# rvp-group/srrg2_slam_interfaces

Hardware: AMD Instinct MI355X
Metric: icp_iterations_per_sec (higher is better)
Workload: dtype f32; 1 GPU; C2: SE(3) point-to-plane AlignerSlice, 100000-pt synthetic cloud pair per GPU, 10 ICP iterations per compute(), gated NN 0.25 m + normal gate, Cauchy 0.05; points=100000, alignments_total=1, all_success=True, last_status=0, last_num_inliers=99432, parallelism=single GPU

## Files before the change

### __graft_entry__.py

```python
import os
import subprocess
import sys

ROOT = os.path.dirname(os.path.abspath(__file__))
if ROOT not in sys.path:
    sys.path.insert(0, ROOT)


def build():
    env = dict(os.environ)
    env.setdefault("HIPCC", "/opt/rocm/bin/hipcc")
    subprocess.check_call(["make", "-j", str(min(8, os.cpu_count() or 1)), "-C", os.path.join(ROOT, "srrg2_slam_interfaces_amd", "csrc"),
                           "ARCH=gfx950", "all", "stall"], env=env)
    subprocess.check_call(["make", "-C", os.path.join(ROOT, "oracle")], env=env)
    subprocess.check_call(["make", "-C", os.path.join(ROOT, "tests", "cpp")], env=env)
    import srrg2_slam_interfaces_amd
    from srrg2_slam_interfaces_amd import _capi

    lib = _capi.lib()
    assert lib.srrg2_amd_abi_version() == 4


def smoke():
    import numpy as np

    import srrg2_slam_interfaces_amd as pkg
    from oracle import pyoracle
    from srrg2_slam_interfaces_amd import _abi as abi
    from srrg2_slam_interfaces_amd import synthetic as syn

    d = syn.cloud_pair_3d(n=8000, seed=77)
    runs = []
    for al in (pyoracle.OracleAligner(abi.SE3_QUAT_RIGHT), pkg.MultiAligner(abi.SE3_QUAT_RIGHT, device=0)):
        c = abi.default_slice_config(abi.SE3_QUAT_RIGHT)
        c.kind = abi.SLICE_P2PLANE
        c.finder_max_distance = 0.25
        c.robustifier = abi.ROBUST_CAUCHY
        c.robustifier_chi_threshold = 0.05
        si = al.add_slice(c)
        al.set_fixed(si, d["fixed"], d["fixed_normals"])
        al.set_moving(si, d["moving"], d["moving_normals"])
        al.set_moving_in_fixed(syn.identity(3))
        al.compute()
        runs.append(al)
    ref, gpu = runs
    assert ref.status() == gpu.status() == abi.SUCCESS, (ref.status(), gpu.status())
    cr, cg = ref.correspondences(0), gpu.correspondences(0)
    assert np.array_equal(cr["fixed_idx"], cg["fixed_idx"]) and np.array_equal(cr["moving_idx"], cg["moving_idx"])
    assert np.max(np.abs(ref.moving_in_fixed() - gpu.moving_in_fixed())) <= 1e-5
    print("smoke ok: %d correspondences, X bit-identical=%s" %
          (len(cg), ref.moving_in_fixed().tobytes() == gpu.moving_in_fixed().tobytes()))


if __name__ == "__main__":
    build()
    if len(sys.argv) > 1 and sys.argv[1] == "smoke":
        smoke()
```

### include/srrg2_slam_amd.h

```cpp
#ifndef SRRG2_SLAM_AMD_H
#define SRRG2_SLAM_AMD_H

#include <stddef.h>
#include <stdint.h>

#ifdef __cplusplus
extern "C" {
#endif

#define SRRG2_AMD_ABI_VERSION 4
#define SRRG2_MAX_SLICES 8


enum srrg2_variable_kind {
  SRRG2_SE2_RIGHT       = 0,
  SRRG2_SE3_EULER_RIGHT = 1,
  SRRG2_SE3_QUAT_RIGHT  = 2
};

enum srrg2_status {
  SRRG2_SUCCESS                    = 0,
  SRRG2_NOT_ENOUGH_CORRESPONDENCES = 1,
  SRRG2_NOT_ENOUGH_INLIERS         = 2,
  SRRG2_FAIL                       = 3
// ... 363 lines not shown
                      srrg2_merge_result* out);
int srrg2_scene_merge_from_aligner(srrg2_scene_h scene, srrg2_scene_h measurement, const float* measurement_in_scene,
                                   srrg2_aligner_h aligner, int slice_idx, srrg2_scene_h clipped,
                                   const srrg2_merger_params* p, srrg2_merge_result* out);


enum srrg2_adaptor_status { SRRG2_ADAPTOR_READY = 0, SRRG2_ADAPTOR_INITIALIZING = 1, SRRG2_ADAPTOR_ERROR = 2 };
enum srrg2_image_type { SRRG2_IMAGE_NONE = 0, SRRG2_IMAGE_U8 = 1, SRRG2_IMAGE_U16 = 2, SRRG2_IMAGE_F32 = 3 };

typedef struct srrg2_depth_adaptor_params {
  float camera_matrix[9];
  int32_t rows, cols;
  float depth_scale;
  float depth_min, depth_max;
  int32_t normal_col_gap, normal_row_gap;
  float normal_max_distance_squared;
  int32_t drop_points_without_normal;
  int32_t compact;
} srrg2_depth_adaptor_params;

typedef struct srrg2_scan_adaptor_params {
  double angle_min, angle_increment;
  float range_min, range_max;
  int32_t normal_half_window;
  float normal_max_distance_squared;
  int32_t drop_points_without_normal;
  int32_t compact;
} srrg2_scan_adaptor_params;

typedef struct srrg2_adapt_result {
  int32_t status;
  int32_t num_raw;
  int32_t num_in_range;
  int32_t num_valid;
  int32_t scene_size;
} srrg2_adapt_result;

void srrg2_adapt_default_depth_params(srrg2_depth_adaptor_params* p);
void srrg2_adapt_default_scan_params(srrg2_scan_adaptor_params* p);
int srrg2_adapt_depth_image(srrg2_scene_h dst, const void* depth, int depth_type, int depth_row_stride_bytes,
                            const void* intensity, int intensity_type, int intensity_row_stride_bytes, int mem,
                            const srrg2_depth_adaptor_params* p, srrg2_adapt_result* out );
int srrg2_adapt_laser_scan(srrg2_scene_h dst, const float* ranges, int num_beams, int mem,
                           const srrg2_scan_adaptor_params* p, srrg2_adapt_result* out );

#define SRRG2_TUNE_PROJ_SEPARATE_LAUNCHES (1 << 17)
#define SRRG2_TUNE_INIT_LAUNCH (1 << 23)
#define SRRG2_TUNE_KNOWN_BITS (SRRG2_TUNE_PROJ_SEPARATE_LAUNCHES | SRRG2_TUNE_INIT_LAUNCH)
typedef struct srrg2_aligner_tuning {
  int32_t strategy_mask;
  int32_t queue_probe_iteration;
  int32_t small_max_points;
  int32_t fast_from_iteration;
  int32_t fast_points_per_thread;
  int32_t fast_min_points;
  int32_t fast_gather;
  int32_t fast_batch_queue;
  int32_t queue_min_points;
  int32_t msort_segments;
  int32_t msort_key_bits;
  int32_t lds_tile;
  float   cell_target;
  float   rmax_cap;
  int32_t search_lists;
  int32_t search_team;
  int32_t batch_pipeline;
  int32_t fused_control;
  int32_t reserved_[6];
} srrg2_aligner_tuning;
void srrg2_aligner_default_tuning(srrg2_aligner_tuning* t);
int srrg2_aligner_get_tuning(srrg2_aligner_h h, srrg2_aligner_tuning* t_out);
int srrg2_aligner_set_tuning(srrg2_aligner_h h, const srrg2_aligner_tuning* t);


int srrg2_aligner_profile_enable(srrg2_aligner_h h, int enable);
int srrg2_aligner_profile_get(srrg2_aligner_h h, double* step_kernel_ms, int64_t* step_kernel_launches,
                              int reset);
#define SRRG2_PATH_FUSED_CONTROL 1
#define SRRG2_PATH_ALL_PASSES_FUSED 2
#define SRRG2_PATH_FINAL_WAVE 4
#define SRRG2_PATH_PROLOGUE_IN_PASS 8
#define SRRG2_PATH_ONE_WORKGROUP 16
#define SRRG2_PATH_PRIORS_FUSED 32
int srrg2_aligner_last_compute_path(srrg2_aligner_h h, int32_t* flags_out);

#ifndef SRRG2_DESCRIPTOR_BYTES
#define SRRG2_DESCRIPTOR_BYTES 32
#endif
typedef struct srrg2_descriptor_db* srrg2_descriptor_db_h;
int srrg2_descriptor_db_create(int device, srrg2_descriptor_db_h* out);
int srrg2_descriptor_db_destroy(srrg2_descriptor_db_h h);
int srrg2_descriptor_db_add(srrg2_descriptor_db_h h, const uint8_t* descriptors, const uint8_t* valid, int n,
                            int* index_out);
int srrg2_descriptor_db_size(srrg2_descriptor_db_h h, int* maps, int64_t* descriptors);
int srrg2_descriptor_db_match(srrg2_descriptor_db_h h, const uint8_t* descriptors, const uint8_t* valid, int n,
                              int64_t query_index, float max_distance, uint32_t min_age, int64_t min_matches,
                              int* K_out);
int srrg2_descriptor_db_get_candidates(srrg2_descriptor_db_h h, int32_t* reference, int64_t* num_matches,
                                       int64_t* corr_offsets, int* n_inout);
int srrg2_descriptor_db_get_correspondences(srrg2_descriptor_db_h h, srrg2_correspondence* buf, int64_t* n_inout);
int srrg2_descriptor_db_get_map_counts(srrg2_descriptor_db_h h, int64_t* counts, int* n_inout);
int srrg2_descriptor_db_last_match_ms(srrg2_descriptor_db_h h, double* ms);
int srrg2_descriptor_db_add_scene(srrg2_descriptor_db_h h, srrg2_scene_h scene, int* index_out);
int srrg2_descriptor_db_match_scene(srrg2_descriptor_db_h h, srrg2_scene_h scene, int64_t query_index, float max_distance,
                                    uint32_t min_age, int64_t min_matches, int* K_out);

#ifdef __cplusplus
}
#endif
#endif
```

### srrg2_slam_interfaces_amd/_abi.py

```python
import ctypes as C

ABI_VERSION = 4
MAX_SLICES = 8

SE2_RIGHT, SE3_EULER_RIGHT, SE3_QUAT_RIGHT = 0, 1, 2
SUCCESS, NOT_ENOUGH_CORRESPONDENCES, NOT_ENOUGH_INLIERS, FAIL = 0, 1, 2, 3
SLICE_P2P, SLICE_P2PLANE, SLICE_REPROJECTION, SLICE_PRIOR = 0, 1, 2, 3
FINDER_NONE, FINDER_NN_GATED, FINDER_PROJECTIVE, FINDER_CORRESPONDENCES = 0, 1, 2, 3
ROBUST_NONE, ROBUST_CLAMP, ROBUST_SATURATED, ROBUST_CAUCHY = 0, 1, 2, 3
FACTOR_INLIER, FACTOR_KERNELIZED, FACTOR_SUPPRESSED = 0, 1, 2
MEM_HOST, MEM_DEVICE, MEM_DEVICE_KEPT = 0, 1, 2


class Correspondence(C.Structure):
    _fields_ = [("fixed_idx", C.c_int32), ("moving_idx", C.c_int32), ("response", C.c_float)]


class IterationStats(C.Structure):
    _fields_ = [
        ("iteration", C.c_int32),
        ("num_inliers", C.c_int32),
        ("num_outliers", C.c_int32),
        ("num_suppressed", C.c_int32),
        ("num_correspondences", C.c_int32),
# ... 121 lines not shown
        ("angle_min", C.c_double),
        ("angle_increment", C.c_double),
        ("range_min", C.c_float),
        ("range_max", C.c_float),
        ("normal_half_window", C.c_int32),
        ("normal_max_distance_squared", C.c_float),
        ("drop_points_without_normal", C.c_int32),
        ("compact", C.c_int32),
    ]


class AdaptResult(C.Structure):
    _fields_ = [("status", C.c_int32), ("num_raw", C.c_int32), ("num_in_range", C.c_int32), ("num_valid", C.c_int32),
                ("scene_size", C.c_int32)]

    def as_dict(self):
        return {n: getattr(self, n) for n, _ in self._fields_}


class NormalsParams(C.Structure):
    _fields_ = [("radius", C.c_float), ("min_neighbours", C.c_int32), ("max_curvature", C.c_float), ("viewpoint", C.c_float * 3),
                ("drop_points_without_normal", C.c_int32), ("reserved", C.c_int32)]


class NormalsResult(C.Structure):
    _fields_ = [("num_points", C.c_int32), ("num_finite", C.c_int32), ("num_with_normal", C.c_int32), ("num_too_few", C.c_int32),
                ("num_degenerate", C.c_int32), ("num_too_curved", C.c_int32), ("scene_size", C.c_int32)]

    def as_dict(self):
        return {n: getattr(self, n) for n, _ in self._fields_}


VOXEL_CENTROID, VOXEL_FIRST = 0, 1


class VoxelParams(C.Structure):
    _fields_ = [("leaf_size", C.c_float), ("origin", C.c_float * 3), ("mode", C.c_int32), ("min_points_per_voxel", C.c_int32),
                ("reserved", C.c_int32 * 2)]


class VoxelResult(C.Structure):
    _fields_ = [("num_points", C.c_int32), ("num_finite", C.c_int32), ("num_occupied", C.c_int32), ("num_voxels", C.c_int32),
                ("num_with_normal", C.c_int32), ("max_points_per_voxel", C.c_int32)]

    def as_dict(self):
        return {n: getattr(self, n) for n, _ in self._fields_}


def transform_size(variable_kind):
    return 9 if variable_kind == SE2_RIGHT else 12


def point_dim(variable_kind):
    return 2 if variable_kind == SE2_RIGHT else 3


def default_aligner_params():
    return AlignerParams(10, 10, 0, 0)


def default_termination_params():
    return TerminationParams(5, 20, 20, 20, 0.2)


def default_slice_config(variable_kind):
    c = SliceConfig()
    c.kind = SLICE_P2P
    c.finder = FINDER_NN_GATED
    c.robustifier = ROBUST_NONE
    c.robustifier_chi_threshold = 1.0
    c.min_num_correspondences = 0
    c.finder_max_distance = 1.0
    c.finder_normal_cos = -2.0
    c.finder_cell_size = 0.0
    ident = [1, 0, 0, 0, 1, 0, 0, 0, 1] if variable_kind == SE2_RIGHT else [1, 0, 0, 0, 0, 1, 0, 0, 0, 0, 1, 0]
    for i, v in enumerate(ident):
        c.sensor_in_robot[i] = v
    for i in range(6):
        c.prior_information_diag[i] = 100.0 if variable_kind == SE2_RIGHT else 1.0
    c.prior_sets_initial_guess = 1
    return c

PATH_FUSED_CONTROL, PATH_ALL_PASSES_FUSED, PATH_FINAL_WAVE, PATH_PROLOGUE_IN_PASS, PATH_ONE_WORKGROUP, PATH_PRIORS_FUSED = 1, 2, 4, 8, 16, 32
```

### srrg2_slam_interfaces_amd/csrc/aligner_host.hip

```cpp
#include <algorithm>
#include <cmath>
#include <cstdio>
#include <cstdlib>
#include <chrono>
#include <cstring>
#include <string>
#include <vector>

#include "det_math.h"
#include "kernels.h"

#include "host_util.h"

namespace srrg2amd {
thread_local std::string g_err;
int fail(int code, const std::string& msg) {
  g_err = msg;
  return code;
}
}

namespace {

using srrg2amd::DevBuf;
// ... 32 lines not shown
  bool moving_has_normals = false;
  DevBuf<int> corr_fixed;
  DevBuf<srrg2_correspondence> gcorr;
  DevBuf<int> gcorr_off;
  DevBuf<uint8_t> gcorr_stat;
  std::vector<srrg2_correspondence> h_gcorr;
  std::vector<int> h_gcorr_off;
  int* qprobe_host = nullptr; size_t qprobe_cap = 0;
  ProblemDev* ms_probs_host = nullptr; size_t ms_probs_host_cap = 0;
  bool ms_pending = false;
  bool fast_queue_only = false;
  DevBuf<float4> prev_f;
  DevBuf<float> prev_m;
  DevBuf<unsigned long long> dbg;
  DevBuf<float4> prev_n;
  DevBuf<int> prev_pos;
  DevBuf<float> corr_resp;
  DevBuf<uint8_t> corr_stat;
  DevBuf<long long> partials;
  const void* slots_zeroed_at = nullptr;
  int slots_zeroed = 0;
  unsigned* bbox_host = nullptr; size_t bbox_host_cap = 0;
  unsigned bbox_seq = 0;
  bool scalars_self_init = false;
  DevBuf<unsigned> bbox_rows;
  DevBuf<unsigned long long> zbuf;
  DevBuf<int> queue;
  DevBuf<int> qcount;
  float prior_Z[12]{};
  bool has_prior = false;
  void release() {
    if (qprobe_host) (void) hipHostFree(qprobe_host);
    qprobe_host = nullptr;
    qprobe_cap  = 0;
    if (bbox_host) (void) hipHostFree(bbox_host);
    bbox_host     = nullptr;
    bbox_host_cap = 0;
    if (ms_probs_host) (void) hipHostFree(ms_probs_host);
    ms_probs_host     = nullptr;
    ms_probs_host_cap = 0;
    fixed_raw.release(); fixed_nrm_raw.release(); fixed_sorted.release(); fixed_nrm_sorted.release();
    cell_start.release(); cursor.release(); scan_sums.release(); scalars.release(); pos_of.release();
    list_start.release(); list_sums.release(); list_ent.release(); list_box.release(); list_offs.release(); list_hdr.release();
    moving.release(); moving_nrm.release(); pinf.release();
    moving_raw.release(); moving_nrm_raw.release(); ms_counts.release(); ms_cursor.release(); ms_sums.release();
    ms_bb.release(); ms_probs.release();
    corr_fixed.release(); gcorr.release(); gcorr_off.release(); gcorr_stat.release(); prev_n.release(); prev_pos.release(); prev_f.release(); prev_m.release(); corr_resp.release(); corr_stat.release(); partials.release(); zbuf.release(); queue.release(); qcount.release(); bbox_rows.release();
  }
};

}

struct srrg2_aligner_s {
  int kind = 0, dim = 3, dof = 6, tsize = 12, device = 0;
  hipStream_t stream = nullptr;
  static constexpr int MAX_PARTS = 8;
  hipStream_t pstream[MAX_PARTS]{};
  int cu_count          = 256;
  int fused_grid_max    = 130000;
  hipEvent_t ev_staged  = nullptr;
  hipEvent_t ev_records = nullptr;
  bool records_unsynced = false;
  int parts_dirty       = 0;
  int batch_parts       = 0;
  int part_begin[MAX_PARTS + 1]{};
  srrg2_aligner_params params{10, 10, 0, 0};
  srrg2_reduce_fn reduce_fn = nullptr;
  void* reduce_user         = nullptr;
  long long shard_total     = 0;
  bool has_term = false;
  srrg2_termination_params term{5, 20, 20, 20, 0.2f};
  std::vector<Slice*> slices;
  float X[12]{};
  int status = SRRG2_FAIL;
  int K = 1;
  DevBuf<ProblemDev> probs;
  DevBuf<ProblemState> states;
  DevBuf<ProblemOut> outs;
  DevBuf<srrg2_iteration_stats> stats;
  DevBuf<float> guesses;
  DevBuf<unsigned long long> pub;
  DevBuf<unsigned> pub_epoch;
  DevBuf<CtlParams> ctl_dev;
  DevBuf<char> staging;
  DevBuf<float4> pair_raw, pair_nrm_raw, pair_sorted, pair_nrm_sorted;
  DevBuf<int> pair_cell_start, pair_cursor, pair_scan_sums, pair_pos_of;
  DevBuf<unsigned> pair_rows;
  DevBuf<ProblemDev> pair_fprobs;
  DevBuf<GridDev> pair_grids;
  DevBuf<char> pair_staging;
  unsigned* pair_rows_host = nullptr; size_t pair_rows_host_cap = 0;
  ProblemDev* pair_fprobs_host = nullptr; size_t pair_fprobs_host_cap = 0;
  GridDev* pair_grids_host = nullptr; size_t pair_grids_host_cap = 0;
  bool pair_normals  = false;
  bool pairs_computed = false;
  ProblemOut* outs_host = nullptr; size_t outs_host_cap = 0;
  int seq = 0;
  srrg2_iteration_stats* stats_host = nullptr; size_t stats_host_cap = 0;
  float* guesses_host = nullptr; size_t guesses_host_cap = 0;
  ProblemDev* probs_host = nullptr; size_t probs_host_cap = 0;
  int max_stats = 0;
  std::vector<srrg2_iteration_stats> last_stats;
  int last_ncorr[SRRG2_MAX_SLICES]{};
  float last_H[36]{};
  bool computed = false;
  int last_path = 0;
  int records_state = 0;
  std::vector<SliceDev> last_sdev;
  std::vector<int> last_proj_owner;
  std::vector<int> last_nm_max;
  srrg2_aligner_tuning tuning{};
  std::string timeline_path;
  bool hosttime = false;
  bool profile = false;
  double prof_ms = 0.0;
  int64_t prof_launches = 0;
  std::vector<std::pair<hipEvent_t, hipEvent_t>> prof_events;
  size_t prof_used = 0;
};

namespace {

using srrg2_aligner = srrg2_aligner_s;

void identity(int kind, float* T) {
  if (kind == SRRG2_SE2_RIGHT) {
    const float I[9] = {1, 0, 0, 0, 1, 0, 0, 0, 1};
    std::memcpy(T, I, sizeof(I));
  } else {
    const float I[12] = {1, 0, 0, 0, 0, 1, 0, 0, 0, 0, 1, 0};
    std::memcpy(T, I, sizeof(I));
  }
}

float proj_extent(int n, float c) {
  return std::fmax(std::fmax((float) n, std::fabs(c + 0.5f)), std::fabs(((float) n - 0.5f) - c));
}

int set_device(srrg2_aligner* a) {
  HIP_TRY(hipSetDevice(a->device));
  return 0;
}

int quiesce_stream2(srrg2_aligner* a) {
  const int n    = a->parts_dirty;
  a->parts_dirty = 0;
  for (int p = 1; p < n; ++p) HIP_TRY(hipStreamSynchronize(a->pstream[p]));
  return 0;
}

template <typename T>
int ensure_pinned(T*& p, size_t& cap, size_t n) {
  if (n <= cap) return 0;
  if (p) (void) hipHostFree(p);
  p = nullptr;
  cap = 0;
  HIP_TRY(hipHostMalloc((void**) &p, (n + 16) * sizeof(T), hipHostMallocDefault));
  cap = n + 16;
  return 0;
}

int stage_input(srrg2_aligner* a, const float* src, int stride_bytes, int n, int dim, int mem, const float** dev_ptr,
                int* stride_floats, size_t staging_offset, DevBuf<char>* staging = nullptr) {
  DevBuf<char>& stg = staging ? *staging : a->staging;
  if (n <= 0) {
    *dev_ptr       = (const float*) stg.p;
// ... 503 lines not shown
  const int split = (K > 1 && a->batch_parts >= 2 && a->part_begin[a->batch_parts] == K) ? a->batch_parts : 0;
  a->batch_parts  = 0;
  if (!split && (rc = quiesce_stream2(a))) return rc;
  const int nslices = (int) a->slices.size();
  int max_nm = 0;
  std::vector<ProblemDev> probs((size_t) K);
  for (int si = 0; si < nslices; ++si) {
    Slice* s = a->slices[si];
    if (s->alias_of < 0) continue;
    if (s->alias_of >= nslices || a->slices[s->alias_of]->alias_of >= 0 || a->slices[s->alias_of]->cfg.kind == SRRG2_SLICE_PRIOR)
      return fail(SRRG2_E_STATE, "compute: a slice shares the clouds of a slice that is gone");
    Slice* o = a->slices[s->alias_of];
    if (s->cfg.finder != SRRG2_FINDER_PROJECTIVE || o->cfg.finder != SRRG2_FINDER_PROJECTIVE)
      return fail(SRRG2_E_UNSUPPORTED, "compute: shared clouds are for slices with the projective finder");
    s->fixed_raw.borrow(o->fixed_raw);   s->fixed_nrm_raw.borrow(o->fixed_nrm_raw);
    s->moving.borrow(o->moving);         s->moving_nrm.borrow(o->moving_nrm);
    s->moving_raw.borrow(o->moving_raw); s->moving_nrm_raw.borrow(o->moving_nrm_raw);
    s->pinf.borrow(o->pinf);             s->scalars.borrow(o->scalars);
    s->nf = o->nf; s->nm_total = o->nm_total; s->has_fixed = o->has_fixed; s->has_moving = o->has_moving;
    s->fixed_has_normals = o->fixed_has_normals; s->moving_has_normals = o->moving_has_normals;
    s->moving_is_batch = o->moving_is_batch;
    const size_t n = (size_t) std::max(s->nm_total, 1);
    if ((rc = s->corr_fixed.reserve(n)) || (rc = s->corr_resp.reserve(n)) || (rc = s->corr_stat.reserve(n))) return rc;
  }
  for (int si = 0; si < nslices; ++si) {
    Slice* s = a->slices[si];
    if (s->cfg.kind == SRRG2_SLICE_PRIOR) {
      if (!s->has_prior) return fail(SRRG2_E_STATE, "compute: prior slice without measurement");
      continue;
    }
    if (!s->has_fixed && !pairs) return fail(SRRG2_E_STATE, "compute: cue slice| no fixed");
    if (!s->has_moving) return fail(SRRG2_E_STATE, "compute: cue slice| no moving");
    if (K == 1 && s->moving_is_batch)
      return fail(SRRG2_E_STATE, "compute: the moving cloud bound to the cue slice is the concatenation of the last "
                                 "compute_batch (K > 1); bind one with set_moving first");
    if (s->cfg.kind == SRRG2_SLICE_P2PLANE && !(pairs ? a->pair_normals : s->fixed_has_normals))
      return fail(SRRG2_E_STATE, "compute: point-to-plane slice needs fixed normals");
    if (s->cfg.finder == SRRG2_FINDER_PROJECTIVE && s->nf != s->cfg.image_rows * s->cfg.image_cols)
      return fail(SRRG2_E_STATE, "compute: projective finder needs an organised fixed cloud of rows x cols points");
  }
  const int slots = 2 * std::max(a->params.max_iterations, 1);
  a->max_stats    = slots;
  if ((rc = a->probs.reserve((size_t) K * std::max(nslices, 1)))) return rc;
  if ((rc = a->states.reserve((size_t) K))) return rc;
  if ((rc = a->outs.reserve((size_t) K))) return rc;
  if ((rc = a->stats.reserve((size_t) K * slots))) return rc;
  if ((rc = a->guesses.reserve((size_t) K * a->tsize))) return rc;
  if ((rc = ensure_pinned(a->outs_host, a->outs_host_cap, (size_t) K))) return rc;
  if ((rc = ensure_pinned(a->stats_host, a->stats_host_cap, (size_t) K * slots))) return rc;
  if ((rc = ensure_pinned(a->guesses_host, a->guesses_host_cap, (size_t) K * a->tsize))) return rc;
  std::memcpy(a->guesses_host, guesses, (size_t) K * a->tsize * sizeof(float));
  if ((rc = ensure_pinned(a->probs_host, a->probs_host_cap, (size_t) K * std::max(nslices, 1)))) return rc;
  std::vector<ProblemDev> all((size_t) K * std::max(nslices, 1));
  for (int si = 0; si < nslices; ++si) {
    Slice* s = a->slices[si];
    const int32_t* off = slice_offsets ? slice_offsets[s->alias_of >= 0 ? s->alias_of : si] : offsets;
    for (int k = 0; k < K; ++k) {
      ProblemDev pd{0, 0};
      if (s->cfg.kind != SRRG2_SLICE_PRIOR) {
        if (K == 1) {
          pd.moff = 0;
          pd.nm   = s->nm_total;
        } else {
          pd.moff = off[k] - off[0];
          pd.nm   = off[k + 1] - off[k];
        }
        max_nm = std::max(max_nm, pd.nm);
      }
      all[(size_t) si * K + k] = pd;
    }
  }
  std::memcpy(a->probs_host, all.data(), all.size() * sizeof(ProblemDev));

  CtlParams C{};
  C.variable_kind = a->kind;
  C.nslices       = nslices;
  C.K             = K;
  C.params        = a->params;
  C.has_term      = a->has_term ? 1 : 0;
  C.term          = a->term;
  C.max_stats     = slots;
  C.seq           = ++a->seq;
  if (C.seq <= 0) C.seq = a->seq = 1;
  for (int k = 0; k < K; ++k) a->outs_host[k].seq = 0;
  const srrg2_aligner_tuning& tn = a->tuning;
  C.probe_it      = tn.queue_probe_iteration;
  if (a->params.max_iterations <= C.probe_it + 3 || K > 4) C.probe_it = -1;
  bool small = false;
  {
    int ncue = 0, fc = -1;
    for (int si = 0; si < nslices; ++si)
      if (a->slices[si]->cfg.kind != SRRG2_SLICE_PRIOR) {
        if (fc < 0) fc = si;
        ++ncue;
      }
    const int small_max = tn.small_max_points;
    small = ncue == 1 && a->slices[fc]->cfg.finder == SRRG2_FINDER_NN_GATED && max_nm <= small_max &&
            a->timeline_path.empty() && !a->reduce_fn;
    const bool priors_launch = nslices > ncue && (tn.fused_control == 2 || nslices - ncue > 2);
    if (small && !pairs && (priors_launch || tn.fused_control == 0 || a->params.max_iterations < 2)) small = max_nm <= 640;
    if (small && !pairs && !(priors_launch || tn.fused_control == 0 || a->params.max_iterations < 2)) {
      const Slice* sfc = a->slices[fc];
      const int sl     = tn.search_lists;
      const bool lists = sl >= 2 || (sl == 1 && K > 4) || (sl < 0 && (K > 4 || sfc->grid_computes >= 1 || sfc->lists_tried));
      small            = !lists && max_nm <= 384;
    }
  }
  const int fast_from = tn.fast_from_iteration;
  bool fuse = false;
  auto fast_ppt_of = [&](int k_launch) {
    return tn.fast_points_per_thread > 0 ? tn.fast_points_per_thread : (k_launch >= (fuse ? 16 : 64) ? 2 : 1);
  };
  const int fast_min = tn.fast_min_points;
  const bool fast_gather = tn.fast_gather >= 0 ? tn.fast_gather != 0 : K > 4;
  const bool fast_batch_queue = tn.fast_batch_queue != 0;
  const int lds_tile = pairs ? 0 : (tn.lds_tile >= 0 ? tn.lds_tile : (K > 4 ? 1 : 0));
  const int search_lists = tn.search_lists;
  const int search_team_knob = tn.search_team;
  std::vector<char> cnl((size_t) std::max(nslices, 1), 0);
  std::vector<SliceDev> sdev((size_t) nslices);
  int first_cue = -1;
  for (int si = 0; si < nslices; ++si) {
    Slice* s     = a->slices[si];
    SliceCtl& sc = C.slices[si];
    sc.kind                     = s->cfg.kind;
    sc.min_num_correspondences  = s->cfg.min_num_correspondences;
    sc.robust_kind              = s->cfg.robustifier;
    sc.robust_thr               = s->cfg.robustifier_chi_threshold;
    sc.gate                     = s->cfg.finder_max_distance;
    sc.has_prior                = s->has_prior ? 1 : 0;
    sc.prior_sets_initial_guess = s->cfg.prior_sets_initial_guess;
    std::memcpy(sc.prior_Z, s->prior_Z, sizeof(sc.prior_Z));
    std::memcpy(sc.prior_info, s->cfg.prior_information_diag, sizeof(sc.prior_info));
    sc.partials  = nullptr;
    sc.finder    = s->cfg.finder;
    sc.K0        = s->cfg.camera_matrix[0];
    sc.K4        = s->cfg.camera_matrix[4];
    sc.umax      = proj_extent(s->cfg.image_cols, s->cfg.camera_matrix[2]);
    sc.vmax      = proj_extent(s->cfg.image_rows, s->cfg.camera_matrix[5]);
    sc.depth_min = s->cfg.depth_min;
    sc.pinf_bits = nullptr;
    sc.ninf_bits = nullptr;
    if (s->cfg.kind == SRRG2_SLICE_PRIOR) continue;
    if (first_cue < 0) first_cue = si;
    int nm_max_s = 0;
    for (int k = 0; k < K; ++k) nm_max_s = std::max(nm_max_s, all[(size_t) si * K + k].nm);
    const int queue_min = tn.queue_min_points;
    const bool want_lists = search_lists >= 2 || (search_lists == 1 && K > 4) ||
                            (search_lists < 0 && (K > 4 || s->grid_computes >= 1 || s->lists_tried));
    if (!pairs) s->grid_computes++;
    if (s->cfg.finder == SRRG2_FINDER_NN_GATED && !small && want_lists && !pairs) {
      if ((rc = ensure_lists(a, s, 96LL << 20))) return rc;
      cnl[(size_t) si] = s->grid.list_R > 0 ? 1 : 0;
    }
    const bool use_queue = s->cfg.finder == SRRG2_FINDER_NN_GATED && nm_max_s >= queue_min && K <= 4 && !small && !cnl[(size_t) si] && !pairs;
    const bool fast_queue = s->cfg.finder == SRRG2_FINDER_NN_GATED && K > 4 && !small && fast_batch_queue && !pairs;
    s->fast_queue_only = fast_queue && !use_queue;
    const int nblocks    = PARTIAL_SLOTS;
    {
      const size_t cap_before = s->partials.cap;
      if ((rc = s->partials.reserve((size_t) 3 * K * nblocks * ACC_N))) return rc;
      if (s->partials.cap != cap_before) s->slots_zeroed = 0;
    }
    if (use_queue || fast_queue) {
      if ((rc = s->queue.reserve((size_t) std::max(s->nm_total, 1) * 10))) return rc;
      if ((rc = s->qcount.reserve((size_t) 2 * K))) return rc;
    }
// ... 273 lines not shown
                                       a->probs.p + (size_t) first_cue * K, a->states.p, a->stats.p, a->outs_host, a->stats_host,
                                       a->stream);
    else
      srrg2amd::launch_icp_small(a->dim, s->cfg.kind == SRRG2_SLICE_P2PLANE, sdev[first_cue], C,
                                 a->probs.p + (size_t) first_cue * K, a->states.p, a->stats.p, a->outs_host, a->stats_host,
                                 a->stream);
  }
  const int probe_it = C.probe_it;
  std::vector<char> queue_on((size_t) std::max(nslices, 1), 1);
  bool probed = false;
  bool final_launched = false;
  auto read_probe = [&]() {
    probed = true;
    for (int si = 0; si < nslices; ++si) {
      if (!sdev[si].queue) continue;
      volatile int* mirror = a->slices[si]->qprobe_host;
      bool small           = true;
      for (int k = 0; k < K; ++k) {
        int spins = 0;
        while (mirror[2 * k] == 0x7f7f7f7f || mirror[2 * k + 1] == 0x7f7f7f7f) {
          if ((++spins & 1023) == 0 && hipStreamQuery(a->stream) != hipErrorNotReady) break;
        }
        const int near = mirror[2 * k], far = mirror[2 * k + 1];
        if (near == 0x7f7f7f7f || far > 32 || near > std::max(1024, all[(size_t) si * K + k].nm / 64)) small = false;
      }
      queue_on[(size_t) si] = small ? 0 : 1;
    }
  };
  auto fused_pass = [&](int slot0, int it) {
    if (!fuse) return false;
    if (fused_all) return true;
    const bool queue_needed = sdev[first_cue].queue && queue_on[(size_t) first_cue];
    return fast_at(slot0, it) && !queue_needed && (slot0 > 0 || probed || probe_it < 0 || !sdev[first_cue].queue);
  };
  auto control = [&](int it, bool last_phase, int h) {
    if (a->reduce_fn) {
      Slice* s = a->slices[first_cue];
      if (a->reduce_fn(a->reduce_user, SRRG2_REDUCE_SUM_I64, s->partials.p, (size_t) K * PARTIAL_SLOTS * ACC_N, (void*) a->stream))
        hook_failed = true;
    }
    const bool last_it = it == a->params.max_iterations - 1;
    if (fuse) {
      Ch[h].parity      = pround % 3;
      Ch[h].zero_parity = (pround + 2) % 3;
      Ch[h].epoch       = epoch + 1;
      const int slot0_now = last_phase && a->params.enable_inlier_only_runs ? a->params.max_iterations : 0;
      if (!fused_all && !probed && slot0_now == 0 && probe_it >= 0 && it == probe_it + 1) read_probe();
      if (!last_it && fused_pass(slot0_now, it + 1) && (fused_all || it != probe_it)) return;
    }
    if (last_phase && last_it) {
      if (fuse && fuse_proj) {
        SliceDev pack[4];
        const ProblemDev* pp[4];
        for (size_t z = 0; z < proj_group.size(); ++z) {
          const int si = proj_group[z];
          Slice* sz    = a->slices[si];
          pack[z]      = sdev[si];
          pp[z]        = a->probs.p + (size_t) si * K;
          pack[z].fc.ctl           = a->ctl_dev.p;
          pack[z].fc.epoch         = epoch + 1;
          pack[z].fc.prev_partials = slot_buffer(sz, pround);
          pack[z].fc.zero_partials = slot_buffer(sz, pround + 2);
        }
        srrg2amd::launch_icp_final_wave_pack(pack, pp, (int) proj_group.size(), a->states.p, a->stats.p, a->outs_host, a->stats_host,
                                             !a->params.enable_inlier_only_runs, hstream[h]);
      } else if (fuse) {
        SliceDev sd          = sdev[first_cue];
        sd.prob0             = h0[h];
        sd.fc.ctl            = a->ctl_dev.p + h;
        sd.fc.epoch          = epoch + 1;
        sd.fc.prev_partials  = slot_buffer(a->slices[first_cue], pround);
        sd.fc.zero_partials  = slot_buffer(a->slices[first_cue], pround + 2);
        srrg2amd::launch_icp_final_wave(Ch[h], sd, a->states.p, a->stats.p, a->outs_host, a->stats_host,
                                        !a->params.enable_inlier_only_runs, hstream[h]);
      } else {
        srrg2amd::launch_icp_control_final(Ch[h], a->states.p, a->stats.p, a->outs_host, a->stats_host,
                                           !a->params.enable_inlier_only_runs , hstream[h]);
      }
      final_launched = true;
    } else {
      srrg2amd::launch_icp_control(Ch[h], a->states.p, a->stats.p, hstream[h]);
    }
  };
  auto run_phase = [&](int slot0, bool last_phase) -> int {
    for (int it = 0; it < a->params.max_iterations; ++it) {
      if (!probed && slot0 == 0 && probe_it >= 0 && it == probe_it + 2) read_probe();
      if (!proj_group.empty()) {
        SliceDev pack[4];
        const ProblemDev* pp[4];
        int nm_max = 0;
        for (size_t z = 0; z < proj_group.size(); ++z) {
          const int si = proj_group[z];
          pack[z]      = sdev[si];
          pp[z]        = a->probs.p + (size_t) si * K;
          for (int k = 0; k < K; ++k) nm_max = std::max(nm_max, all[(size_t) si * K + k].nm);
        }
        hipEvent_t e0 = nullptr, e1 = nullptr;
        if (a->profile) {
          if (a->prof_used == a->prof_events.size()) {
            hipEvent_t x, y;
            HIP_TRY(hipEventCreate(&x));
            HIP_TRY(hipEventCreate(&y));
            a->prof_events.emplace_back(x, y);
          }
          e0 = a->prof_events[a->prof_used].first;
          e1 = a->prof_events[a->prof_used].second;
          a->prof_used++;
          HIP_TRY(hipEventRecord(e0, a->stream));
        }
        if (fuse)
          for (size_t z = 0; z < proj_group.size(); ++z) {
            Slice* sz              = a->slices[proj_group[z]];
            pack[z].fc.ctl         = a->ctl_dev.p;
            pack[z].fc.epoch       = epoch;
            pack[z].partials       = slot_buffer(sz, pround);
            pack[z].fc.prev_partials = slot_buffer(sz, pround + 2);
            pack[z].fc.zero_partials = slot_buffer(sz, pround + 1);
            pack[z].fc.prior       = (slot0 > 0 || it > 0) ? 1 : 0;
            if (it == 0) pack[z].fc.prior_mask = 0;
          }
        if (proj_fused) {
          const bool first_pass_init = fold_init && fuse_proj && slot0 == 0 && it == 0;
          srrg2amd::launch_proj_step_fused(pack, pp, (int) proj_group.size(), a->states.p, K, nm_max, a->stream,
                                           first_pass_init ? &Ch[0] : nullptr, first_pass_init ? &fold_inl : nullptr,
                                           first_pass_init ? a->probs.p : nullptr);
          sdev[proj_group[0]].zbuf_parity ^= 1;
        } else {
          srrg2amd::launch_proj_step_pack(pack, pp, (int) proj_group.size(), a->states.p, K, nm_max, a->stream);
          for (int si : proj_group) sdev[si].zbuf_parity ^= 1;
        }
        if (a->profile) HIP_TRY(hipEventRecord(e1, a->stream));
        control(it, last_phase, 0);
        ++epoch;
        ++pround;
        continue;
      }
      for (int si = 0; si < nslices; ++si) {
        Slice* s = a->slices[si];
        if (s->cfg.kind == SRRG2_SLICE_PRIOR) continue;
        const bool plane = s->cfg.kind == SRRG2_SLICE_P2PLANE;
        int nm_max       = 0;
        for (int k = 0; k < K; ++k) nm_max = std::max(nm_max, all[(size_t) si * K + k].nm);
        hipEvent_t e0 = nullptr, e1 = nullptr;
        if (a->profile) {
          if (a->prof_used == a->prof_events.size()) {
            hipEvent_t x, y;
            HIP_TRY(hipEventCreate(&x));
            HIP_TRY(hipEventCreate(&y));
            a->prof_events.emplace_back(x, y);
          }
          e0 = a->prof_events[a->prof_used].first;
          e1 = a->prof_events[a->prof_used].second;
          a->prof_used++;
          HIP_TRY(hipEventRecord(e0, a->stream));
        }
        if (s->cfg.finder == SRRG2_FINDER_CORRESPONDENCES) {
          int max_nc = 0;
          for (int k = 0; k < K; ++k) max_nc = std::max(max_nc, s->h_gcorr_off[(size_t) k + 1] - s->h_gcorr_off[(size_t) k]);
          srrg2amd::launch_corr_step(a->dim, plane, sdev[si], a->probs.p + (size_t) si * K, a->states.p, K, max_nc, a->stream);
        } else if (s->cfg.finder == SRRG2_FINDER_PROJECTIVE) {
          srrg2amd::launch_proj_step(s->cfg.kind == SRRG2_SLICE_REPROJECTION, sdev[si], a->probs.p + (size_t) si * K,
                                     a->states.p, K, nm_max, a->stream);
          sdev[si].zbuf_parity ^= 1;
        } else {
          SliceDev sd = sdev[si];
          const bool fast = (slot0 > 0 || (it >= fast_from && it >= 1)) && nm_max >= fast_min;
          if (!queue_on[si] || (s->fast_queue_only && !fast)) {
            sd.queue  = nullptr;
            sd.qcount = nullptr;
// ... 55 lines not shown
      if ((rc = run_phase(a->params.max_iterations, true))) return rc;
    }
  }
  if (!final_launched)
    for (int h = 0; h < nhalves; ++h)
      srrg2amd::launch_icp_finalize(Ch[h], a->states.p, a->stats.p, a->outs_host, a->stats_host,
                                    !a->params.enable_inlier_only_runs , hstream[h]);
  if (split) a->parts_dirty = std::max(a->parts_dirty, split);
  HIP_TRY(hipGetLastError());
  const bool hosttime = a->hosttime;
  auto t_enq = std::chrono::steady_clock::now();
  bool seen = true;
  for (int k = 0; k < K && seen; ++k) {
    volatile int* flag = &a->outs_host[k].seq;
    int spins          = 0;
    hipStream_t qs = a->stream;
    for (int h = 1; h < nhalves; ++h)
      if (k >= h0[h]) qs = hstream[h];
    while (*flag != C.seq)
      if ((++spins & 4095) == 0 && hipStreamQuery(qs) != hipErrorNotReady) {
        seen = *flag == C.seq;
        break;
      }
  }
  if (!seen || a->profile || !a->timeline_path.empty()) {
    HIP_TRY(hipStreamSynchronize(a->stream));
    for (int h = 1; h < nhalves; ++h) HIP_TRY(hipStreamSynchronize(hstream[h]));
  }
  if (hook_failed) return fail(SRRG2_E_INVALID, "the reduction hook of the point-sharded alignment failed");
  if (hosttime) {
    auto t_end = std::chrono::steady_clock::now();
    std::fprintf(stderr, "compute: prep %.1f us, first launch %.1f us, enqueue %.1f us, wait %.1f us\n",
                 std::chrono::duration<double, std::micro>(t_prep - t_begin).count(),
                 std::chrono::duration<double, std::micro>(t_init - t_prep).count(),
                 std::chrono::duration<double, std::micro>(t_enq - t_begin).count(),
                 std::chrono::duration<double, std::micro>(t_end - t_enq).count());
  }
  if (const char* tl_path = a->timeline_path.empty() ? nullptr : a->timeline_path.c_str()) {
    for (int si = 0; si < nslices; ++si) {
      Slice* s = a->slices[si];
      if (!sdev[si].dbg) continue;
      int nm_max = 0;
      for (int k = 0; k < K; ++k) nm_max = std::max(nm_max, all[(size_t) si * K + k].nm);
      const unsigned long long nw = (unsigned long long) K * ((nm_max + 255) / 256) * 4;
      std::vector<unsigned long long> host(32 * nw * 16);
      HIP_TRY(hipMemcpy(host.data(), s->dbg.p, host.size() * sizeof(unsigned long long), hipMemcpyDeviceToHost));
      if (FILE* f = std::fopen(tl_path, "wb")) {
        std::fwrite(&nw, sizeof(nw), 1, f);
        std::fwrite(host.data(), sizeof(unsigned long long), host.size(), f);
        std::fclose(f);
      }
    }
  }
  if (a->profile) {
    for (size_t i = 0; i < a->prof_used; ++i) {
      float ms = 0.f;
      HIP_TRY(hipEventElapsedTime(&ms, a->prof_events[i].first, a->prof_events[i].second));
      a->prof_ms += ms;
      a->prof_launches++;
    }
    a->prof_used = 0;
  }
  for (Slice* sl : a->slices) sl->ms_pending = false;
  a->K = K;
  const ProblemOut& o = a->outs_host[K - 1];
  std::memcpy(a->X, o.X, sizeof(float) * a->tsize);
  a->status = o.status;
  int ns    = std::min(o.nstats, slots);
  a->last_stats.assign(a->stats_host + (size_t) (K - 1) * slots, a->stats_host + (size_t) (K - 1) * slots + ns);
  for (int si = 0; si < SRRG2_MAX_SLICES; ++si) a->last_ncorr[si] = o.ncorr[si];
  std::memcpy(a->last_H, o.H, sizeof(a->last_H));
  a->computed = true;
  a->last_sdev = sdev;
  a->last_proj_owner.assign((size_t) nslices, -1);
  if (proj_fused)
    for (int si : proj_group) a->last_proj_owner[(size_t) si] = proj_group[0];
  a->last_nm_max.assign((size_t) nslices, 0);
  for (int si = 0; si < nslices; ++si)
    for (int k = 0; k < K; ++k) a->last_nm_max[(size_t) si] = std::max(a->last_nm_max[(size_t) si], all[(size_t) si * K + k].nm);
  a->records_state  = pairs ? 2 : 1;
  a->pairs_computed = pairs;
  a->last_path = (fuse ? SRRG2_PATH_FUSED_CONTROL : 0) | (fuse && fused_all ? SRRG2_PATH_ALL_PASSES_FUSED : 0) |
                 (fuse && final_launched && !small ? SRRG2_PATH_FINAL_WAVE : 0) | (fold_init ? SRRG2_PATH_PROLOGUE_IN_PASS : 0) |
                 (small ? SRRG2_PATH_ONE_WORKGROUP : 0) | (fuse && prior_mask ? SRRG2_PATH_PRIORS_FUSED : 0);
  if (fuse && final_launched && first_cue >= 0 && !small) {
    for (int si = 0; si < nslices; ++si) {
      if (si != first_cue && !(fuse_proj && std::find(proj_group.begin(), proj_group.end(), si) != proj_group.end())) continue;
      Slice* s           = a->slices[si];
      s->slots_zeroed    = 3 * K;
      s->slots_zeroed_at = (const void*) s->partials.p;
    }
  }
  return 0;
}

int plan_batch_parts(srrg2_aligner* a, int K, const int32_t* offsets, int* pbegin) {
  int nparts = 0;
  {
    const srrg2_aligner_tuning& tn = a->tuning;
    int max_nm = 0;
    for (int k = 0; k < K; ++k) max_nm = std::max(max_nm, offsets[k + 1] - offsets[k]);
    bool one_cue = true;
    for (size_t si = 1; si < a->slices.size(); ++si)
      if (a->slices[si]->cfg.kind != SRRG2_SLICE_PRIOR) one_cue = false;
    int want = tn.batch_pipeline == 0 ? 1 : (tn.batch_pipeline == 1 ? 2 : (tn.batch_pipeline > 1 ? tn.batch_pipeline : (K >= 8 ? 2 : 1)));
    want     = std::min(std::min(want, (int) srrg2_aligner::MAX_PARTS), K);
    if (want >= 2 && one_cue && a->slices[0]->cfg.finder == SRRG2_FINDER_NN_GATED && max_nm > tn.small_max_points &&
        !tn.fast_batch_queue && !a->reduce_fn && !a->profile && a->timeline_path.empty()) {
      nparts = want;
      for (int p = 1; p < nparts; ++p)
        if (!a->pstream[p] && hipStreamCreateWithFlags(&a->pstream[p], hipStreamNonBlocking) != hipSuccess) {
          (void) hipGetLastError();
          a->pstream[p] = nullptr;
          nparts        = p >= 2 ? p : 0;
          break;
        }
      for (int p = 0; p <= nparts; ++p) pbegin[p] = (int) ((long long) K * p / nparts);
    }
  }
  return nparts;
}

void fill_batch_results(const srrg2_aligner* a, int K, srrg2_batch_result* results) {
  const int slots = a->max_stats;
  for (int k = 0; k < K; ++k) {
    const ProblemOut& o = a->outs_host[k];
    std::memset(&results[k], 0, sizeof(results[k]));
    std::memcpy(results[k].moving_in_fixed, o.X, sizeof(float) * a->tsize);
    results[k].status         = o.status;
    results[k].num_iterations = o.nstats;
    if (o.nstats > 0) results[k].last = a->stats_host[(size_t) k * slots + std::min(o.nstats, slots) - 1];
    int tot = 0;
    for (size_t si = 0; si < a->slices.size(); ++si) {
      const int c = a->slices[si]->cfg.kind == SRRG2_SLICE_PRIOR ? 1 : o.ncorr[si];
      if (c >= 0) tot += c;
    }
    results[k].num_correspondences = tot;
    std::memcpy(results[k].information, o.H, sizeof(o.H));
  }
}

int materialize_records(srrg2_aligner* a, bool host_wait = true) {
  if (a->records_state != 1) {
    if (host_wait && a->records_unsynced) {
      HIP_TRY(hipStreamSynchronize(a->stream));
      a->records_unsynced = false;
    }
    return 0;
  }
  int rc;
  if ((rc = set_device(a))) return rc;
  if ((rc = quiesce_stream2(a))) return rc;
  std::vector<char> rebuilt(a->slices.size(), 0);
  for (size_t si = 0; si < a->slices.size() && si < a->last_sdev.size(); ++si) {
    Slice* s = a->slices[si];
    if (s->cfg.kind == SRRG2_SLICE_PRIOR) continue;
    if (s->cfg.finder == SRRG2_FINDER_PROJECTIVE) {
      const int owner = si < a->last_proj_owner.size() && a->last_proj_owner[si] >= 0 ? a->last_proj_owner[si] : (int) si;
      srrg2amd::launch_proj_records(a->last_sdev[(size_t) owner], a->last_sdev[si], a->probs.p + (size_t) owner * a->K,
                                    a->probs.p + si * (size_t) a->K, a->states.p, a->K, a->last_nm_max[si],
                                    !rebuilt[(size_t) owner], a->stream);
      rebuilt[(size_t) owner] = 1;
      continue;
    }
    if (s->cfg.finder != SRRG2_FINDER_NN_GATED) continue;
    srrg2amd::launch_icp_outputs(a->dim, s->cfg.kind == SRRG2_SLICE_P2PLANE, a->last_sdev[si], a->probs.p + si * (size_t) a->K,
                                 a->states.p, a->K, a->last_nm_max[si], a->stream);
// ... 66 lines not shown
}

int srrg2_aligner_set_tuning(srrg2_aligner_h a, const srrg2_aligner_tuning* t) {
  if (!a || !t) return fail(SRRG2_E_INVALID, "set_tuning: null argument");
  if (t->fast_points_per_thread < 0 || t->fast_from_iteration < 1 || !(t->cell_target > 0.f) || t->msort_key_bits > 18 ||
      t->msort_key_bits < -1 || t->msort_segments < 0 || t->search_team < 0)
    return fail(SRRG2_E_INVALID, "set_tuning: value out of range");
  if (t->strategy_mask & ~SRRG2_TUNE_KNOWN_BITS) return fail(SRRG2_E_INVALID, "set_tuning: unknown strategy_mask bit");
  a->tuning = *t;
  return 0;
}

void srrg2_termination_default_params(srrg2_termination_params* p) {
  if (!p) return;
  p->window_size = 5;
  p->num_correspondences_range = 20;
  p->num_inliers_range = 20;
  p->num_outliers_range = 20;
  p->chi_epsilon = 0.2f;
}

void srrg2_slice_default_config(srrg2_slice_config* c, int variable_kind) {
  if (!c) return;
  std::memset(c, 0, sizeof(*c));
  c->kind = SRRG2_SLICE_P2P;
  c->finder = SRRG2_FINDER_NN_GATED;
  c->robustifier = SRRG2_ROBUST_NONE;
  c->robustifier_chi_threshold = 1.f;
  c->min_num_correspondences = 0;
  c->finder_max_distance = 1.f;
  c->finder_normal_cos = -2.f;
  c->finder_cell_size = 0.f;
  identity(variable_kind, c->sensor_in_robot);
  for (int i = 0; i < 6; ++i) c->prior_information_diag[i] = variable_kind == SRRG2_SE2_RIGHT ? 100.f : 1.f;
  c->prior_sets_initial_guess = 1;
}

int srrg2_aligner_create(int variable_kind, int device, srrg2_aligner_h* out) {
  if (!out || variable_kind < 0 || variable_kind > 2) return fail(SRRG2_E_INVALID, "create: bad arguments");
  int n = 0;
  hipError_t e = hipGetDeviceCount(&n);
  if (e != hipSuccess || n <= 0)
    return fail(SRRG2_E_NO_DEVICE, "create: no HIP device visible (this library has no CPU fallback)");
  if (device < 0 || device >= n) return fail(SRRG2_E_INVALID, "create: bad device ordinal");
  srrg2_aligner* a = new srrg2_aligner();
  a->kind   = variable_kind;
  a->dim    = variable_kind == SRRG2_SE2_RIGHT ? 2 : 3;
  a->dof    = variable_kind == SRRG2_SE2_RIGHT ? 3 : 6;
  a->tsize  = variable_kind == SRRG2_SE2_RIGHT ? 9 : 12;
  a->device = device;
  identity(variable_kind, a->X);
  tuning_from_environment(&a->tuning);
  if (const char* tl = std::getenv("SRRG2_AMD_TIMELINE")) a->timeline_path = tl;
  a->hosttime = std::getenv("SRRG2_AMD_HOSTTIME") != nullptr;
  if (const char* fg = std::getenv("SRRG2_AMD_FUSED_GRID_MAX")) a->fused_grid_max = std::atoi(fg);
  bool ok = hipSetDevice(device) == hipSuccess && hipStreamCreateWithFlags(&a->stream, hipStreamNonBlocking) == hipSuccess;
  a->pstream[0] = a->stream;
  ok = ok && hipEventCreateWithFlags(&a->ev_staged, hipEventDisableTiming) == hipSuccess;
  ok = ok && hipEventCreateWithFlags(&a->ev_records, hipEventDisableTiming) == hipSuccess;
  if (ok && (hipDeviceGetAttribute(&a->cu_count, hipDeviceAttributeMultiprocessorCount, device) != hipSuccess || a->cu_count <= 0)) {
    (void) hipGetLastError();
    a->cu_count = 256;
  }
  if (!ok) {
    for (int p = 0; p < srrg2_aligner::MAX_PARTS; ++p)
      if (a->pstream[p]) (void) hipStreamDestroy(a->pstream[p]);
    delete a;
    return fail(SRRG2_E_HIP, "create: cannot create stream");
  }
  *out = a;
  return 0;
}

int srrg2_aligner_destroy(srrg2_aligner_h a) {
  if (!a) return 0;
  (void) hipSetDevice(a->device);
  for (int p = 0; p < srrg2_aligner::MAX_PARTS; ++p)
    if (a->pstream[p]) (void) hipStreamSynchronize(a->pstream[p]);
  for (Slice* s : a->slices) {
    s->release();
    delete s;
  }
  a->probs.release(); a->states.release(); a->outs.release(); a->stats.release(); a->guesses.release();
  a->pub.release(); a->pub_epoch.release(); a->ctl_dev.release();
  a->staging.release();
  a->pair_raw.release(); a->pair_nrm_raw.release(); a->pair_sorted.release(); a->pair_nrm_sorted.release();
  a->pair_cell_start.release(); a->pair_cursor.release(); a->pair_scan_sums.release(); a->pair_pos_of.release();
  a->pair_rows.release(); a->pair_fprobs.release(); a->pair_grids.release(); a->pair_staging.release();
  if (a->pair_rows_host) (void) hipHostFree(a->pair_rows_host);
  if (a->pair_fprobs_host) (void) hipHostFree(a->pair_fprobs_host);
  if (a->pair_grids_host) (void) hipHostFree(a->pair_grids_host);
  if (a->outs_host) (void) hipHostFree(a->outs_host);
  if (a->stats_host) (void) hipHostFree(a->stats_host);
  if (a->guesses_host) (void) hipHostFree(a->guesses_host);
  if (a->probs_host) (void) hipHostFree(a->probs_host);
  for (auto& ev : a->prof_events) {
    (void) hipEventDestroy(ev.first);
    (void) hipEventDestroy(ev.second);
  }
  if (a->ev_staged) (void) hipEventDestroy(a->ev_staged);
  if (a->ev_records) (void) hipEventDestroy(a->ev_records);
  for (int p = srrg2_aligner::MAX_PARTS - 1; p >= 0; --p)
    if (a->pstream[p]) (void) hipStreamDestroy(a->pstream[p]);
  delete a;
  return 0;
}

int srrg2_aligner_set_params(srrg2_aligner_h a, const srrg2_aligner_params* p) {
  if (!a || !p || p->max_iterations < 0) return fail(SRRG2_E_INVALID, "set_params: bad arguments");
  a->params = *p;
  return 0;
}

int srrg2_aligner_set_termination(srrg2_aligner_h a, const srrg2_termination_params* p) {
  if (!a) return fail(SRRG2_E_INVALID, "set_termination: null handle");
  if (!p) {
    a->has_term = false;
    return 0;
  }
  if (p->window_size < 1 || p->window_size > TERM_WINDOW_MAX) return fail(SRRG2_E_INVALID, "set_termination: window_size");
  a->has_term = true;
  a->term     = *p;
  return 0;
}

int srrg2_aligner_add_slice(srrg2_aligner_h a, const srrg2_slice_config* c, int* idx) {
  if (!a || !c) return fail(SRRG2_E_INVALID, "add_slice: bad arguments");
  if ((int) a->slices.size() >= SRRG2_MAX_SLICES) return fail(SRRG2_E_INVALID, "add_slice: too many slices");
  if (c->kind != SRRG2_SLICE_PRIOR && c->finder != SRRG2_FINDER_NN_GATED && c->finder != SRRG2_FINDER_PROJECTIVE &&
      c->finder != SRRG2_FINDER_CORRESPONDENCES)
    return fail(SRRG2_E_INVALID, "add_slice| no finder");
  if (c->finder == SRRG2_FINDER_CORRESPONDENCES && c->kind != SRRG2_SLICE_P2P && c->kind != SRRG2_SLICE_P2PLANE)
    return fail(SRRG2_E_INVALID, "add_slice: given correspondences drive point-to-point / point-to-plane factors");
  if (c->finder == SRRG2_FINDER_PROJECTIVE || c->kind == SRRG2_SLICE_REPROJECTION) {
    if (a->dim != 3) return fail(SRRG2_E_UNSUPPORTED, "add_slice: projective finder / reprojection factor are SE(3) only");
    if (c->finder != SRRG2_FINDER_PROJECTIVE)
      return fail(SRRG2_E_INVALID, "add_slice: a reprojection slice needs the projective finder");
    if (c->image_rows <= 0 || c->image_cols <= 0 || !(c->depth_min > 0.f) || !(c->depth_max >= c->depth_min) ||
        !(c->camera_matrix[0] > 0.f) || !(c->camera_matrix[4] > 0.f))
      return fail(SRRG2_E_INVALID, "add_slice: projective slice with bad camera / image / depth range");
  }
  if (c->kind == SRRG2_SLICE_PRIOR && a->kind == SRRG2_SE3_EULER_RIGHT)
    return fail(SRRG2_E_UNSUPPORTED, "add_slice: SE3 prior factors exist for the quaternion variable only "
                                     "(SE3PriorErrorFactorAD, aligner_slice_odometry_prior.h:33)");
  Slice* s = new Slice();
  s->cfg   = *c;
  if (idx) *idx = (int) a->slices.size();
  a->slices.push_back(s);
  return 0;
}

int srrg2_aligner_clear_slices(srrg2_aligner_h a) {
  if (!a) return fail(SRRG2_E_INVALID, "clear_slices: null handle");
  (void) hipSetDevice(a->device);
  (void) hipStreamSynchronize(a->stream);
  for (Slice* s : a->slices) {
    s->release();
    delete s;
  }
  a->slices.clear();
  return 0;
}

int srrg2_aligner_set_robustifier(srrg2_aligner_h a, int si, int kind, float thr) {
  int rc = check_slice(a, si, "set_robustifier");
  if (rc) return rc;
  a->slices[si]->cfg.robustifier               = kind;
// ... 747 lines not shown
```

### srrg2_slam_interfaces_amd/csrc/device_types.h

```cpp
#pragma once
#include <hip/hip_runtime.h>
#include <stdint.h>

#include "../../include/srrg2_slam_amd.h"

#define ACC_N 32
#define PARTIAL_SLOTS 32
#define ACC_B 21
#define ACC_CHI_IN 27
#define ACC_CHI_OUT 28
#define ACC_N_IN 29
#define ACC_N_OUT 30
#define ACC_N_CORR 31
#define TERM_WINDOW_MAX 64
#define NO_MATCH 0x7fffffff

__host__ __device__ __forceinline__ constexpr int hidx(int a, int b) {
  return a * 6 - (a * (a - 1)) / 2 + (b - a);
}

struct GridDev {
  float ox, oy, oz;
  float h, inv_h;
  int nx, ny, nz;
  int rmax;
  int rfar_gate;
  float gate2;
  float gate2_ext;
  int n;
  const int* cell_start;
  const float4* pts;
  const float4* nrm;
  const int* pos_of;
  int list_R;
  const struct GridLists* lists;
};
struct GridLists {
  int R;
  int lnx, lny, lnz;
  const int* start;
  const uint4* ent;
  float cls_b2[14];
};
#define CNL_MAX_R 3
#ifndef CNL_ENTRY_MAX
#define CNL_ENTRY_MAX 16
#endif
#define CNL_MAX_CLASS 12

#define PUB_SLICE_GRANULES 64
#define PUB_G_KEXP 24
#define PUB_G_FLAGS 25
#define PUB_G_NSTATS 26
#define PUB_G_WCOUNT 27
#define PUB_G_NPASSES 28
#define PUB_G_X 32
#define PUB_FLAG_STOP 1u
#define PUB_FLAG_PHASE1 2u
#define PUB_FLAG_PRIOR 4u
#define PUB_EPOCH_REPLICAS 8
#define PUB_EPOCH_STRIDE 32
struct CtlParams;
struct FusedCtl {
  unsigned long long* pub;
  unsigned* pub_epoch;
  const CtlParams* ctl;
  srrg2_iteration_stats* stats;
  long long* prev_partials;
  long long* zero_partials;
  int epoch;
  int min_num_correspondences;
  int max_stats;
  int has_term;
  int first_round;
  int prior;
  int prior_mask;
  int nslices;
};

struct SliceDev {
  GridDev grid;
  const float4* mpts;
  const float4* mnrm;
  int* corr_fixed;
  float* corr_resp;
  uint8_t* corr_stat;
  float4* prev_f;
  float4* prev_n;
  int* prev_pos;
  float* prev_m;
  long long* partials;
  void* queue;
  int* qcount;
  int slice_idx;
  int robust_kind;
  float robust_thr;
  float normal_cos;
  int use_normal_gate;
  int gather_prev;
  int variable_kind;
  int finder;
  int factor;
  float K[9];
  int rows, cols;
  float depth_min, depth_max;
  float gate;
  const float4* fixed_org;
  const float4* fixed_org_nrm;
  unsigned long long* zbuf;
  int zbuf_parity;
  const srrg2_correspondence* gcorr;
  const int* gcorr_off;
  uint8_t* gcorr_stat;
  const float4* moving_raw;
  unsigned long long* dbg;
  int prob0;
  float Sinv[12];
  FusedCtl fc;
};

struct ProblemDev {
  int moff;
  int nm;
};

struct ProblemState {
  float X[12];
  float Xprev[12];
  int status;
  int done;
  int finished;
  int nstats;
  int phase;
  int kexp[SRRG2_MAX_SLICES];
  int ncorr[SRRG2_MAX_SLICES];
  int ninl[SRRG2_MAX_SLICES];
  int qmode[SRRG2_MAX_SLICES];
  float Tf[SRRG2_MAX_SLICES][12], Tfprev[SRRG2_MAX_SLICES][12];
  float Tlast[SRRG2_MAX_SLICES][12];
  int npasses;
  int w_count;
  double w_corr[TERM_WINDOW_MAX], w_inl[TERM_WINDOW_MAX], w_out[TERM_WINDOW_MAX], w_chi[TERM_WINDOW_MAX];
  double last_H[36], last_b[6], last_dx[6];
};

struct ProblemOut {
  float X[12];
  int status;
  int nstats;
  int ncorr[SRRG2_MAX_SLICES];
  float H[36];
  int seq;
};

struct SliceCtl {
  int kind;
  int min_num_correspondences;
  int robust_kind;
  float robust_thr;
  float gate;
  int has_prior;
  int prior_sets_initial_guess;
  float prior_Z[12];
  float prior_info[6];
  int finder;
  float K0, K4;
  float umax, vmax;
  float depth_min;
  int* qcount;
  int* qprobe_host;
  const ProblemDev* probs;
  int nm_global;
  const long long* partials;
  const unsigned* pinf_bits;
  const unsigned* ninf_bits;
  const unsigned* finf_bits;
  const int* gcorr_off;
  float Sinv[12];
};

#define PAIR_ROW_WORDS 8
#define PAIR_ROW_NINF 7

struct InitInline {
  int use;
  float guess[12];
  ProblemDev pd[SRRG2_MAX_SLICES];
};

#define INIT_BATCH_MAX 16
struct InitBatch {
  float guess[INIT_BATCH_MAX][12];
  ProblemDev pd[INIT_BATCH_MAX];
  int cue_slice;
};

struct CtlParams {
  int variable_kind;
  int nslices;
  int K;
  srrg2_aligner_params params;
  int has_term;
  srrg2_termination_params term;
  int max_stats;
  int probe_it;
  int seq;
  int prob0, nprob;
  unsigned long long* pub;
  unsigned* pub_epoch;
  CtlParams* ctl_dev;
  int epoch;
  int parity;
  int zero_parity;
  SliceCtl slices[SRRG2_MAX_SLICES];
};
```

### srrg2_slam_interfaces_amd/csrc/kernels.h

```cpp
#pragma once
#include "device_types.h"

namespace srrg2amd {

void launch_ingest(const float* src, int stride_floats, int n, int dim, float4* dst, unsigned* maxabs_bits,
                   int finite_per_point, hipStream_t s);
void launch_ingest_batch(const float* src, int stride_floats, const ProblemDev* probs, int K, int max_nm, int dim,
                         float4* dst, unsigned* maxabs_bits, int finite_per_point, hipStream_t s);
void launch_bbox(const float4* pts, int n, unsigned* mn, unsigned* mx, int* nvalid, hipStream_t s);
void launch_ingest_bbox(const float* src, int stride_floats, int n, int dim, float4* dst, unsigned* maxabs_bits, unsigned* mn,
                        unsigned* mx, int* nvalid, hipStream_t s, unsigned* ticket, unsigned* host_out, unsigned seq,
                        unsigned* block_out , unsigned* clear_after);
#define INGEST_BBOX_MAX_BLOCKS 512
void launch_grid_count(const GridDev& g, const float4* pts, int n, int* counts, hipStream_t s);
void launch_count_nonzero(const int* counts, int n, int* out, hipStream_t s);
int scan_num_blocks(int n);
void launch_exclusive_scan(int* data, int n, int* block_sums, int* grand_total, hipStream_t s, int* copy = nullptr);
void launch_grid_scatter(const GridDev& g, const float4* pts, const float4* nrm, int n, int* cursor, float4* out_pts,
                         float4* out_nrm, int* pos_of, hipStream_t s);
void launch_cnl_build(const GridDev& g, const GridLists& L, const int4* offs, int noffs, int* list_start, uint2* box_at,
                      uint4* ent, hipStream_t s);
void launch_icp_step_cnl(int dim, bool plane, const SliceDev& S, const GridLists& GL, const ProblemDev* probs,
                         ProblemState* states, int K, int max_nm, int team, hipStream_t s, const CtlParams* init_C = nullptr,
                         const InitInline* init_inl = nullptr, const InitBatch* init_bat = nullptr);
bool launch_msort_local(const float* src, int sf, const float* nsrc, int nsf, const ProblemDev* probs, int K, int dim, int kbits,
                        int aniso, int segments, int max_nm, float4* out_pts, float4* out_nrm, unsigned* maxabs_bits,
                        hipStream_t s);
void launch_msort(const float4* pts, const float4* nrm, const ProblemDev* probs, int K, int max_nm, int kbits, int aniso,
                  unsigned* bb, int* counts, int* cursor, int* scan_sums, int* scan_total, float4* out_pts,
                  float4* out_nrm, hipStream_t s);
void launch_icp_step(int dim, bool plane, const SliceDev& S, const ProblemDev* probs, ProblemState* states, int K,
                     int max_nm, hipStream_t s, const CtlParams* init_C = nullptr, const InitInline* init_inl = nullptr);
void launch_icp_step_tile(int dim, bool plane, const SliceDev& S, const ProblemDev* probs, ProblemState* states, int K,
                          int max_nm, int cap, hipStream_t s);
void launch_icp_step_fast(int dim, bool plane, const SliceDev& S, const ProblemDev* probs, ProblemState* states, int K,
                          int max_nm, int ppt, bool gather, hipStream_t s);
void launch_icp_outputs(int dim, bool plane, const SliceDev& S, const ProblemDev* probs, const ProblemState* states, int K,
                        int max_nm, hipStream_t s);
int icp_step_blocks(int max_nm);
int icp_queue_blocks(int max_nm, int K);
void launch_proj_step_pack(const SliceDev* slices, const ProblemDev* const* probs, int nslices, ProblemState* states, int K,
                           int max_nm, hipStream_t s);
void launch_proj_records(const SliceDev& S0, const SliceDev& S, const ProblemDev* probs0, const ProblemDev* probs,
                         ProblemState* states, int K, int max_nm, bool rebuild, hipStream_t s);
void launch_proj_step_fused(const SliceDev* slices, const ProblemDev* const* probs, int nslices, ProblemState* states, int K,
                            int max_nm, hipStream_t s,
                            const CtlParams* init_C = nullptr, const InitInline* init_inl = nullptr, ProblemDev* probs_base = nullptr);
void launch_corr_step(int dim, bool plane, const SliceDev& S, const ProblemDev* probs, ProblemState* states, int K,
                      int max_ncorr, hipStream_t s);
void launch_proj_step(bool repro, const SliceDev& S, const ProblemDev* probs, ProblemState* states, int K, int max_nm,
                      hipStream_t s);
void launch_icp_init(const CtlParams& C, const ProblemDev* probs_host, ProblemDev* probs, ProblemState* states,
                     const float* guesses_host, int tsize, hipStream_t s, bool pairs = false);
bool make_init_inline(const CtlParams& C, const ProblemDev* probs_host, const float* guesses_host, int tsize, InitInline* inl);
void launch_icp_control(const CtlParams& C, ProblemState* states, srrg2_iteration_stats* stats, hipStream_t s);
void launch_icp_final_wave_pack(const SliceDev* slices, const ProblemDev* const* probs, int nslices, ProblemState* states,
                                srrg2_iteration_stats* stats, ProblemOut* outs_host, srrg2_iteration_stats* stats_host,
                                bool with_post, hipStream_t s);
void launch_icp_small(int dim, bool plane, const SliceDev& S, const CtlParams& C, const ProblemDev* probs, ProblemState* states,
                      srrg2_iteration_stats* stats, ProblemOut* outs_host, srrg2_iteration_stats* stats_host, hipStream_t s);
void launch_icp_step_pairs(int dim, bool plane, const SliceDev& S, const GridDev* grids, const ProblemDev* probs,
                           ProblemState* states, int K, int max_nm, hipStream_t s);
void launch_icp_step_fast_pairs(int dim, bool plane, const SliceDev& S, const GridDev* grids, const ProblemDev* probs,
                                ProblemState* states, int K, int max_nm, int ppt, bool gather, hipStream_t s);
void launch_icp_small_pairs(int dim, bool plane, const SliceDev& S, const GridDev* grids, const CtlParams& C, const ProblemDev* probs,
                            ProblemState* states, srrg2_iteration_stats* stats, ProblemOut* outs_host,
                            srrg2_iteration_stats* stats_host, hipStream_t s);
void launch_pairs_ingest(const float* src, int sf, const float* nsrc, int nsf, const ProblemDev* fprobs, int K, int max_nf, int dim,
                         float4* dst, float4* dst_nrm, unsigned* rows, hipStream_t s);
void launch_pairs_grid_build(const GridDev* grids, const ProblemDev* fprobs, int K, int max_nf, int max_cells, int total_cells,
                             const float4* pts, const float4* nrm, int* cell_start, int* cursor, int* scan_sums, int* scan_total,
                             float4* out_pts, float4* out_nrm, int* pos_of, hipStream_t s);
void launch_icp_final_wave(const CtlParams& C, const SliceDev& S, ProblemState* states, srrg2_iteration_stats* stats,
                           ProblemOut* outs_host, srrg2_iteration_stats* stats_host, bool with_post, hipStream_t s);
void launch_icp_control_final(const CtlParams& C, ProblemState* states, srrg2_iteration_stats* stats, ProblemOut* outs_host,
                               srrg2_iteration_stats* stats_host, bool with_post, hipStream_t s);
void launch_icp_post(const CtlParams& C, ProblemState* states, const srrg2_iteration_stats* stats, hipStream_t s);
void launch_icp_finalize(const CtlParams& C, ProblemState* states, const srrg2_iteration_stats* stats,
                         ProblemOut* outs_host, srrg2_iteration_stats* stats_host, bool with_post, hipStream_t s);

}
```

### srrg2_slam_interfaces_amd/csrc/kernels.hip

```cpp
#include <cstdlib>
#include <algorithm>

#include "kernels.h"

#include <type_traits>

#include "det_math.h"

#include "device_util.h"

namespace {

#define FX_MAGIC 6755399441055744.0
#define FX_MAGIC_BITS 0x4338000000000000ll
__device__ __forceinline__ long long fx_bits(double biased) { return __double_as_longlong(biased) - FX_MAGIC_BITS; }

__device__ __forceinline__ unsigned long long key_min(unsigned long long a, unsigned long long b) {
  double r;
  asm("v_min_f64 %0, %1, %2" : "=v"(r) : "v"(__longlong_as_double((long long) a)), "v"(__longlong_as_double((long long) b)));
  return (unsigned long long) __double_as_longlong(r);
}

template <int DIM>
__device__ __forceinline__ float cand_d2(const float4 f, float qx, float qy, float qz) {
// ... 1826 lines not shown
        ((st->nstats > 0 || st->phase == 1) ? PUB_FLAG_PRIOR : 0u);
  else if (lane == PUB_G_NSTATS) v = (unsigned) st->nstats;
  else if (lane == PUB_G_WCOUNT) v = (unsigned) st->w_count;
  else if (lane == PUB_G_NPASSES) v = (unsigned) st->npasses;
  else if (lane >= PUB_G_X && lane < PUB_G_X + 12) v = __float_as_uint(st->X[lane - PUB_G_X]);
  return v;
}
__device__ __forceinline__ void pub_write_epoch(unsigned* pub_epoch, int prob, int lane, unsigned epoch) {
  if (lane < PUB_EPOCH_REPLICAS)
    __hip_atomic_store(pub_epoch + ((size_t) prob * PUB_EPOCH_REPLICAS + lane) * PUB_EPOCH_STRIDE, epoch, __ATOMIC_RELAXED,
                       __HIP_MEMORY_SCOPE_AGENT);
}
__device__ __forceinline__ void pub_publish_state(const CtlParams& C, const ProblemState* st, int prob, int lane, unsigned epoch) {
  for (int s = 0; s < C.nslices; ++s) {
    if (C.slices[s].kind == SRRG2_SLICE_PRIOR) continue;
    pub_store(C.pub + ((size_t) prob * SRRG2_MAX_SLICES + s) * PUB_SLICE_GRANULES + lane,
              ((unsigned long long) epoch << 32) | pub_granule_of(C, st, s, lane));
  }
}

template <int D>
__device__ __forceinline__ int wave_prior(const float (&prior_Z)[12], const float (&prior_info)[6], float robust_thr, int rk,
                                          const float (&X)[12], int lane, double& pH, double& pb, double& chi_out) {
  const int hr = lane / D, hc = lane - hr * D;
  double e[D];
  float Zinv[12], E[12];
  double qw = 0.0;
  if constexpr (D == 6) {
    dm::se3_inverse(prior_Z, Zinv);
    dm::se3_compose(Zinv, X, E);
    dm::se3_t2v_quat(E, e);
    const double n2 = (e[3] * e[3] + e[4] * e[4]) + e[5] * e[5];
    qw              = n2 < 1.0 ? sqrt(1.0 - n2) : 0.0;
  } else {
    dm::se2_inverse(prior_Z, Zinv);
    dm::se2_compose(Zinv, X, E);
    dm::se2_t2v(E, e);
  }
  auto Jat = [&](int k, int col) -> double {
    if constexpr (D == 6) {
      if (k < 3) return col == 0 ? (double) E[k * 4 + 0] : (col == 1 ? (double) E[k * 4 + 1] : (col == 2 ? (double) E[k * 4 + 2] : 0.0));
      const double m0 = k == 3 ? qw : (k == 4 ? e[5] : -e[4]);
      const double m1 = k == 3 ? -e[5] : (k == 4 ? qw : e[3]);
      const double m2 = k == 3 ? e[4] : (k == 4 ? -e[3] : qw);
      return col == 3 ? m0 : (col == 4 ? m1 : (col == 5 ? m2 : 0.0));
    } else {
      if (k < 2) return col == 0 ? (double) E[k * 3 + 0] : (col == 1 ? (double) E[k * 3 + 1] : 0.0);
      return col == 2 ? 1.0 : 0.0;
    }
  };
  double chi = 0.0;
#pragma unroll
  for (int i = 0; i < D; ++i) chi = chi + (e[i] * (double) prior_info[i]) * e[i];
  bool kernelized;
  const float w = robust_weight(rk, robust_thr, (float) chi, kernelized);
  chi_out       = chi;
  const int status = !isfinite(chi) ? (int) SRRG2_FACTOR_SUPPRESSED
                                    : (kernelized ? (int) SRRG2_FACTOR_KERNELIZED : (int) SRRG2_FACTOR_INLIER);
  pH = 0.0;
  pb = 0.0;
  if (status == SRRG2_FACTOR_SUPPRESSED) return status;
  double th = 0.0, tb = 0.0;
#pragma unroll
  for (int k = 0; k < D; ++k) {
    th = th + (Jat(k, hr) * (double) prior_info[k]) * Jat(k, hc);
    tb = tb + (Jat(k, lane) * (double) prior_info[k]) * e[k];
  }
  pH = (double) w * th;
  pb = (double) w * tb;
  return status;
}

struct FinalRegs {
  bool applied;
  float Xl;
  double Hl;
  int nstats;
  int num_in;
  int sw;
  bool stats_written;
  int nc[4], ni[4];
};

template <int D, int MAXS, bool PUBLISH = true, bool PRIORS = false, bool FINAL = false>
__device__ __forceinline__ void wave_control(const SliceDev* __restrict__ Sv, int ns, ProblemState* __restrict__ states, int prob,
                                             const unsigned long long (&g)[MAXS], unsigned (*out)[MAXS] = nullptr,
                                             FinalRegs* fin = nullptr) {
  if constexpr (FINAL) fin->applied = false;
  const FusedCtl& F  = Sv[0].fc;
  const int lane     = threadIdx.x & 63;
  ProblemState* st   = &states[prob];
  const unsigned epoch = (unsigned) F.epoch;
  constexpr int TS   = D == 3 ? 9 : 12;
  int pw[SRRG2_MAX_SLICES];
#pragma unroll
  for (int q = 0; q < SRRG2_MAX_SLICES; ++q) {
    pw[q] = 0;
    if constexpr (PRIORS)
      if (((unsigned) F.prior_mask >> q) & 1u) pw[q] = reinterpret_cast<const int*>(&F.ctl->slices[q])[lane & 31];
  }
  long long v[MAXS];
#pragma unroll
  for (int z = 0; z < MAXS; ++z) {
    v[z] = 0;
    if (z < ns) {
      const long long* p = Sv[z].fc.prev_partials + (size_t) prob * PARTIAL_SLOTS * ACC_N;
#pragma unroll
      for (int q = 0; q < PARTIAL_SLOTS * ACC_N / 64; ++q) v[z] += p[q * 64 + lane];
    }
  }
  const int w          = (int) (unsigned) g[0];
  float Xl             = __int_as_float(__shfl(w, (PUB_G_X + lane) & 63));
  const unsigned fl0   = (unsigned) __builtin_amdgcn_readlane(w, PUB_G_FLAGS);
  const int nstats0    = __builtin_amdgcn_readlane(w, PUB_G_NSTATS);
  const int wc         = __builtin_amdgcn_readlane(w, PUB_G_WCOUNT);
  const int npasses0   = __builtin_amdgcn_readlane(w, PUB_G_NPASSES);
  float told[MAXS];
  int kexp[MAXS];
#pragma unroll
  for (int z = 0; z < MAXS; ++z) {
    told[z] = __int_as_float((int) (unsigned) g[z]);
    kexp[z] = __builtin_amdgcn_readlane((int) (unsigned) g[z], PUB_G_KEXP);
  }
  if (fl0 & PUB_FLAG_STOP) {
#pragma unroll
    for (int z = 0; z < MAXS; ++z)
      if (z < ns) {
        if constexpr (PUBLISH)
          pub_store(F.pub + ((size_t) prob * SRRG2_MAX_SLICES + Sv[z].slice_idx) * PUB_SLICE_GRANULES + lane,
                    ((unsigned long long) epoch << 32) | (unsigned) g[z]);
        else
          (*out)[z] = (unsigned) g[z];
      }
    if constexpr (PUBLISH) pub_write_epoch(F.pub_epoch, prob, lane, epoch);
    return;
  }
  double wo = 0.0, wi = 0.0, wx = 0.0;
  int W = 1;
  if (F.has_term) {
    W = F.ctl->term.window_size;
    if (lane < W) {
      wo = st->w_out[lane];
      wi = st->w_inl[lane];
      wx = st->w_chi[lane];
    }
  }
  int ps0 = -1, ps1 = -1, pt0 = 0, pt1 = 0;
  double pH0 = 0.0, pb0 = 0.0, pc0 = 0.0, pH1 = 0.0, pb1 = 0.0, pc1 = 0.0;
  if constexpr (PRIORS) {
    const unsigned pm0 = (unsigned) F.prior_mask, pm1 = pm0 & (pm0 - 1u);
    ps0 = pm0 ? __builtin_ctz(pm0) : -1;
    ps1 = pm1 ? __builtin_ctz(pm1) : -1;
    float Xa[12];
#pragma unroll
    for (int i = 0; i < 12; ++i) Xa[i] = i < TS ? rl_f(Xl, i) : 0.f;
#pragma unroll 1
    for (int j = 0; j < 2; ++j) {
      const int sl = j == 0 ? ps0 : ps1;
      if (sl < 0) break;
      int pword = pw[0];
#pragma unroll
      for (int q = 1; q < SRRG2_MAX_SLICES; ++q) pword = sl == q ? pw[q] : pword;
      constexpr int W_RK = (int) (offsetof(SliceCtl, robust_kind) / 4), W_THR = (int) (offsetof(SliceCtl, robust_thr) / 4),
                    W_Z = (int) (offsetof(SliceCtl, prior_Z) / 4), W_INFO = (int) (offsetof(SliceCtl, prior_info) / 4);
      static_assert(W_INFO + 6 <= 32, "the prefetched head of SliceCtl covers the prior's fields");
      const int robust_kind  = __builtin_amdgcn_readlane(pword, W_RK);
      const float robust_thr = __int_as_float(__builtin_amdgcn_readlane(pword, W_THR));
      float pZ[12], pinfo[6];
#pragma unroll
      for (int i = 0; i < 12; ++i) pZ[i] = __int_as_float(__builtin_amdgcn_readlane(pword, W_Z + i));
#pragma unroll
      for (int i = 0; i < 6; ++i) pinfo[i] = __int_as_float(__builtin_amdgcn_readlane(pword, W_INFO + i));
      const int rk = ((fl0 & PUB_FLAG_PHASE1) && robust_kind != SRRG2_ROBUST_NONE) ? (int) SRRG2_ROBUST_CLAMP : robust_kind;
      double pH, pb, pchi;
      const int pstat = wave_prior<D>(pZ, pinfo, robust_thr, rk, Xa, lane, pH, pb, pchi);
      if (j == 0) {
        pH0 = pH; pb0 = pb; pc0 = pchi; pt0 = pstat;
      } else {
        pH1 = pH; pb1 = pb; pc1 = pchi; pt1 = pstat;
      }
    }
  }
  const int hr = lane / D, hc = lane - hr * D;
  const int hsrc = hidx(hr < hc ? hr : hc, hr < hc ? hc : hr) & 31;
  double Hl = 0.0, bl = 0.0;
  int num_in = 0, num_out = 0, num_sup = 0, num_corr = 0;
  double chi_in = 0.0, chi_out = 0.0;
  bool good = false;
  const unsigned pmask = PRIORS ? (unsigned) F.prior_mask : 0u;
  const int first_cue  = Sv[0].slice_idx;
  const int s_end      = pmask ? F.nslices : first_cue + 1;
#pragma unroll 1
  for (int sl = pmask ? 0 : first_cue; sl < s_end; ++sl) {
  if ((pmask >> sl) & 1u) {
    const bool pfirst = sl == ps0;
    const double pH = pfirst ? pH0 : pH1, pb = pfirst ? pb0 : pb1, pchi = pfirst ? pc0 : pc1;
    const int pstat = pfirst ? pt0 : pt1;
    good = true;
    Hl   = Hl + pH;
    bl   = bl + pb;
    if (pstat == SRRG2_FACTOR_INLIER) {
      num_in += 1;
      chi_in = chi_in + pchi;
    } else if (pstat == SRRG2_FACTOR_KERNELIZED) {
      num_out += 1;
      chi_out = chi_out + pchi;
    } else {
      num_sup += 1;
    }
    num_corr += 1;
    if constexpr (PUBLISH)
      if (lane == 0) st->ninl[sl] = pstat == SRRG2_FACTOR_INLIER ? 1 : 0;
    continue;
  }
  if (sl != first_cue) continue;
#pragma unroll
  for (int z = 0; z < MAXS; ++z) {
    if (z >= ns) break;
    v[z] += __shfl_xor(v[z], 32);
    if constexpr (PUBLISH) {
      long long* p = Sv[z].fc.zero_partials + (size_t) prob * PARTIAL_SLOTS * ACC_N;
#pragma unroll
      for (int q = 0; q < PARTIAL_SLOTS * ACC_N / 64; ++q) p[q * 64 + lane] = 0;
    }
    const double scaled = (double) v[z] * dm::pow2(-kexp[z]);
    const int nc = (int) rl_ll(v[z], ACC_N_CORR), n_in = (int) rl_ll(v[z], ACC_N_IN), n_out = (int) rl_ll(v[z], ACC_N_OUT);
    good |= nc > Sv[z].fc.min_num_correspondences;
    if constexpr (FINAL)
      if (z < 4) {
        fin->nc[z] = nc;
        fin->ni[z] = n_in;
      }
    Hl = Hl + __shfl(scaled, hsrc);
    bl = bl + __shfl(scaled, (ACC_B + lane) & 31);
    num_in += n_in;
    num_out += n_out;
    num_sup += nc - n_in - n_out;
    num_corr += nc >= 0 ? nc : 0;
    chi_in  = chi_in + rl_d(scaled, ACC_CHI_IN);
    chi_out = chi_out + rl_d(scaled, ACC_CHI_OUT);
    if constexpr (PUBLISH) {
      const int s = Sv[z].slice_idx;
      if (lane == 0) {
        st->ncorr[s] = nc;
        st->ninl[s]  = n_in;
      }
      if (lane < 12) st->Tlast[s][lane] = told[z];
    }
  }
  }
  if constexpr (PUBLISH)
    if (lane == 0) st->npasses = npasses0 + 1;
  if (!good) {
    if constexpr (PUBLISH)
      if (lane == 0) {
        st->status = SRRG2_NOT_ENOUGH_CORRESPONDENCES;
        st->done   = 1;
      }
#pragma unroll
    for (int z = 0; z < MAXS; ++z) {
      if (z >= ns) break;
      unsigned nv = (unsigned) g[z];
      if (lane == PUB_G_FLAGS) nv = fl0 | PUB_FLAG_STOP;
      if (lane == PUB_G_NPASSES) nv = (unsigned) (npasses0 + 1);
      if constexpr (PUBLISH)
        pub_store(F.pub + ((size_t) prob * SRRG2_MAX_SLICES + Sv[z].slice_idx) * PUB_SLICE_GRANULES + lane,
                  ((unsigned long long) epoch << 32) | nv);
      else
        (*out)[z] = nv;
    }
    if constexpr (PUBLISH) pub_write_epoch(F.pub_epoch, prob, lane, epoch);
    return;
  }
  PASS_TS_W(F.epoch, 5, Hl);
  double Lv = 0.0, Dv = 0.0, Iv = 0.0;
  double Tv = Hl;
  bool bad  = false;
#pragma unroll
  for (int j = 0; j < D; ++j) {
    const double sj = rl_d(Tv, j * D + j);
    if (!(sj > 0.0)) {
      bad = true;
      break;
    }
    const double inv = 1.0 / sj;
    if (lane == j * D + j) {
      Dv = sj;
      Iv = inv;
    }
    if (hc == j && hr > j && lane < D * D) Lv = Tv * inv;
    if (j + 1 < D) {
      const double lij = __shfl(Lv, (hr * D + j) & 63);
      const double ljj = __shfl(Lv, (hc * D + j) & 63);
      Tv               = Tv - (lij * ljj) * sj;
    }
  }
  double yv = 0.0, dxv = 0.0;
  if (!bad) {
    double tv = -bl;
#pragma unroll
    for (int k = 0; k < D; ++k) {
      const double yk = rl_d(tv, k);
      if (lane == k) yv = tv;
      if (k + 1 < D) tv = tv - __shfl(Lv, (lane * D + k) & 63) * yk;
    }
#pragma unroll
// ... 37 lines not shown
        const double qw  = sqrt(small ? 1.0 - n2 : 1.0);
        const double xx = v3 * v3, yy = v4 * v4, zz = v5 * v5;
        const double xy = v3 * v4, xz = v3 * v5, yz = v4 * v5;
        const double wx_ = qw * v3, wy_ = qw * v4, wz_ = qw * v5;
        R0 = small ? 1.0 - 2.0 * (yy + zz) : 1.0; R1 = small ? 2.0 * (xy - wz_) : 0.0;      R2 = small ? 2.0 * (xz + wy_) : 0.0;
        R3 = small ? 2.0 * (xy + wz_) : 0.0;      R4 = small ? 1.0 - 2.0 * (xx + zz) : 1.0; R5 = small ? 2.0 * (yz - wx_) : 0.0;
        R6 = small ? 2.0 * (xz - wy_) : 0.0;      R7 = small ? 2.0 * (yz + wx_) : 0.0;      R8 = small ? 1.0 - 2.0 * (xx + yy) : 1.0;
      } else {
        double sa, ca, sb, cb, sc, cc;
        dm::sincos(v3, sa, ca);
        dm::sincos(v4, sb, cb);
        dm::sincos(v5, sc, cc);
        R0 = cb * cc;                   R1 = -(cb * sc);                R2 = sb;
        R3 = ca * sc + (sa * sb) * cc;  R4 = ca * cc - (sa * sb) * sc;  R5 = -(sa * cb);
        R6 = sa * sc - (ca * sb) * cc;  R7 = sa * cc + (ca * sb) * sc;  R8 = ca * cb;
      }
      const int i = lane >> 2, j = lane & 3;
      const double a0 = (double) __shfl(Xl, (i * 4 + 0) & 63), a1 = (double) __shfl(Xl, (i * 4 + 1) & 63),
                   a2 = (double) __shfl(Xl, (i * 4 + 2) & 63), a3 = (double) __shfl(Xl, (i * 4 + 3) & 63);
      double r0 = v0, r1 = v1, r2 = v2;
      if (j == 0) { r0 = R0; r1 = R3; r2 = R6; }
      if (j == 1) { r0 = R1; r1 = R4; r2 = R7; }
      if (j == 2) { r0 = R2; r1 = R5; r2 = R8; }
      double o = (a0 * r0 + a1 * r1) + a2 * r2;
      if (j == 3) o = o + a3;
      if (lane < 12) Xl = (float) o;
    }
    if constexpr (PUBLISH)
      if (lane < TS) st->X[lane] = Xl;
  }
  PASS_TS_W(F.epoch, 7, (double) Xl);
  const float chi_in_f = (float) chi_in, chi_out_f = (float) chi_out;
  static_assert(sizeof(srrg2_iteration_stats) == 32, "eight words");
  const int sw = lane == 0 ? nstats0 : lane == 1 ? num_in : lane == 2 ? num_out : lane == 3 ? num_sup : lane == 4 ? num_corr
               : lane == 5 ? (bad ? 1 : 0) : lane == 6 ? __float_as_int(chi_in_f) : __float_as_int(chi_out_f);
  if (PUBLISH && nstats0 < F.max_stats && lane < 8) reinterpret_cast<int*>(F.stats + (size_t) prob * F.max_stats + nstats0)[lane] = sw;
  if constexpr (FINAL) {
    fin->applied = true;
    fin->Xl = Xl;
    fin->Hl = Hl;
    fin->nstats = nstats0 + 1;
    fin->num_in = num_in;
    fin->sw = sw;
    fin->stats_written = nstats0 < F.max_stats;
  }
  if constexpr (PUBLISH)
    if (lane == 0) st->nstats = nstats0 + 1;
  bool stop = false;
  int wc1   = wc;
  if (F.has_term && num_in != 0) {
    const srrg2_termination_params& tp = F.ctl->term;
    const float chi = chi_in_f / (float) num_in;
    const int slot  = wc % W;
    const int n     = wc + 1 < W ? wc + 1 : W;
    wc1             = wc + 1;
    if (n >= W) {
      const bool in = lane < n;
      if (lane == slot) {
        wo = (double) num_out;
        wi = (double) num_in;
        wx = (double) chi;
      }
      const double first_o = rl_d(wo, 0), first_i = rl_d(wi, 0), first_x = rl_d(wx, 0);
      const double omax = wave_max_d(in ? wo : first_o), omin = wave_min_d(in ? wo : first_o);
      const double imax = wave_max_d(in ? wi : first_i), imin = wave_min_d(in ? wi : first_i);
      const double xmax = wave_max_d(in ? wx : first_x), xmin = wave_min_d(in ? wx : first_x);
      stop = true;
      if (omax - omin > (double) tp.num_correspondences_range) stop = false;
      if (imax - imin > (double) tp.num_inliers_range) stop = false;
      const float chi_range = (float) (xmax - xmin);
      if (chi_range > (float) tp.num_outliers_range) stop = false;
      if (chi_range / (float) xmax > tp.chi_epsilon) stop = false;
    }
    if (PUBLISH && lane == 0) {
      st->w_corr[slot] = num_corr;
      st->w_inl[slot]  = num_in;
      st->w_out[slot]  = num_out;
      st->w_chi[slot]  = (double) chi;
      st->w_count      = wc + 1;
    }
  }
  if (PUBLISH && stop && lane == 0) st->done = 1;
  const unsigned x_up = __float_as_uint(__shfl(Xl, (lane - PUB_G_X) & 63));
#pragma unroll
  for (int z = 0; z < MAXS; ++z) {
    if (z >= ns) break;
    const int s = Sv[z].slice_idx;
    float tnew  = told[z];
    if (!bad) {
      const float* A = Sv[z].Sinv;
      const int i = (lane >> 2) % 3, j = lane & 3;
      const float A0 = i == 0 ? A[0] : (i == 1 ? A[D == 6 ? 4 : 3] : A[D == 6 ? 8 : 6]);
      const float A1 = i == 0 ? A[1] : (i == 1 ? A[D == 6 ? 5 : 4] : A[D == 6 ? 9 : 7]);
      const float A2 = i == 0 ? A[2] : (i == 1 ? A[D == 6 ? 6 : 5] : A[D == 6 ? 10 : 8]);
      if constexpr (D == 6) {
        const float A3  = i == 0 ? A[3] : (i == 1 ? A[7] : A[11]);
        const double b0 = (double) __shfl(Xl, (0 * 4 + j) & 63), b1 = (double) __shfl(Xl, (1 * 4 + j) & 63),
                     b2 = (double) __shfl(Xl, (2 * 4 + j) & 63);
        double o = ((double) A0 * b0 + (double) A1 * b1) + (double) A2 * b2;
        if (j == 3) o = o + (double) A3;
        tnew = (float) o;
      } else {
        const int jj = j == 3 ? 2 : j;
        const double b0 = (double) __shfl(Xl, (0 * 3 + jj) & 63), b1 = (double) __shfl(Xl, (1 * 3 + jj) & 63);
        double o = (double) A0 * b0 + (double) A1 * b1;
        if (j == 3) o = o + (double) A2;
        float f = (float) o;
        if (j == 2) f = 0.f;
        if (i == 2) f = j == 2 ? 1.f : 0.f;
        tnew = f;
      }
      if (PUBLISH && lane < 12) st->Tf[s][lane] = tnew;
    }
    if (PUBLISH && lane < 12) st->Tfprev[s][lane] = told[z];
    const unsigned told_up = __float_as_uint(__shfl(told[z], (lane - 12) & 63));
    unsigned nv = 0u;
    if (lane < 12) nv = __float_as_uint(tnew);
    if (lane >= 12 && lane < 24) nv = told_up;
    if (lane == PUB_G_KEXP) nv = (unsigned) kexp[z];
    if (lane == PUB_G_FLAGS) nv = (stop ? PUB_FLAG_STOP : 0u) | (fl0 & PUB_FLAG_PHASE1) | PUB_FLAG_PRIOR;
    if (lane == PUB_G_NSTATS) nv = (unsigned) (nstats0 + 1);
    if (lane == PUB_G_WCOUNT) nv = (unsigned) wc1;
    if (lane == PUB_G_NPASSES) nv = (unsigned) (npasses0 + 1);
    if (lane >= PUB_G_X && lane < PUB_G_X + 12) nv = x_up;
    if constexpr (PUBLISH)
      pub_store(F.pub + ((size_t) prob * SRRG2_MAX_SLICES + s) * PUB_SLICE_GRANULES + lane, ((unsigned long long) epoch << 32) | nv);
    else
      (*out)[z] = nv;
  }
  if constexpr (PUBLISH) pub_write_epoch(F.pub_epoch, prob, lane, epoch);
}

struct PassView {
  float T[12], Tprev[12];
  int kexp;
  bool stop, phase1, prior;
};

__device__ __forceinline__ void pass_view_legacy(const SliceDev& S, const ProblemState* __restrict__ st, PassView& v) {
#pragma unroll
  for (int i = 0; i < 12; ++i) v.T[i] = st->Tf[S.slice_idx][i];
#pragma unroll
  for (int i = 0; i < 12; ++i) v.Tprev[i] = st->Tfprev[S.slice_idx][i];
  v.kexp   = st->kexp[S.slice_idx];
  v.stop   = st->done || st->finished;
  v.phase1 = st->phase == 1;
  v.prior  = st->nstats > 0 || st->phase == 1;
}

#ifndef SRRG2_FUSED_POLL_LIMIT
#define SRRG2_FUSED_POLL_LIMIT 64
#endif
#ifdef SRRG2_FUSED_STALL
__device__ unsigned long long g_fused_fallbacks;
extern "C" int srrg2_amd_debug_fused_fallbacks(unsigned long long* out, int reset) {
  if (out && hipMemcpyFromSymbol(out, HIP_SYMBOL(g_fused_fallbacks), sizeof(unsigned long long)) != hipSuccess) return -1;
  if (reset) {
    const unsigned long long zero = 0;
    if (hipMemcpyToSymbol(HIP_SYMBOL(g_fused_fallbacks), &zero, sizeof(zero)) != hipSuccess) return -1;
  }
  return 0;
}
#define FUSED_STALL()                                                              \
  do {                                                                             \
    for (int stall_i = 0; stall_i < (SRRG2_FUSED_STALL); ++stall_i) __builtin_amdgcn_s_sleep(127); \
  } while (0)
#define FUSED_FALLBACK_COUNT()                                                     \
  do {                                                                             \
    if ((threadIdx.x & 63) == 0) atomicAdd(&g_fused_fallbacks, 1ull);              \
  } while (0)
#else
#define FUSED_STALL() do { } while (0)
#define FUSED_FALLBACK_COUNT() do { } while (0)
#endif

template <int DIM, bool PRIORS = false>
__device__ __forceinline__ void fused_control_if_due(const SliceDev& S, ProblemState* __restrict__ states, int prob) {
  if (blockIdx.y != 0 || threadIdx.x >= 64) return;
  const unsigned long long g[1] = {
    pub_load(S.fc.pub + ((size_t) prob * SRRG2_MAX_SLICES + S.slice_idx) * PUB_SLICE_GRANULES + (threadIdx.x & 63))};
  if (!__all((unsigned) (g[0] >> 32) == (unsigned) S.fc.epoch)) {
    FUSED_STALL();
    wave_control<DIM == 3 ? 6 : 3, 1, true, PRIORS>(&S, 1, states, prob, g);
  }
  PASS_TS(S.fc.epoch, 1);
}

template <int DIM, bool PRIORS = false>
__device__ __forceinline__ void pass_view_fused(const SliceDev& S, ProblemState* __restrict__ states, int prob, PassView& v) {
  __shared__ unsigned rec_lds[PUB_SLICE_GRANULES];
  const int lane = threadIdx.x & 63;
  if (threadIdx.x < 64) {
    const unsigned long long* rec = S.fc.pub + ((size_t) prob * SRRG2_MAX_SLICES + S.slice_idx) * PUB_SLICE_GRANULES + lane;
    const bool late      = (int) (blockIdx.y * gridDim.x + blockIdx.x) >= S.fc.first_round;
    unsigned long long g = late ? *rec : pub_load(rec);
    if (!__all((unsigned) (g >> 32) == (unsigned) S.fc.epoch)) {
      const unsigned* ep = S.fc.pub_epoch + ((size_t) prob * PUB_EPOCH_REPLICAS + (blockIdx.y & (PUB_EPOCH_REPLICAS - 1))) * PUB_EPOCH_STRIDE;
      int spins = 0;
      for (;;) {
        if ((int) __hip_atomic_load(ep, __ATOMIC_RELAXED, __HIP_MEMORY_SCOPE_AGENT) >= S.fc.epoch) {
          g = pub_load(rec);
          if (__all((unsigned) (g >> 32) == (unsigned) S.fc.epoch)) break;
        }
        __builtin_amdgcn_s_sleep(4);
        if (++spins > SRRG2_FUSED_POLL_LIMIT) {
          g = pub_load(rec);
          if (__all((unsigned) (g >> 32) == (unsigned) S.fc.epoch)) break;
          if (__all((unsigned) (g >> 32) == (unsigned) (S.fc.epoch - 1))) {
            const unsigned long long gv[1] = {g};
            unsigned nv[1];
            wave_control<DIM == 3 ? 6 : 3, 1, false, PRIORS>(&S, 1, states, prob, gv, &nv);
            g = (unsigned long long) nv[0];
            FUSED_FALLBACK_COUNT();
            break;
          }
          spins = 0;
        }
      }
    }
    rec_lds[lane] = (unsigned) g;
  }
  __syncthreads();
  PASS_TS(S.fc.epoch, 2);
#pragma unroll
  for (int i = 0; i < 12; ++i) v.T[i] = __int_as_float(__builtin_amdgcn_readfirstlane((int) rec_lds[i]));
#pragma unroll
  for (int i = 0; i < 12; ++i) v.Tprev[i] = __int_as_float(__builtin_amdgcn_readfirstlane((int) rec_lds[12 + i]));
  v.kexp = __builtin_amdgcn_readfirstlane((int) rec_lds[PUB_G_KEXP]);
  const unsigned fl = (unsigned) __builtin_amdgcn_readfirstlane((int) rec_lds[PUB_G_FLAGS]);
  v.stop   = (fl & PUB_FLAG_STOP) != 0;
  v.phase1 = (fl & PUB_FLAG_PHASE1) != 0;
  v.prior  = (fl & PUB_FLAG_PRIOR) != 0;
}

template <int DIM>
__device__ __forceinline__ void pass_view_init(const SliceDev& S, const CtlParams& C, const InitInline& inl, int prob, int nm,
                                               PassView& v, const InitBatch* bat = nullptr) {
  const SliceCtl& sc = C.slices[S.slice_idx];
  float X[12];
  if (bat) {
    const int lp = prob - C.prob0;
#pragma unroll
    for (int i = 0; i < 12; ++i) X[i] = bat->guess[lp][i];
  } else {
#pragma unroll
    for (int i = 0; i < 12; ++i) X[i] = inl.guess[i];
  }
  const int nm_of = sc.nm_global > 0 ? sc.nm_global : nm;
  v.kexp = slice_exponent(C, sc, prob, nm_of, X);
  float T[12];
  finder_transform_of(sc.Sinv, DIM, X, T);
#pragma unroll
  for (int i = 0; i < 12; ++i) v.T[i] = v.Tprev[i] = T[i];
  v.stop = v.phase1 = v.prior = false;
}
__device__ __forceinline__ void fused_init_tail(const CtlParams& C, const InitInline& inl, int prob, ProblemDev* __restrict__ probs,
                                                ProblemState* __restrict__ states, const InitBatch* bat, const PassView& v, int cue) {
  const int lane   = threadIdx.x & 63;
  const int lp     = prob - C.prob0;
  ProblemState* st = &states[prob];
  if (C.ctl_dev && blockIdx.x == 0) {
    const int* src = reinterpret_cast<const int*>(&C);
    int* dst       = reinterpret_cast<int*>(C.ctl_dev);
    for (int k = lane; k < (int) (sizeof(CtlParams) / sizeof(int)); k += 64) dst[k] = src[k];
  }
  static_assert(PUB_G_X == 32, "the record's X granules sit one half-wave above the state's");
  float x = 0.f;
#pragma unroll
  for (int i = 0; i < 12; ++i) {
    const float gi = bat ? bat->guess[lp][i] : inl.guess[i];
    x              = (lane & 31) == i ? gi : x;
  }
  float t = 0.f;
#pragma unroll
  for (int i = 0; i < 12; ++i) {
    const float ti = __int_as_float(__builtin_amdgcn_readfirstlane(__float_as_int(v.T[i])));
    t              = (lane == i || lane == 12 + i) ? ti : t;
  }
  if (lane < 12) {
    st->X[lane]          = x;
    st->Xprev[lane]      = x;
    st->Tf[cue][lane]     = t;
    st->Tfprev[cue][lane] = t;
  }
  if (lane == 0) {
    st->status   = SRRG2_FAIL;
    st->done     = 0;
    st->finished = 0;
    st->nstats   = 0;
    st->phase    = 0;
    st->w_count  = 0;
    st->npasses  = 0;
  }
  if (lane < SRRG2_MAX_SLICES) st->qmode[lane] = 1;
#pragma unroll
  for (int s = 0; s < SRRG2_MAX_SLICES; ++s) {
    if (s >= C.nslices) break;
    ProblemDev pd{0, 0};
    if (bat) {
      if (s == cue) pd = bat->pd[lp];
    } else {
      pd = inl.pd[s];
    }
    int* qc = C.slices[s].qcount;
    if (lane == s) {
      probs[(size_t) s * C.K + prob] = pd;
      st->ncorr[s] = 0;
      st->ninl[s]  = 0;
      st->kexp[s]  = s == cue ? v.kexp : 0;
      if (qc) qc[2 * prob] = qc[2 * prob + 1] = 0;
    }
  }
  if (!C.pub) return;
  unsigned gran = 0u;
  if (lane < 24) gran = __float_as_uint(t);
// ... 273 lines not shown
      if (FIRST) acc[hidx(a, b)] = __double_as_longlong(t); else acc[hidx(a, b)] += __double_as_longlong(t);
    }
    double t = FX_MAGIC;
#pragma unroll
    for (int r = 0; r < ROWS; ++r) t = __fma_rn(wj[r], (double) e[r], t);
    if (FIRST) acc[ACC_B + a] = __double_as_longlong(t); else acc[ACC_B + a] += __double_as_longlong(t);
  }
  if (D == 3) {
#pragma unroll
    for (int k = 0; k < ACC_CHI_IN; ++k) {
      bool used = false;
#pragma unroll
      for (int a = 0; a < D; ++a) {
#pragma unroll
        for (int b = a; b < D; ++b) used |= k == hidx(a, b);
        used |= k == ACC_B + a;
      }
      if (!used) { if (FIRST) acc[k] = FX_MAGIC_BITS; else acc[k] += FX_MAGIC_BITS; }
    }
  }
  return !ok ? SRRG2_FACTOR_SUPPRESSED : (kernelized ? SRRG2_FACTOR_KERNELIZED : SRRG2_FACTOR_INLIER);
}

template <int DIM, bool PLANE>
__device__ __forceinline__ void point_rows(const float* T, float kk, const float4 p, float qx, float qy, float qz,
                                           const float4 f, const float4 nf,
                                           float (&J)[PLANE ? 1 : DIM][DIM == 3 ? 6 : 3], float (&e)[PLANE ? 1 : DIM]) {
  constexpr int D    = DIM == 3 ? 6 : 3;
  constexpr int ROWS = PLANE ? 1 : DIM;
  if constexpr (DIM == 3) {
    float m[ROWS][3];
    if (PLANE) {
      e[0]    = (nf.x * (qx - f.x) + nf.y * (qy - f.y)) + nf.z * (qz - f.z);
      m[0][0] = (T[0] * nf.x + T[4] * nf.y) + T[8] * nf.z;
      m[0][1] = (T[1] * nf.x + T[5] * nf.y) + T[9] * nf.z;
      m[0][2] = (T[2] * nf.x + T[6] * nf.y) + T[10] * nf.z;
    } else {
      const float q[3]  = {qx, qy, qz};
      const float ff[3] = {f.x, f.y, f.z};
#pragma unroll
      for (int r = 0; r < ROWS; ++r) {
        e[r]    = q[r] - ff[r];
        m[r][0] = T[r * 4 + 0];
        m[r][1] = T[r * 4 + 1];
        m[r][2] = T[r * 4 + 2];
      }
    }
#pragma unroll
    for (int r = 0; r < ROWS; ++r) {
      J[r][0]     = m[r][0];
      J[r][1]     = m[r][1];
      J[r][2]     = m[r][2];
      J[r][D - 3] = kk * (p.y * m[r][2] - p.z * m[r][1]);
      J[r][D - 2] = kk * (p.z * m[r][0] - p.x * m[r][2]);
      J[r][D - 1] = kk * (p.x * m[r][1] - p.y * m[r][0]);
    }
  } else {
    float m[ROWS][2];
    if (PLANE) {
      e[0]    = nf.x * (qx - f.x) + nf.y * (qy - f.y);
      m[0][0] = T[0] * nf.x + T[4] * nf.y;
      m[0][1] = T[1] * nf.x + T[5] * nf.y;
    } else {
      const float q[2]  = {qx, qy};
      const float ff[2] = {f.x, f.y};
#pragma unroll
      for (int r = 0; r < ROWS; ++r) {
        e[r]    = q[r] - ff[r];
        m[r][0] = T[r * 4 + 0];
        m[r][1] = T[r * 4 + 1];
      }
    }
#pragma unroll
    for (int r = 0; r < ROWS; ++r) {
      J[r][0] = m[r][0];
      J[r][1] = m[r][1];
      J[r][2] = m[r][1] * p.x - m[r][0] * p.y;
    }
  }
}

}

template <int DIM, bool PLANE, int PPT, bool GATHER, int FUSED>
__device__ __forceinline__ void icp_step_fast_body(const SliceDev& S, const ProblemDev* __restrict__ probs,
                                                   ProblemState* __restrict__ states) {
  constexpr int D    = DIM == 3 ? 6 : 3;
  constexpr int ROWS = PLANE ? 1 : DIM;
  const int prob     = (FUSED ? blockIdx.x : blockIdx.y) + S.prob0;
  const int tile     = FUSED ? (int) blockIdx.y : (int) blockIdx.x;
  const ProblemState* st = &states[prob];
  PassView pv;
  if constexpr (!FUSED) {
    pass_view_legacy(S, st, pv);
    if (pv.stop) return;
  } else {
    PASS_TS(S.fc.epoch, 0);
    fused_control_if_due<DIM, FUSED == 2>(S, states, prob);
  }
  const ProblemDev pd = probs[prob];
  if (tile * (256 * PPT) >= pd.nm && (!FUSED || tile != 0)) return;
  float T[12], Tprev[12];
  double scale;
  int rk;
  if constexpr (!FUSED) {
    load_T(pv.T, T);
    load_T(pv.Tprev, Tprev);
    scale = dm::pow2(pv.kexp);
    rk    = (pv.phase1 && S.robust_kind != SRRG2_ROBUST_NONE) ? (int) SRRG2_ROBUST_CLAMP : S.robust_kind;
  }
  const float thr    = S.robust_thr;
  const float kk     = S.variable_kind == SRRG2_SE3_QUAT_RIGHT ? 2.f : 1.f;
  const GridDev& g   = S.grid;
  const float gfar   = g.gate2_ext;
  const int rfar     = g.rmax;
  const float gate_r = S.gate * 1.000001f;
  const bool ngate   = S.use_normal_gate != 0;
  const bool use_q   = !FUSED && S.queue != nullptr && st->qmode[S.slice_idx] != 0;
  const int lane     = threadIdx.x & 63;
  const int wid      = threadIdx.x >> 6;
  union FastWaveLds {
    CnlWave cnl;
    int coop[288];
  };
  __shared__ FastWaveLds fast_lds[4];
  int* const coop_lds_w = fast_lds[wid].coop;

  auto linearize = [&](auto first, long long (&acc)[ACC_N], bool valid, const float4 pk, const float4 fk, const float4 nk,
                       const float4 nmk, float qx, float qy, float qz, float best) {
    bool found = valid && __float_as_int(fk.w) != NO_MATCH && best <= g.gate2;
    if (ngate) {
      float dot;
      if constexpr (DIM == 3) {
        const float rx = (T[0] * nmk.x + T[1] * nmk.y) + T[2] * nmk.z;
        const float ry = (T[4] * nmk.x + T[5] * nmk.y) + T[6] * nmk.z;
        const float rz = (T[8] * nmk.x + T[9] * nmk.y) + T[10] * nmk.z;
        dot            = (nk.x * rx + nk.y * ry) + nk.z * rz;
      } else {
        const float rx = T[0] * nmk.x + T[1] * nmk.y;
        const float ry = T[4] * nmk.x + T[5] * nmk.y;
        dot            = nk.x * rx + nk.y * ry;
      }
      found = found && dot > S.normal_cos;
    }
    float J[ROWS][D], e[ROWS];
    point_rows<DIM, PLANE>(T, kk, pk, qx, qy, qz, fk, nk, J, e);
    (void) factor_accumulate_flat<D, ROWS, decltype(first)::value>(J, e, found, rk, thr, scale, acc);
  };

  long long acc[ACC_N];

  float4 p[PPT], pf[PPT], pnm[PPT], pn[PPT];
  float pm[PPT];
  int gi_[PPT];
  bool inr[PPT];
#pragma unroll
  for (int k = 0; k < PPT; ++k) {
    const int i = (tile * PPT + k) * 256 + (int) threadIdx.x;
    inr[k]      = i < pd.nm;
    gi_[k]      = pd.moff + (inr[k] ? i : 0);
    int ppos    = -1;
    p[k]        = S.mpts[gi_[k]];
    pm[k]       = S.prev_m[gi_[k]];
    pf[k]       = make_float4(0.f, 0.f, 0.f, __int_as_float(NO_MATCH));
    pn[k]       = make_float4(0.f, 0.f, 0.f, 0.f);
    pnm[k]      = make_float4(0.f, 0.f, 0.f, 0.f);
    if (GATHER) {
      ppos = S.prev_pos[gi_[k]];
    } else {
      pf[k] = S.prev_f[gi_[k]];
      if (PLANE || ngate) pn[k] = S.prev_n[gi_[k]];
    }
    if (ngate) pnm[k] = S.mnrm[gi_[k]];
    if (GATHER && ppos >= 0 && ppos < g.n) {
      pf[k] = g.pts[ppos];
      if (PLANE || ngate) pn[k] = g.nrm[ppos];
    }
  }
  if constexpr (FUSED) {
    pass_view_fused<DIM, FUSED == 2>(S, states, prob, pv);
    if (pv.stop || tile * (256 * PPT) >= pd.nm) return;
    load_T(pv.T, T);
    load_T(pv.Tprev, Tprev);
    scale = dm::pow2(pv.kexp);
    rk    = (pv.phase1 && S.robust_kind != SRRG2_ROBUST_NONE) ? (int) SRRG2_ROBUST_CLAMP : S.robust_kind;
  }

  float open_ball2[PPT];
  bool any_open = false;
  auto search_open = [&](float (&sbest)[PPT], int (&sidx)[PPT], float (&sexcl)[PPT], int (&spos)[PPT]) {
  #pragma unroll
    for (int k = 0; k < PPT; ++k) {
      sbest[k] = INFINITY; sexcl[k] = 0.f; sidx[k] = NO_MATCH; spos[k] = 0;
      const bool open = open_ball2[k] >= 0.f;
      if (!__ballot(open)) continue;
      float qx = 0.f, qy = 0.f, qz = 0.f;
      if (open) transform_point<DIM>(T, p[k], qx, qy, qz);
      if (g.list_R > 0 && __popcll(__ballot(open)) > 4) {
        unsigned long long skey;
        float sb2, sL;
        cnl_search<DIM, 1>(g, *g.lists, fast_lds[wid].cnl, lane, open, qx, qy, qz, open_ball2[k], gfar, skey, sb2, sL);
        if (open) {
          sbest[k] = key_best(skey);
          sidx[k]  = key_idx(skey);
          sexcl[k] = sqrtf(fminf(sb2, fminf(sL, g.gate2_ext))) * 0.99999f;
        }
        continue;
      }
      bool open_k = open;
      if constexpr (PPT == 1) {
        if (!(g.list_R > 0) && __popcll(__ballot(open)) > 4) {
          unsigned long long lkey = NO_KEY;
          float lb2 = INFINITY, lc2 = INFINITY;
          if (open)
            scan_radius1<DIM>(g, qx, qy, qz, cell_coord(qx, g.ox, g.inv_h), cell_coord(qy, g.oy, g.inv_h),
                              DIM == 3 ? cell_coord(qz, g.oz, g.inv_h) : 0, open_ball2[k], lkey, lb2, lc2);
          const float b2_1 = bound2_of(1, g.h);
          if (open && key_idx(lkey) != NO_MATCH && key_best(lkey) <= gfar && key_best(lkey) <= b2_1) {
            sbest[k] = key_best(lkey);
            sidx[k]  = key_idx(lkey);
            sexcl[k] = sqrtf(fminf(fminf(lb2, lc2), b2_1)) * 0.99999f;
            open_k   = false;
          }
        }
      }
      const int r2 = open_ball2[k] <= bound2_of(2, g.h) ? 2 : max(rfar, 3);
      unsigned long long near = __ballot(open_k && r2 == 2);
      while (near) {
        int src[4];
  #pragma unroll
        for (int t = 0; t < 4; ++t) {
          src[t] = near ? __ffsll((long long) near) - 1 : -1;
          near &= near - 1;
        }
        const int team = lane >> 4;
        const int mine = team == 0 ? src[0] : (team == 1 ? src[1] : (team == 2 ? src[2] : src[3]));
        const int from = mine >= 0 ? mine : lane;
        const float sqx = __shfl(qx, from), sqy = __shfl(qy, from), sqz = __shfl(qz, from), sball = __shfl(open_ball2[k], from);
        const int scx = cell_coord(sqx, g.ox, g.inv_h), scy = cell_coord(sqy, g.oy, g.inv_h);
        const int scz = DIM == 3 ? cell_coord(sqz, g.oz, g.inv_h) : 0;
        float wbest, wexcl2;
        int widx, wpos;
        coop_scan<DIM, 16>(g, lane, coop_lds_w, sqx, sqy, sqz, scx, scy, scz, mine >= 0 ? 2 : -1, sball, wbest, widx, wpos, wexcl2);
  #pragma unroll
        for (int t = 0; t < 4; ++t) {
          const float rb = __shfl(wbest, 16 * t), re = __shfl(wexcl2, 16 * t);
          const int ri = __shfl(widx, 16 * t), rp = __shfl(wpos, 16 * t);
          if (lane == src[t]) {
            sbest[k] = rb;
            sidx[k]  = ri;
            spos[k]  = rp;
            sexcl[k] = sqrtf(re) * 0.99999f;
          }
        }
      }
      unsigned long long todo = __ballot(open_k && r2 != 2);
      while (todo) {
        const int src = __ffsll((long long) todo) - 1;
        todo &= todo - 1;
        const float sqx = __shfl(qx, src), sqy = __shfl(qy, src), sqz = __shfl(qz, src);
        const int scx = cell_coord(sqx, g.ox, g.inv_h), scy = cell_coord(sqy, g.oy, g.inv_h);
        const int scz = DIM == 3 ? cell_coord(sqz, g.oz, g.inv_h) : 0;
        float wbest, wexcl2;
        int widx, wpos;
        coop_scan<DIM, 64>(g, lane, coop_lds_w, sqx, sqy, sqz, scx, scy, scz, __shfl(r2, src), __shfl(open_ball2[k], src),
                           wbest, widx, wpos, wexcl2);
        if (lane == src) {
          sbest[k] = wbest;
          sidx[k]  = widx;
          spos[k]  = wpos;
          sexcl[k] = sqrtf(wexcl2) * 0.99999f;
        }
      }
    }
  };
  constexpr bool defer = PPT == 1 && FUSED;
  float d_qx = 0.f, d_qy = 0.f, d_qz = 0.f, d_best = INFINITY;
  bool d_valid = false;
#pragma unroll
  for (int k = 0; k < PPT; ++k) {
    const bool active = inr[k] && finite3(p[k].x, p[k].y, p[k].z);
    float qx, qy, qz, px, py, pz;
    transform_point<DIM>(T, p[k], qx, qy, qz);
    transform_point<DIM>(Tprev, p[k], px, py, pz);
    const float ex = qx - px, ey = qy - py, ez = qz - pz;
    const float dl   = __builtin_amdgcn_sqrtf((ex * ex + ey * ey) + ez * ez);
    const bool hasp  = __float_as_int(pf[k].w) != NO_MATCH;
    unsigned long long k1 = NO_KEY;
    test_candidate<DIM>(pf[k], qx, qy, qz, true, k1);
    const float best = key_best(k1);
    const float d1   = __builtin_amdgcn_sqrtf(best);
    const float rhs  = pm[k] * 0.99999f;
    const bool ca   = hasp && (d1 * 1.00001f + dl * 1.00001f < rhs);
    const bool cc   = !hasp && pm[k] > 0.f && (gate_r * 1.00001f + dl * 1.00001f < rhs);
    const bool have = active && (ca || cc);
    const float excl = pm[k] * 0.9999999f - dl * 1.00001f;
    const float pad  = fminf(2.f * dl, PAD_CAP * g.h) + PAD_MIN * g.h;
    const float rr   = (d1 + pad) * 1.00001f;
    const float r2box = hasp ? fminf(rr * rr, gfar) : gfar;
    open_ball2[k]     = (active && !have) ? r2box : -1.f;
    any_open |= active && !have;
#ifdef SRRG2_PASS_TIMELINE
    if constexpr (FUSED) {
      if (active && !have && S.fc.epoch >= 0 && S.fc.epoch < 16 && blockIdx.x == 0) {
        unsigned long long* c = &g_pass_ts[((size_t) S.fc.epoch * 512 + 500) * 8];
        const float gap = (pm[k] - d1) / g.h;
        atomicAdd(&c[0], 1ull);
        if (!hasp) atomicAdd(&c[1], 1ull);
        else if (gap < 1e-4f) atomicAdd(&c[2], 1ull);
        else if (gap < 0.0202f) atomicAdd(&c[3], 1ull);
        else atomicAdd(&c[4], 1ull);
        if (dl > 1e-3f * g.h) atomicAdd(&c[5], 1ull);
        if (pm[k] <= 0.f) atomicAdd(&c[6], 1ull);
      }
    }
#endif
    if constexpr (defer) {
      d_qx = qx; d_qy = qy; d_qz = qz; d_best = best; d_valid = have && ca;
    } else if (k == 0) {
      linearize(std::true_type{}, acc, have && ca, p[k], pf[k], pn[k], pnm[k], qx, qy, qz, best);
    } else {
      linearize(std::false_type{}, acc, have && ca, p[k], pf[k], pn[k], pnm[k], qx, qy, qz, best);
    }
    if (have) S.prev_m[gi_[k]] = excl;
  }
  if constexpr (defer) {
    {
      if (__any(any_open)) {
        float sbest[PPT], sexcl[PPT];
        int sidx[PPT], spos[PPT];
        search_open(sbest, sidx, sexcl, spos);
        const bool open = open_ball2[0] >= 0.f;
        const bool same = open && sidx[0] != NO_MATCH && sidx[0] == __float_as_int(pf[0].w);
        if (open && !same) {
          pf[0] = make_float4(0.f, 0.f, 0.f, __int_as_float(NO_MATCH));
          pn[0] = make_float4(0.f, 0.f, 0.f, 0.f);
          if (sidx[0] != NO_MATCH) {
            spos[0] = g.pos_of[sidx[0]];
            pf[0]   = g.pts[spos[0]];
            if (PLANE || ngate) pn[0] = g.nrm[spos[0]];
          }
          S.prev_pos[gi_[0]] = sidx[0] != NO_MATCH ? spos[0] : -1;
          if (!GATHER) {
            S.prev_f[gi_[0]] = pf[0];
            if (PLANE || ngate) S.prev_n[gi_[0]] = pn[0];
          }
        }
        if (open) {
          S.prev_m[gi_[0]] = sexcl[0];
          d_best  = sbest[0];
          d_valid = true;
        }
      }
      linearize(std::true_type{}, acc, d_valid, p[0], pf[0], pn[0], pnm[0], d_qx, d_qy, d_qz, d_best);
      block_reduce_store_biased<4>(acc, S.partials, prob, tile, PPT);
      if constexpr (FUSED) PASS_TS(S.fc.epoch, 3);
      return;
    }
  }
  if (use_q) {
#pragma unroll
    for (int k = 0; k < PPT; ++k) {
      const bool open               = open_ball2[k] >= 0.f;
      const unsigned long long need = __ballot(open);
      if (!need) continue;
      const int r2 = open_ball2[k] <= bound2_of(2, g.h) ? 2 : max(rfar, 3);
      const unsigned long long need_near = __ballot(open && r2 == 2);
      const unsigned long long need_far  = need & ~need_near;
      int base_near = 0, base_far = 0;
      if (lane == 0) {
        if (need_near) base_near = atomicAdd(&S.qcount[2 * prob], __popcll(need_near));
        if (need_far) base_far = atomicAdd(&S.qcount[2 * prob + 1], __popcll(need_far));
      }
      base_near = __shfl(base_near, 0);
      base_far  = __shfl(base_far, 0);
      if (open) {
        const unsigned long long below = (1ull << lane) - 1ull;
        QEntry q;
        q.i = (tile * PPT + k) * 256 + (int) threadIdx.x;
        q.r2 = r2; q.best = INFINITY; q.bidx = NO_MATCH; q.bpos = 0;
        transform_point<DIM>(T, p[k], q.qx, q.qy, q.qz);
        q.ball2 = open_ball2[k]; q.pad_ = 0;
        QEntry* qbase = reinterpret_cast<QEntry*>(S.queue) + pd.moff;
        if (r2 == 2)
          qbase[base_near + __popcll(need_near & below)] = q;
        else
          qbase[pd.nm - 1 - (base_far + __popcll(need_far & below))] = q;
      }
    }
  }
  block_reduce_store_biased<4, 1>(acc, S.partials, prob, tile, PPT);
  if (use_q || !__any(any_open)) {
    block_reduce_store_biased<4, 2>(acc, S.partials, prob, tile, PPT);
    if constexpr (FUSED) PASS_TS(S.fc.epoch, 3);
    return;
  }

  float sbest[PPT], sexcl[PPT];
  int sidx[PPT], spos[PPT];
  search_open(sbest, sidx, sexcl, spos);
  long long acc2[ACC_N];
#pragma unroll
  for (int k = 0; k < PPT; ++k) {
    const bool open = open_ball2[k] >= 0.f;
    float4 fk = make_float4(0.f, 0.f, 0.f, __int_as_float(NO_MATCH)), nk = make_float4(0.f, 0.f, 0.f, 0.f);
    bool same = false;
    if constexpr (PPT == 1) same = open && sidx[k] != NO_MATCH && sidx[k] == __float_as_int(pf[k].w);
    if (same) {
      fk = pf[k];
      nk = pn[k];
    } else if (open && sidx[k] != NO_MATCH) {
      spos[k] = g.pos_of[sidx[k]];
      fk      = g.pts[spos[k]];
      if (PLANE || ngate) nk = g.nrm[spos[k]];
    }
    float qx, qy, qz;
    transform_point<DIM>(T, p[k], qx, qy, qz);
    if (k == 0)
      linearize(std::true_type{}, acc2, open, p[k], fk, nk, pnm[k], qx, qy, qz, sbest[k]);
    else
      linearize(std::false_type{}, acc2, open, p[k], fk, nk, pnm[k], qx, qy, qz, sbest[k]);
    if (open) {
      S.prev_m[gi_[k]] = sexcl[k];
      if (!same) {
        S.prev_pos[gi_[k]] = sidx[k] != NO_MATCH ? spos[k] : -1;
        if (!GATHER) {
          S.prev_f[gi_[k]] = fk;
          if (PLANE || ngate) S.prev_n[gi_[k]] = nk;
        }
      }
    }
  }
  block_reduce_store_biased<1>(acc2, S.partials, prob, tile, PPT);
  if constexpr (FUSED) PASS_TS_ANY(S.fc.epoch, 4);
  block_reduce_store_biased<4, 2>(acc, S.partials, prob, tile, PPT);
  if constexpr (FUSED) PASS_TS(S.fc.epoch, 3);
}

template <int DIM, bool PLANE, int PPT, bool GATHER, int FUSED>
__global__ __launch_bounds__(256) void k_icp_step_fast(SliceDev S, const ProblemDev* __restrict__ probs,
                                                       ProblemState* __restrict__ states) {
  icp_step_fast_body<DIM, PLANE, PPT, GATHER, FUSED>(S, probs, states);
}
template <int DIM, bool PLANE, int PPT, bool GATHER>
__global__ __launch_bounds__(256) void k_icp_step_fast_pairs(SliceDev S, const GridDev* __restrict__ grids,
                                                             const ProblemDev* __restrict__ probs, ProblemState* __restrict__ states) {
  S.grid = grids[blockIdx.y + S.prob0];
  icp_step_fast_body<DIM, PLANE, PPT, GATHER, 0>(S, probs, states);
}
template <int DIM, bool PLANE, int TEAM, int FUSED>
__device__ __forceinline__ void cnl_pass_body(const SliceDev& S, const GridLists& GL, const ProblemDev* __restrict__ probs,
                                              ProblemState* __restrict__ states, const CtlParams* Ci = nullptr,
                                              const InitInline* inl = nullptr, const InitBatch* bat = nullptr) {
  constexpr int NW  = 4;
  constexpr int PPB = NW * 64 / TEAM;
  const int prob    = (FUSED ? blockIdx.x : blockIdx.y) + S.prob0;
  PassView pv;
  if constexpr (!FUSED) {
    pass_view_legacy(S, &states[prob], pv);
    if (pv.stop) return;
  } else if constexpr (FUSED != 3) {
    PASS_TS(S.fc.epoch, 0);
    fused_control_if_due<DIM, FUSED == 2>(S, states, prob);
  }
  ProblemDev pd;
  if constexpr (FUSED == 3) {
    if (bat)
      pd = bat->pd[prob - Ci->prob0];
    else
      pd = inl->pd[S.slice_idx];
  } else {
    pd = probs[prob];
  }
  const int tile      = FUSED ? blockIdx.y : blockIdx.x;
  const bool tail_wg = FUSED == 3 && tile == (int) gridDim.y - 1;
  if (tile * PPB >= pd.nm && (!FUSED || (FUSED == 3 ? !tail_wg : tile != 0))) return;
  float T[12], Tprev[12];
  double scale;
  int rk;
  bool use_prior;
  if constexpr (!FUSED) {
    load_T(pv.T, T);
    load_T(pv.Tprev, Tprev);
    scale     = dm::pow2(pv.kexp);
    rk        = (pv.phase1 && S.robust_kind != SRRG2_ROBUST_NONE) ? (int) SRRG2_ROBUST_CLAMP : S.robust_kind;
    use_prior = pv.prior;
  } else {
    use_prior = S.fc.prior != 0;
  }
  const float thr    = S.robust_thr;
  const float kk     = S.variable_kind == SRRG2_SE3_QUAT_RIGHT ? 2.f : 1.f;
  const GridDev& g   = S.grid;
  const float gfar = use_prior ? g.gate2_ext : g.gate2;

  __shared__ CnlWave wlds[NW];

  const int i        = tile * PPB + (int) threadIdx.x / TEAM;
  const int lane     = threadIdx.x & 63;
  const int wid      = threadIdx.x >> 6;
  const bool leader  = (threadIdx.x & (TEAM - 1)) == 0;
  const bool inrange = i < pd.nm;
  const int gi       = pd.moff + (inrange ? i : 0);
  float4 p           = make_float4(0.f, 0.f, 0.f, 0.f);
  float4 pf          = make_float4(0.f, 0.f, 0.f, __int_as_float(NO_MATCH));
  float4 pn          = make_float4(0.f, 0.f, 0.f, 0.f);
  float4 pnm         = make_float4(0.f, 0.f, 0.f, 0.f);
  float pm           = 0.f;
  if (inrange) {
    p = S.mpts[gi];
    if (use_prior) {
      pm = S.prev_m[gi];
      if (S.use_normal_gate) pnm = S.mnrm[gi];
      if (S.gather_prev) {
        const int ppos = S.prev_pos[gi];
        if (ppos >= 0 && ppos < S.grid.n) {
          pf = S.grid.pts[ppos];
          if (PLANE || S.use_normal_gate) pn = S.grid.nrm[ppos];
        }
      } else {
// ... 1323 lines not shown
    }
    part[c][a] = v;
    __syncthreads();
    long long* pz = const_cast<long long*>(sc.partials) + ((size_t) C.zero_parity * C.K + prob) * PARTIAL_SLOTS * ACC_N;
#pragma unroll
    for (int q = 0; q < PARTIAL_SLOTS / 8; ++q) pz[(size_t) (c + 8 * q) * ACC_N + a] = 0;
    if (threadIdx.x < ACC_N) {
      long long t = 0;
#pragma unroll
      for (int k = 0; k < 8; ++k) t += part[k][threadIdx.x];
      sums[s][threadIdx.x]   = t;
      scaled[s][threadIdx.x] = (double) t * dm::pow2(-st->kexp[s]);
    }
    __syncthreads();
  }
  if (threadIdx.x != 0) return;
  if (C.variable_kind == SRRG2_SE2_RIGHT)
    control_body<3>(C, st, stats, prob, sums, scaled);
  else
    control_body<6>(C, st, stats, prob, sums, scaled);
}

__global__ __launch_bounds__(256) void k_icp_control(CtlParams C, ProblemState* __restrict__ states,
                                                     srrg2_iteration_stats* __restrict__ stats) {
  const int prob   = blockIdx.x + C.prob0;
  ProblemState* st = &states[prob];
  const PrePartials pre = prefetch_partials(C, prob);
  __shared__ ProblemState sst;
  state_to_lds(&sst, st);
  __syncthreads();
  if (sst.done || sst.finished) {
    if (C.pub && threadIdx.x < 64) {
      pub_publish_state(C, &sst, prob, threadIdx.x, (unsigned) C.epoch);
      pub_write_epoch(C.pub_epoch, prob, threadIdx.x, (unsigned) C.epoch);
    }
    return;
  }
  icp_control_block(C, &sst, stats, prob, pre);
  __syncthreads();
  state_from_lds(st, &sst);
  if (C.pub && threadIdx.x < 64) {
    pub_publish_state(C, &sst, prob, threadIdx.x, (unsigned) C.epoch);
    pub_write_epoch(C.pub_epoch, prob, threadIdx.x, (unsigned) C.epoch);
  }
}

__device__ void icp_post_one(const CtlParams& C, ProblemState* st, const srrg2_iteration_stats* stats, int prob) {
  if (st->nstats == 0) {
    st->status   = SRRG2_FAIL;
    st->finished = 1;
    return;
  }
  int last = st->nstats < C.max_stats ? st->nstats - 1 : C.max_stats - 1;
  if (stats[(size_t) prob * C.max_stats + last].num_inliers < C.params.min_num_inliers) {
    st->status   = SRRG2_NOT_ENOUGH_INLIERS;
    st->finished = 1;
    return;
  }
  if (C.params.enable_inlier_only_runs) {
    st->phase = 1;
    st->done  = 0;
  }
}

__global__ __launch_bounds__(64) void k_icp_post(CtlParams C, ProblemState* __restrict__ states,
                                                 const srrg2_iteration_stats* __restrict__ stats) {
  const int prob = blockIdx.x + C.prob0;
  if (threadIdx.x == 0) icp_post_one(C, &states[prob], stats, prob);
  if (!C.pub) return;
  for (int s = 0; s < C.nslices; ++s) {
    const SliceCtl& sc = C.slices[s];
    if (sc.kind == SRRG2_SLICE_PRIOR || !sc.partials) continue;
    for (int buf = 0; buf < 3; ++buf) {
      long long* p = const_cast<long long*>(sc.partials) + ((size_t) buf * C.K + prob) * PARTIAL_SLOTS * ACC_N;
      for (int k = threadIdx.x; k < PARTIAL_SLOTS * ACC_N; k += 64) p[k] = 0;
    }
  }
  __syncthreads();
  pub_publish_state(C, &states[prob], prob, threadIdx.x, (unsigned) C.epoch);
  pub_write_epoch(C.pub_epoch, prob, threadIdx.x, (unsigned) C.epoch);
}

__device__ void icp_finalize_block(const CtlParams& C, ProblemState* st, const srrg2_iteration_stats* stats,
                                   ProblemOut* outs_host, srrg2_iteration_stats* stats_host, int prob, bool with_post) {
  if (with_post) {
    if (threadIdx.x == 0) icp_post_one(C, st, stats, prob);
    __syncthreads();
  }
  {
    const int n       = min(st->nstats, C.max_stats) * (int) (sizeof(srrg2_iteration_stats) / sizeof(int));
    const int* src    = reinterpret_cast<const int*>(stats + (size_t) prob * C.max_stats);
    int* dst          = reinterpret_cast<int*>(stats_host + (size_t) prob * C.max_stats);
    for (int k = threadIdx.x; k < n; k += blockDim.x) dst[k] = src[k];
  }
  __threadfence_system();
  __syncthreads();
  if (threadIdx.x != 0) return;
  if (!st->finished) {
    if (C.params.keep_only_inlier_correspondences) {
      for (int s = 0; s < C.nslices; ++s)
        if (C.slices[s].kind != SRRG2_SLICE_PRIOR) st->ncorr[s] = st->ninl[s];
    }
    if (C.variable_kind == SRRG2_SE2_RIGHT)
      dm::se2_fix_transform(st->X);
    else
      dm::se3_fix_transform(st->X);
    st->status = SRRG2_SUCCESS;
  }
  ProblemOut* o = &outs_host[prob];
  for (int i = 0; i < 12; ++i) o->X[i] = st->X[i];
  o->status = st->status;
  o->nstats = st->nstats;
  for (int s = 0; s < SRRG2_MAX_SLICES; ++s) o->ncorr[s] = st->ncorr[s];
  {
    const int DD = C.variable_kind == SRRG2_SE2_RIGHT ? 9 : 36;
    for (int i = 0; i < 36; ++i) o->H[i] = (i < DD && st->nstats > 0) ? (float) st->last_H[i] : 0.f;
  }
  __threadfence_system();
  *reinterpret_cast<volatile int*>(&o->seq) = C.seq;
}

__global__ __launch_bounds__(64) void k_icp_finalize(CtlParams C, ProblemState* __restrict__ states,
                                                     const srrg2_iteration_stats* __restrict__ stats,
                                                     ProblemOut* __restrict__ outs_host,
                                                     srrg2_iteration_stats* __restrict__ stats_host, int with_post) {
  icp_finalize_block(C, &states[blockIdx.x + C.prob0], stats, outs_host, stats_host, blockIdx.x + C.prob0, with_post != 0);
}

__global__ __launch_bounds__(256) void k_icp_control_final(CtlParams C, ProblemState* __restrict__ states,
                                                           srrg2_iteration_stats* __restrict__ stats,
                                                           ProblemOut* __restrict__ outs_host,
                                                           srrg2_iteration_stats* __restrict__ stats_host, int with_post) {
  const int prob = blockIdx.x + C.prob0;
  const PrePartials pre = prefetch_partials(C, prob);
  __shared__ ProblemState sst;
  state_to_lds(&sst, &states[prob]);
  __syncthreads();
  if (!sst.done && !sst.finished) icp_control_block(C, &sst, stats, prob, pre);
  __threadfence();
  __syncthreads();
  icp_finalize_block(C, &sst, stats, outs_host, stats_host, prob, with_post != 0);
  __syncthreads();
  state_from_lds(&states[prob], &sst);
}

namespace srrg2amd {
template <int D, int MAXS, bool PRIORS>
__device__ __forceinline__ void final_wave_body(const CtlParams& C, const SliceDev* __restrict__ Sv, int ns,
                                                ProblemState* __restrict__ states, srrg2_iteration_stats* __restrict__ stats,
                                                ProblemOut* __restrict__ outs_host, srrg2_iteration_stats* __restrict__ stats_host,
                                                int with_post) {
  const FusedCtl& F = Sv[0].fc;
  const int prob = blockIdx.x + C.prob0;
  const int lane = threadIdx.x & 63;
  ProblemState* st = &states[prob];
  unsigned long long g[MAXS];
  bool stale = false;
#pragma unroll
  for (int z = 0; z < MAXS; ++z) {
    g[z] = 0ull;
    if (z < ns) {
      g[z]  = pub_load(F.pub + ((size_t) prob * SRRG2_MAX_SLICES + Sv[z].slice_idx) * PUB_SLICE_GRANULES + lane);
      stale = stale || (unsigned) (g[z] >> 32) != (unsigned) F.epoch;
    }
  }
  int ncorr_l = 0;
  if (lane < SRRG2_MAX_SLICES) ncorr_l = st->ncorr[lane];
  FinalRegs fin;
  fin.applied = false;
  if (__any(stale)) wave_control<D, MAXS, true, PRIORS, true>(Sv, ns, states, prob, g, nullptr, &fin);
#pragma unroll
  for (int z = 0; z < MAXS; ++z) {
    if (z >= ns) break;
    if (const long long* base = C.slices[Sv[z].slice_idx].partials) {
#pragma unroll 1
      for (int buf = 0; buf < 3; ++buf) {
        long long* p = const_cast<long long*>(base) + ((size_t) buf * C.K + prob) * PARTIAL_SLOTS * ACC_N;
#pragma unroll
        for (int q = 0; q < PARTIAL_SLOTS * ACC_N / 64; ++q) p[q * 64 + lane] = 0;
      }
    }
  }
  if (!fin.applied || !fin.stats_written) {
    __threadfence();
    icp_finalize_block(C, st, stats, outs_host, stats_host, prob, with_post != 0);
    return;
  }
  int status    = SRRG2_SUCCESS;
  bool finished = false;
  if (with_post && fin.num_in < C.params.min_num_inliers) {
    status   = SRRG2_NOT_ENOUGH_INLIERS;
    finished = true;
  }
  float Xa[12];
#pragma unroll
  for (int i = 0; i < 12; ++i) Xa[i] = rl_f(fin.Xl, i);
  const bool keep_inl = !finished && C.params.keep_only_inlier_correspondences;
  if (!finished) {
    if constexpr (D == 3)
      dm::se2_fix_transform(Xa);
    else
      dm::se3_fix_transform(Xa);
  }
  float xl = Xa[0];
#pragma unroll
  for (int i = 1; i < 12; ++i) xl = lane == i ? Xa[i] : xl;
  int ncorr_s = ncorr_l;
#pragma unroll
  for (int z = 0; z < MAXS; ++z)
    if (z < ns && lane == Sv[z].slice_idx) ncorr_s = keep_inl ? fin.ni[z] : fin.nc[z];
  if (lane < 12) st->X[lane] = xl;
  if (lane < SRRG2_MAX_SLICES) st->ncorr[lane] = ncorr_s;
  if (lane == 0) {
    st->status = status;
    if (finished) st->finished = 1;
  }
  constexpr int W_STATUS = 12, W_NSTATS = 13, W_NCORR = 14, W_H = W_NCORR + SRRG2_MAX_SLICES, W_SEQ = W_H + 36;
  static_assert(offsetof(ProblemOut, status) == 4 * W_STATUS && offsetof(ProblemOut, ncorr) == 4 * W_NCORR &&
                  offsetof(ProblemOut, H) == 4 * W_H && offsetof(ProblemOut, seq) == 4 * W_SEQ && W_SEQ < 64,
                "one word of the record per lane");
  const int ncorr_w = __shfl(ncorr_s, (lane - W_NCORR) & 63);
  const float h_w   = (float) __shfl(fin.Hl, (lane - W_H) & 63);
  int word = __float_as_int(xl);
  if (lane == W_STATUS) word = status;
  if (lane == W_NSTATS) word = fin.nstats;
  if (lane >= W_NCORR && lane < W_H) word = ncorr_w;
  if (lane >= W_H && lane < W_SEQ) word = lane - W_H < D * D ? __float_as_int(h_w) : __float_as_int(0.f);
  if (lane < W_SEQ) reinterpret_cast<int*>(&outs_host[prob])[lane] = word;
  {
    const int nrec  = min(fin.nstats, C.max_stats);
    const int n     = nrec * 8;
    const int* src  = reinterpret_cast<const int*>(stats + (size_t) prob * C.max_stats);
    int* dst        = reinterpret_cast<int*>(stats_host + (size_t) prob * C.max_stats);
    const int lastw = __shfl(fin.sw, lane & 7);
    for (int k = lane; k < n; k += 64) dst[k] = (k >> 3) == fin.nstats - 1 ? lastw : src[k];
  }
  __threadfence_system();
  if (lane == 0) *reinterpret_cast<volatile int*>(&outs_host[prob].seq) = C.seq;
}
template <int D, bool PRIORS>
__global__ __launch_bounds__(64) void k_icp_final_wave(CtlParams C, SliceDev S, ProblemState* __restrict__ states,
                                                        srrg2_iteration_stats* __restrict__ stats,
                                                        ProblemOut* __restrict__ outs_host,
                                                        srrg2_iteration_stats* __restrict__ stats_host, int with_post) {
  final_wave_body<D, 1, PRIORS>(C, &S, 1, states, stats, outs_host, stats_host, with_post);
}
template <bool PRIORS>
__global__ __launch_bounds__(64) void k_icp_final_wave_pack(SlicePack P, int ns, ProblemState* __restrict__ states,
                                                             srrg2_iteration_stats* __restrict__ stats,
                                                             ProblemOut* __restrict__ outs_host,
                                                             srrg2_iteration_stats* __restrict__ stats_host, int with_post) {
  final_wave_body<6, 4, PRIORS>(*P.s[0].fc.ctl, P.s, ns, states, stats, outs_host, stats_host, with_post);
}
}

template <int DIM, bool PLANE>
__global__ __launch_bounds__(512) void k_icp_small(SliceDev S, CtlParams C, const ProblemDev* __restrict__ probs,
                                                   ProblemState* __restrict__ states, srrg2_iteration_stats* __restrict__ stats,
                                                   ProblemOut* __restrict__ outs_host,
                                                   srrg2_iteration_stats* __restrict__ stats_host) {
  constexpr int NW = 8;
  constexpr int D  = DIM == 3 ? 6 : 3;
  const int prob   = blockIdx.x;
  __shared__ ProblemState sst;
  __shared__ long long sums[SRRG2_MAX_SLICES][ACC_N];
  __shared__ double scaled[SRRG2_MAX_SLICES][ACC_N];
  state_to_lds(&sst, &states[prob]);
  __syncthreads();
  const ProblemDev pd = probs[prob];
  const int ntiles    = (pd.nm + NW * 64 - 1) / (NW * 64);
  const int nrun      = C.params.enable_inlier_only_runs ? 2 : 1;
  for (int run = 0; run < nrun; ++run) {
    for (int it = 0; it < C.params.max_iterations; ++it) {
      if (sst.done || sst.finished) break;
      if (threadIdx.x < ACC_N) sums[S.slice_idx][threadIdx.x] = 0;
      __syncthreads();
      for (int tile = 0; tile < ntiles; ++tile) {
        StepView sv;
        step_view_of_state(S, &sst, sv);
        icp_step_body<DIM, PLANE, NW>(S, pd, sv, prob, tile, ntiles, C.K, sums[S.slice_idx]);
        __syncthreads();
      }
      if (threadIdx.x < ACC_N)
        scaled[S.slice_idx][threadIdx.x] = (double) sums[S.slice_idx][threadIdx.x] * dm::pow2(-sst.kexp[S.slice_idx]);
      __syncthreads();
      if (threadIdx.x == 0) control_body<D>(C, &sst, stats, prob, sums, scaled);
      __syncthreads();
    }
    if (run == 0 && nrun == 2) {
      if (threadIdx.x == 0) icp_post_one(C, &sst, stats, prob);
      __syncthreads();
    }
  }
  __threadfence();
  __syncthreads();
  icp_finalize_block(C, &sst, stats, outs_host, stats_host, prob, nrun == 1);
  __syncthreads();
  state_from_lds(&states[prob], &sst);
}
template <int DIM, bool PLANE>
__global__ __launch_bounds__(512) void k_icp_small_pairs(SliceDev S, const GridDev* __restrict__ grids, CtlParams C,
                                                         const ProblemDev* __restrict__ probs, ProblemState* __restrict__ states,
                                                         srrg2_iteration_stats* __restrict__ stats, ProblemOut* __restrict__ outs_host,
                                                         srrg2_iteration_stats* __restrict__ stats_host) {
  S.grid = grids[blockIdx.x];
  constexpr int NW = 8;
  constexpr int D  = DIM == 3 ? 6 : 3;
  const int prob   = blockIdx.x;
  __shared__ ProblemState sst;
  __shared__ long long sums[SRRG2_MAX_SLICES][ACC_N];
  __shared__ double scaled[SRRG2_MAX_SLICES][ACC_N];
  state_to_lds(&sst, &states[prob]);
  __syncthreads();
  const ProblemDev pd = probs[prob];
  const int ntiles    = (pd.nm + NW * 64 - 1) / (NW * 64);
  const int nrun      = C.params.enable_inlier_only_runs ? 2 : 1;
  for (int run = 0; run < nrun; ++run) {
    for (int it = 0; it < C.params.max_iterations; ++it) {
      if (sst.done || sst.finished) break;
      if (threadIdx.x < ACC_N) sums[S.slice_idx][threadIdx.x] = 0;
      __syncthreads();
      for (int tile = 0; tile < ntiles; ++tile) {
        StepView sv;
        step_view_of_state(S, &sst, sv);
        icp_step_body<DIM, PLANE, NW>(S, pd, sv, prob, tile, ntiles, C.K, sums[S.slice_idx]);
        __syncthreads();
      }
      if (threadIdx.x < ACC_N)
        scaled[S.slice_idx][threadIdx.x] = (double) sums[S.slice_idx][threadIdx.x] * dm::pow2(-sst.kexp[S.slice_idx]);
      __syncthreads();
      if (threadIdx.x == 0) control_body<D>(C, &sst, stats, prob, sums, scaled);
      __syncthreads();
    }
    if (run == 0 && nrun == 2) {
      if (threadIdx.x == 0) icp_post_one(C, &sst, stats, prob);
// ... 241 lines not shown
    return;
  }
  if (P.s[0].fc.pub) {
    with_value<true, false>(P.s[0].fc.prior_mask != 0, [&](auto PRIORS) {
      hipLaunchKernelGGL(k_proj_zbuf_fz<PRIORS()>, grid, dim3(256), 0, s, P, nslices, states);
    });
    hipLaunchKernelGGL(k_icp_step_proj_fused<true>, grid, dim3(256), 0, s, P, nslices, states);
    return;
  }
  hipLaunchKernelGGL(k_proj_zbuf, grid, dim3(256), 0, s, P.s[0], P.probs[0], states);
  hipLaunchKernelGGL(k_icp_step_proj_fused<false>, grid, dim3(256), 0, s, P, nslices, states);
}

void launch_proj_records(const SliceDev& S0, const SliceDev& S, const ProblemDev* probs0, const ProblemDev* probs,
                         ProblemState* states, int K, int max_nm, bool rebuild, hipStream_t s) {
  if (K <= 0 || max_nm <= 0 || !S0.zbuf) return;
  dim3 grid(icp_step_blocks(max_nm), K);
  if (rebuild) {
    (void) hipMemsetAsync(S0.zbuf, 0xff, (size_t) K * S0.rows * S0.cols * sizeof(unsigned long long), s);
    hipLaunchKernelGGL(k_proj_zbuf_last, grid, dim3(256), 0, s, S0, probs0, states);
  }
  hipLaunchKernelGGL(k_proj_records, grid, dim3(256), 0, s, S0, S, probs, (const ProblemState*) states);
}

bool make_init_inline(const CtlParams& C, const ProblemDev* probs_host, const float* guesses_host, int tsize, InitInline* inl) {
  *inl = InitInline{};
  if (C.K != 1) return false;
  inl->use = 1;
  for (int i = 0; i < 12; ++i) inl->guess[i] = i < tsize ? guesses_host[i] : 0.f;
  for (int sl = 0; sl < C.nslices && sl < SRRG2_MAX_SLICES; ++sl) inl->pd[sl] = probs_host[sl];
  return true;
}
void launch_icp_init(const CtlParams& C, const ProblemDev* probs_host, ProblemDev* probs, ProblemState* states,
                     const float* guesses_host, int tsize, hipStream_t s, bool pairs) {
  InitInline inl{};
  (void) make_init_inline(C, probs_host, guesses_host, tsize, &inl);
  const dim3 grid(ctl_problems(C));
  if (pairs)
    hipLaunchKernelGGL(k_icp_init_pairs, grid, dim3(64), 0, s, C, probs_host, probs, states, guesses_host, tsize, inl);
  else
    hipLaunchKernelGGL(k_icp_init, grid, dim3(64), 0, s, C, probs_host, probs, states, guesses_host, tsize, inl);
}
void launch_icp_control(const CtlParams& C, ProblemState* states, srrg2_iteration_stats* stats, hipStream_t s) {
  hipLaunchKernelGGL(k_icp_control, dim3(ctl_problems(C)), dim3(256), 0, s, C, states, stats);
}
void launch_icp_small(int dim, bool plane, const SliceDev& S, const CtlParams& C, const ProblemDev* probs, ProblemState* states,
                      srrg2_iteration_stats* stats, ProblemOut* outs_host, srrg2_iteration_stats* stats_host, hipStream_t s) {
  if (C.K <= 0) return;
  with_dim_plane(dim, plane, [&](auto D, auto P) {
    hipLaunchKernelGGL((k_icp_small<D(), P()>), dim3(C.K), dim3(512), 0, s, S, C, probs, states, stats, outs_host, stats_host);
  });
}

void launch_icp_step_pairs(int dim, bool plane, const SliceDev& S, const GridDev* grids, const ProblemDev* probs,
                           ProblemState* states, int K, int max_nm, hipStream_t s) {
  if (K <= 0 || max_nm <= 0) return;
  const dim3 grid(icp_step_blocks(max_nm), K);
  with_dim_plane(dim, plane, [&](auto D, auto P) {
    hipLaunchKernelGGL((k_icp_step_pairs<D(), P()>), grid, dim3(256), 0, s, S, grids, probs, states);
  });
}
void launch_icp_step_fast_pairs(int dim, bool plane, const SliceDev& S, const GridDev* grids, const ProblemDev* probs,
                                ProblemState* states, int K, int max_nm, int ppt, bool gather, hipStream_t s) {
  if (K <= 0 || max_nm <= 0) return;
  with_value<2, 1>(ppt >= 2, [&](auto PPT) {
    const dim3 grid((max_nm + 256 * PPT() - 1) / (256 * PPT()), K);
    with_value<true, false>(gather, [&](auto GATHER) {
      with_dim_plane(dim, plane, [&](auto D, auto P) {
        hipLaunchKernelGGL((k_icp_step_fast_pairs<D(), P(), PPT(), GATHER()>), grid, dim3(256), 0, s, S, grids, probs, states);
      });
    });
  });
}
void launch_icp_small_pairs(int dim, bool plane, const SliceDev& S, const GridDev* grids, const CtlParams& C, const ProblemDev* probs,
                            ProblemState* states, srrg2_iteration_stats* stats, ProblemOut* outs_host,
                            srrg2_iteration_stats* stats_host, hipStream_t s) {
  if (C.K <= 0) return;
  with_dim_plane(dim, plane, [&](auto D, auto P) {
    hipLaunchKernelGGL((k_icp_small_pairs<D(), P()>), dim3(C.K), dim3(512), 0, s, S, grids, C, probs, states, stats, outs_host,
                       stats_host);
  });
}

void launch_icp_final_wave(const CtlParams& C, const SliceDev& S, ProblemState* states, srrg2_iteration_stats* stats,
                           ProblemOut* outs_host, srrg2_iteration_stats* stats_host, bool with_post, hipStream_t s) {
  const dim3 grid(ctl_problems(C));
  with_value<3, 6>(C.variable_kind == SRRG2_SE2_RIGHT, [&](auto D) {
    with_value<true, false>(S.fc.prior_mask != 0, [&](auto PRIORS) {
      hipLaunchKernelGGL((k_icp_final_wave<D(), PRIORS()>), grid, dim3(64), 0, s, C, S, states, stats, outs_host, stats_host,
                         with_post ? 1 : 0);
    });
  });
}
void launch_icp_final_wave_pack(const SliceDev* slices, const ProblemDev* const* probs, int nslices, ProblemState* states,
                                srrg2_iteration_stats* stats, ProblemOut* outs_host, srrg2_iteration_stats* stats_host,
                                bool with_post, hipStream_t s) {
  if (nslices <= 0 || nslices > 4) return;
  const SlicePack P = make_slice_pack(slices, probs, nslices);
  with_value<true, false>(P.s[0].fc.prior_mask != 0, [&](auto PRIORS) {
    hipLaunchKernelGGL(k_icp_final_wave_pack<PRIORS()>, dim3(1), dim3(64), 0, s, P, nslices, states, stats, outs_host, stats_host,
                       with_post ? 1 : 0);
  });
}
void launch_icp_control_final(const CtlParams& C, ProblemState* states, srrg2_iteration_stats* stats, ProblemOut* outs_host,
                               srrg2_iteration_stats* stats_host, bool with_post, hipStream_t s) {
  hipLaunchKernelGGL(k_icp_control_final, dim3(ctl_problems(C)), dim3(256), 0, s, C, states, stats, outs_host, stats_host,
                     with_post ? 1 : 0);
}
void launch_icp_post(const CtlParams& C, ProblemState* states, const srrg2_iteration_stats* stats, hipStream_t s) {
  hipLaunchKernelGGL(k_icp_post, dim3(ctl_problems(C)), dim3(64), 0, s, C, states, stats);
}
void launch_icp_finalize(const CtlParams& C, ProblemState* states, const srrg2_iteration_stats* stats,
                         ProblemOut* outs_host, srrg2_iteration_stats* stats_host, bool with_post, hipStream_t s) {
  hipLaunchKernelGGL(k_icp_finalize, dim3(ctl_problems(C)), dim3(64), 0, s, C, states, stats, outs_host, stats_host,
                     with_post ? 1 : 0);
}

}
```

Measured before the change: 58600 iterations/s.

## Run all remaining ICP iterations in one persistent kernel with grid-wide sync

Adds a persistent 'run fast' kernel that carries out all remaining ICP iterations in a single launch. Workgroups signal arrivals through sharded atomic counters, and a designated wave runs the control step and publishes the next pose. The goal is to remove per-iteration kernel launches and host round trips for the single-problem NN-gated case. A host spin-wait handles completion, and there is a bail path back to the normal per-iteration launches if co-residency or polling fails. This adds complexity and the risk of spin stalls or a deadlock if not all workgroups are resident.

Result: no change. 58990 iterations/s (median of 4 runs) (+0.7%).

```diff
diff --git a/__graft_entry__.py b/__graft_entry__.py
--- a/__graft_entry__.py
+++ b/__graft_entry__.py
@@ -11,7 +11,7 @@
     env = dict(os.environ)
     env.setdefault("HIPCC", "/opt/rocm/bin/hipcc")
     subprocess.check_call(["make", "-j", str(min(8, os.cpu_count() or 1)), "-C", os.path.join(ROOT, "srrg2_slam_interfaces_amd", "csrc"),
-                           "ARCH=gfx950", "all", "stall"], env=env)
+                           "ARCH=gfx950", "all", "stall", "runbail"], env=env)
     subprocess.check_call(["make", "-C", os.path.join(ROOT, "oracle")], env=env)
     subprocess.check_call(["make", "-C", os.path.join(ROOT, "tests", "cpp")], env=env)
     import srrg2_slam_interfaces_amd
diff --git a/include/srrg2_slam_amd.h b/include/srrg2_slam_amd.h
--- a/include/srrg2_slam_amd.h
+++ b/include/srrg2_slam_amd.h
@@ -469,6 +469,8 @@
 #define SRRG2_PATH_PROLOGUE_IN_PASS 8
 #define SRRG2_PATH_ONE_WORKGROUP 16
 #define SRRG2_PATH_PRIORS_FUSED 32
+#define SRRG2_PATH_RUN_FAST 64
+#define SRRG2_PATH_RUN_FAST_BAILED 128
 int srrg2_aligner_last_compute_path(srrg2_aligner_h h, int32_t* flags_out);
 
 #ifndef SRRG2_DESCRIPTOR_BYTES
diff --git a/srrg2_slam_interfaces_amd/_abi.py b/srrg2_slam_interfaces_amd/_abi.py
--- a/srrg2_slam_interfaces_amd/_abi.py
+++ b/srrg2_slam_interfaces_amd/_abi.py
@@ -227,3 +227,4 @@
     return c
 
 PATH_FUSED_CONTROL, PATH_ALL_PASSES_FUSED, PATH_FINAL_WAVE, PATH_PROLOGUE_IN_PASS, PATH_ONE_WORKGROUP, PATH_PRIORS_FUSED = 1, 2, 4, 8, 16, 32
+PATH_RUN_FAST, PATH_RUN_FAST_BAILED = 64, 128
diff --git a/srrg2_slam_interfaces_amd/csrc/aligner_host.hip b/srrg2_slam_interfaces_amd/csrc/aligner_host.hip
--- a/srrg2_slam_interfaces_amd/csrc/aligner_host.hip
+++ b/srrg2_slam_interfaces_amd/csrc/aligner_host.hip
@@ -138,6 +138,9 @@
   DevBuf<unsigned long long> pub;
   DevBuf<unsigned> pub_epoch;
   DevBuf<CtlParams> ctl_dev;
+  DevBuf<unsigned> run_sync;
+  bool run_sync_dirty = true;
+  int run_blocks_per_cu[2][2] = {{-1, -1}, {-1, -1}};
   DevBuf<char> staging;
   DevBuf<float4> pair_raw, pair_nrm_raw, pair_sorted, pair_nrm_sorted;
   DevBuf<int> pair_cell_start, pair_cursor, pair_scan_sums, pair_pos_of;
@@ -807,7 +810,7 @@
   C.max_stats     = slots;
   C.seq           = ++a->seq;
   if (C.seq <= 0) C.seq = a->seq = 1;
-  for (int k = 0; k < K; ++k) a->outs_host[k].seq = 0;
+  for (int k = 0; k < K; ++k) a->outs_host[k].seq = a->outs_host[k].run = 0;
   const srrg2_aligner_tuning& tn = a->tuning;
   C.probe_it      = tn.queue_probe_iteration;
   if (a->params.max_iterations <= C.probe_it + 3 || K > 4) C.probe_it = -1;
@@ -1247,9 +1250,88 @@
       srrg2amd::launch_icp_control(Ch[h], a->states.p, a->stats.p, hstream[h]);
     }
   };
+  bool run_fast_ok = fuse && fused_all && !fuse_proj && K == 1 && !split && !pairs && ncue_all == 1 && prior_mask == 0 &&
+                     tn.fused_control == 3 && !a->profile && !sdev[first_cue].queue && fast_ppt_of(1) == 1 && !fast_gather &&
+                     nm_max_cue > 0 && a->slices[first_cue]->cfg.finder == SRRG2_FINDER_NN_GATED;
+  if (run_fast_ok) {
+    const bool plane = a->slices[first_cue]->cfg.kind == SRRG2_SLICE_P2PLANE;
+    int& per_cu      = a->run_blocks_per_cu[a->dim == 3 ? 1 : 0][plane ? 1 : 0];
+    if (per_cu < 0) per_cu = srrg2amd::icp_run_fast_blocks_per_cu(a->dim, plane);
+    run_fast_ok = 2LL * ((nm_max_cue + 255) / 256) <= (long long) per_cu * a->cu_count;
+    if (run_fast_ok && !a->run_sync.p) {
+      if ((rc = a->run_sync.reserve((size_t) RUN_SYNC_WORDS))) return rc;
+      a->run_sync_dirty = true;
+    }
+  }
+  bool run_fast_used = false, run_fast_bailed = false;
   auto run_phase = [&](int slot0, bool last_phase) -> int {
     for (int it = 0; it < a->params.max_iterations; ++it) {
       if (!probed && slot0 == 0 && probe_it >= 0 && it == probe_it + 2) read_probe();
+      if (run_fast_ok && last_phase && !run_fast_bailed && fast_at(slot0, it) && a->params.max_iterations - it <= RUN_MAX_ITERS) {
+        Slice* s     = a->slices[first_cue];
+        const int n  = a->params.max_iterations - it;
+        SliceDev sd  = sdev[first_cue];
+        sd.prob0     = 0;
+        sd.fc.ctl    = a->ctl_dev.p;
+        sd.fc.epoch  = epoch;
+        sd.partials  = slot_buffer(s, pround);
+        sd.fc.prev_partials = slot_buffer(s, pround + 2);
+        sd.fc.zero_partials = slot_buffer(s, pround + 1);
+        sd.fc.prior         = (slot0 > 0 || it > 0) ? 1 : 0;
+        if (a->run_sync_dirty) {
+          HIP_TRY(hipMemsetAsync(a->run_sync.p, 0, (size_t) RUN_SYNC_WORDS * sizeof(unsigned), a->stream));
+          a->run_sync_dirty = false;
+        }
+        const RunArgs R{a->run_sync.p, &a->outs_host[0].run, s->partials.p, n, pround, C.seq};
+        srrg2amd::launch_icp_run_fast(a->dim, s->cfg.kind == SRRG2_SLICE_P2PLANE, sd, R, a->probs.p + (size_t) first_cue * K,
+                                      a->states.p, a->stats.p, a->outs_host, a->stats_host, !a->params.enable_inlier_only_runs,
+                                      nm_max_cue, a->stream);
+        HIP_TRY(hipGetLastError());
+        run_fast_used = true;
+        volatile int* flag = &a->outs_host[0].seq;
+        volatile int* word = &a->outs_host[0].run;
+        const unsigned tag = (unsigned) C.seq & 0xffffffu;
+        int code = 0, spins = 0;
+        auto look = [&]() {
+          if (*flag == C.seq) return true;
+          const unsigned w = (unsigned) *word;
+          if ((w >> 8) == tag && (w & 0xffu)) {
+            code = (int) (w & 0xffu);
+            return true;
+          }
+          return false;
+        };
+        while (!look())
+          if ((++spins & 4095) == 0 && hipStreamQuery(a->stream) != hipErrorNotReady) {
+            (void) look();
+            break;
+          }
+        if (code == 0) {
+          epoch += n;
+          pround += n;
+          final_launched = true;
+          return 0;
+        }
+        run_fast_bailed   = true;
+        a->run_sync_dirty = true;
+        HIP_TRY(hipStreamSynchronize(a->stream));
+        unsigned lost = 0;
+        HIP_TRY(hipMemcpy(&lost, a->run_sync.p + RUN_SYNC_LOST, sizeof(lost), hipMemcpyDeviceToHost));
+        if (lost || code == RUN_WORD_LOST || code > n)
+          return fail(SRRG2_E_STATE, "internal: a workgroup of the run kernel never saw its control step");
+        if (code < n) {
+          epoch += code;
+          pround += code;
+          it += code - 1;
+          continue;
+        }
+        epoch += n - 1;
+        pround += n - 1;
+        control(a->params.max_iterations - 1, last_phase, 0);
+        ++epoch;
+        ++pround;
+        return 0;
+      }
       if (!proj_group.empty()) {
         SliceDev pack[4];
         const ProblemDev* pp[4];
@@ -1471,7 +1553,8 @@
   a->pairs_computed = pairs;
   a->last_path = (fuse ? SRRG2_PATH_FUSED_CONTROL : 0) | (fuse && fused_all ? SRRG2_PATH_ALL_PASSES_FUSED : 0) |
                  (fuse && final_launched && !small ? SRRG2_PATH_FINAL_WAVE : 0) | (fold_init ? SRRG2_PATH_PROLOGUE_IN_PASS : 0) |
-                 (small ? SRRG2_PATH_ONE_WORKGROUP : 0) | (fuse && prior_mask ? SRRG2_PATH_PRIORS_FUSED : 0);
+                 (small ? SRRG2_PATH_ONE_WORKGROUP : 0) | (fuse && prior_mask ? SRRG2_PATH_PRIORS_FUSED : 0) |
+                 (run_fast_used ? SRRG2_PATH_RUN_FAST : 0) | (run_fast_bailed ? SRRG2_PATH_RUN_FAST_BAILED : 0);
   if (fuse && final_launched && first_cue >= 0 && !small) {
     for (int si = 0; si < nslices; ++si) {
       if (si != first_cue && !(fuse_proj && std::find(proj_group.begin(), proj_group.end(), si) != proj_group.end())) continue;
@@ -1704,7 +1787,7 @@
     delete s;
   }
   a->probs.release(); a->states.release(); a->outs.release(); a->stats.release(); a->guesses.release();
-  a->pub.release(); a->pub_epoch.release(); a->ctl_dev.release();
+  a->pub.release(); a->pub_epoch.release(); a->ctl_dev.release(); a->run_sync.release();
   a->staging.release();
   a->pair_raw.release(); a->pair_nrm_raw.release(); a->pair_sorted.release(); a->pair_nrm_sorted.release();
   a->pair_cell_start.release(); a->pair_cursor.release(); a->pair_scan_sums.release(); a->pair_pos_of.release();
diff --git a/srrg2_slam_interfaces_amd/csrc/device_types.h b/srrg2_slam_interfaces_amd/csrc/device_types.h
--- a/srrg2_slam_interfaces_amd/csrc/device_types.h
+++ b/srrg2_slam_interfaces_amd/csrc/device_types.h
@@ -76,6 +76,22 @@
   int prior;
   int prior_mask;
   int nslices;
+};
+
+#define RUN_SYNC_STRIDE 32
+#define RUN_SYNC_SHARDS 8
+#define RUN_SYNC_BAIL (8 * RUN_SYNC_STRIDE)
+#define RUN_SYNC_LOST (9 * RUN_SYNC_STRIDE)
+#define RUN_SYNC_WORDS (10 * RUN_SYNC_STRIDE)
+#define RUN_WORD_LOST 0xff
+#define RUN_MAX_ITERS 200
+struct RunArgs {
+  unsigned* sync;
+  volatile int* word_host;
+  long long* partials;
+  int n_iters;
+  int round0;
+  int seq;
 };
 
 struct SliceDev {
@@ -151,6 +167,7 @@
   int ncorr[SRRG2_MAX_SLICES];
   float H[36];
   int seq;
+  int run;
 };
 
 struct SliceCtl {
diff --git a/srrg2_slam_interfaces_amd/csrc/kernels.h b/srrg2_slam_interfaces_amd/csrc/kernels.h
--- a/srrg2_slam_interfaces_amd/csrc/kernels.h
+++ b/srrg2_slam_interfaces_amd/csrc/kernels.h
@@ -73,6 +73,10 @@
                              float4* out_pts, float4* out_nrm, int* pos_of, hipStream_t s);
 void launch_icp_final_wave(const CtlParams& C, const SliceDev& S, ProblemState* states, srrg2_iteration_stats* stats,
                            ProblemOut* outs_host, srrg2_iteration_stats* stats_host, bool with_post, hipStream_t s);
+int icp_run_fast_blocks_per_cu(int dim, bool plane);
+void launch_icp_run_fast(int dim, bool plane, const SliceDev& S, const RunArgs& R, const ProblemDev* probs,
+                         ProblemState* states, srrg2_iteration_stats* stats, ProblemOut* outs_host,
+                         srrg2_iteration_stats* stats_host, bool with_post, int max_nm, hipStream_t s);
 void launch_icp_control_final(const CtlParams& C, ProblemState* states, srrg2_iteration_stats* stats, ProblemOut* outs_host,
                                srrg2_iteration_stats* stats_host, bool with_post, hipStream_t s);
 void launch_icp_post(const CtlParams& C, ProblemState* states, const srrg2_iteration_stats* stats, hipStream_t s);
diff --git a/srrg2_slam_interfaces_amd/csrc/kernels.hip b/srrg2_slam_interfaces_amd/csrc/kernels.hip
--- a/srrg2_slam_interfaces_amd/csrc/kernels.hip
+++ b/srrg2_slam_interfaces_amd/csrc/kernels.hip
@@ -1932,15 +1932,21 @@
   int nc[4], ni[4];
 };
 
-template <int D, int MAXS, bool PUBLISH = true, bool PRIORS = false, bool FINAL = false>
+struct RunIter {
+  int epoch;
+  long long* partials;
+  long long* prev_partials;
+  long long* zero_partials;
+};
+template <int D, int MAXS, bool PUBLISH = true, bool PRIORS = false, bool FINAL = false, bool RUN = false>
 __device__ __forceinline__ void wave_control(const SliceDev* __restrict__ Sv, int ns, ProblemState* __restrict__ states, int prob,
                                              const unsigned long long (&g)[MAXS], unsigned (*out)[MAXS] = nullptr,
-                                             FinalRegs* fin = nullptr) {
+                                             FinalRegs* fin = nullptr, const RunIter* rit = nullptr) {
   if constexpr (FINAL) fin->applied = false;
   const FusedCtl& F  = Sv[0].fc;
   const int lane     = threadIdx.x & 63;
   ProblemState* st   = &states[prob];
-  const unsigned epoch = (unsigned) F.epoch;
+  const unsigned epoch = (unsigned) (RUN ? rit->epoch : F.epoch);
   constexpr int TS   = D == 3 ? 9 : 12;
   int pw[SRRG2_MAX_SLICES];
 #pragma unroll
@@ -1954,9 +1960,14 @@
   for (int z = 0; z < MAXS; ++z) {
     v[z] = 0;
     if (z < ns) {
-      const long long* p = Sv[z].fc.prev_partials + (size_t) prob * PARTIAL_SLOTS * ACC_N;
-#pragma unroll
-      for (int q = 0; q < PARTIAL_SLOTS * ACC_N / 64; ++q) v[z] += p[q * 64 + lane];
+      const long long* p = (RUN ? rit->prev_partials : Sv[z].fc.prev_partials) + (size_t) prob * PARTIAL_SLOTS * ACC_N;
+#pragma unroll
+      for (int q = 0; q < PARTIAL_SLOTS * ACC_N / 64; ++q) {
+        if constexpr (RUN)
+          v[z] += __hip_atomic_load(p + q * 64 + lane, __ATOMIC_RELAXED, __HIP_MEMORY_SCOPE_AGENT);
+        else
+          v[z] += p[q * 64 + lane];
+      }
     }
   }
   const int w          = (int) (unsigned) g[0];
@@ -2069,9 +2080,14 @@
     if (z >= ns) break;
     v[z] += __shfl_xor(v[z], 32);
     if constexpr (PUBLISH) {
-      long long* p = Sv[z].fc.zero_partials + (size_t) prob * PARTIAL_SLOTS * ACC_N;
-#pragma unroll
-      for (int q = 0; q < PARTIAL_SLOTS * ACC_N / 64; ++q) p[q * 64 + lane] = 0;
+      long long* p = (RUN ? rit->zero_partials : Sv[z].fc.zero_partials) + (size_t) prob * PARTIAL_SLOTS * ACC_N;
+#pragma unroll
+      for (int q = 0; q < PARTIAL_SLOTS * ACC_N / 64; ++q) {
+        if constexpr (RUN && !FINAL)
+          __hip_atomic_store(p + q * 64 + lane, 0ll, __ATOMIC_RELAXED, __HIP_MEMORY_SCOPE_AGENT);
+        else
+          p[q * 64 + lane] = 0;
+      }
     }
     const double scaled = (double) v[z] * dm::pow2(-kexp[z]);
     const int nc = (int) rl_ll(v[z], ACC_N_CORR), n_in = (int) rl_ll(v[z], ACC_N_IN), n_out = (int) rl_ll(v[z], ACC_N_OUT);
@@ -2275,6 +2291,7 @@
   }
   if (PUBLISH && stop && lane == 0) st->done = 1;
   const unsigned x_up = __float_as_uint(__shfl(Xl, (lane - PUB_G_X) & 63));
+  if constexpr (RUN && !FINAL) asm volatile("s_waitcnt vmcnt(0)" ::: "memory");
 #pragma unroll
   for (int z = 0; z < MAXS; ++z) {
     if (z >= ns) break;
@@ -2367,14 +2384,27 @@
 #define FUSED_FALLBACK_COUNT() do { } while (0)
 #endif
 
-template <int DIM, bool PRIORS = false>
-__device__ __forceinline__ void fused_control_if_due(const SliceDev& S, ProblemState* __restrict__ states, int prob) {
+__device__ __forceinline__ void pass_view_of_record(const unsigned* rec_lds, PassView& v) {
+#pragma unroll
+  for (int i = 0; i < 12; ++i) v.T[i] = __int_as_float(__builtin_amdgcn_readfirstlane((int) rec_lds[i]));
+#pragma unroll
+  for (int i = 0; i < 12; ++i) v.Tprev[i] = __int_as_float(__builtin_amdgcn_readfirstlane((int) rec_lds[12 + i]));
+  v.kexp = __builtin_amdgcn_readfirstlane((int) rec_lds[PUB_G_KEXP]);
+  const unsigned fl = (unsigned) __builtin_amdgcn_readfirstlane((int) rec_lds[PUB_G_FLAGS]);
+  v.stop   = (fl & PUB_FLAG_STOP) != 0;
+  v.phase1 = (fl & PUB_FLAG_PHASE1) != 0;
+  v.prior  = (fl & PUB_FLAG_PRIOR) != 0;
+}
+
+template <int DIM, bool PRIORS = false, bool RUN = false>
+__device__ __forceinline__ void fused_control_if_due(const SliceDev& S, ProblemState* __restrict__ states, int prob,
+                                                     const RunIter* rit = nullptr) {
   if (blockIdx.y != 0 || threadIdx.x >= 64) return;
   const unsigned long long g[1] = {
     pub_load(S.fc.pub + ((size_t) prob * SRRG2_MAX_SLICES + S.slice_idx) * PUB_SLICE_GRANULES + (threadIdx.x & 63))};
-  if (!__all((unsigned) (g[0] >> 32) == (unsigned) S.fc.epoch)) {
+  if (!__all((unsigned) (g[0] >> 32) == (unsigned) (RUN ? rit->epoch : S.fc.epoch))) {
     FUSED_STALL();
-    wave_control<DIM == 3 ? 6 : 3, 1, true, PRIORS>(&S, 1, states, prob, g);
+    wave_control<DIM == 3 ? 6 : 3, 1, true, PRIORS, false, RUN>(&S, 1, states, prob, g, nullptr, nullptr, rit);
   }
   PASS_TS(S.fc.epoch, 1);
 }
@@ -2415,15 +2445,73 @@
   }
   __syncthreads();
   PASS_TS(S.fc.epoch, 2);
-#pragma unroll
-  for (int i = 0; i < 12; ++i) v.T[i] = __int_as_float(__builtin_amdgcn_readfirstlane((int) rec_lds[i]));
-#pragma unroll
-  for (int i = 0; i < 12; ++i) v.Tprev[i] = __int_as_float(__builtin_amdgcn_readfirstlane((int) rec_lds[12 + i]));
-  v.kexp = __builtin_amdgcn_readfirstlane((int) rec_lds[PUB_G_KEXP]);
-  const unsigned fl = (unsigned) __builtin_amdgcn_readfirstlane((int) rec_lds[PUB_G_FLAGS]);
-  v.stop   = (fl & PUB_FLAG_STOP) != 0;
-  v.phase1 = (fl & PUB_FLAG_PHASE1) != 0;
-  v.prior  = (fl & PUB_FLAG_PRIOR) != 0;
+  pass_view_of_record(rec_lds, v);
+}
+
+#ifdef SRRG2_RUN_BAIL
+#define SRRG2_RUN_ARRIVE_POLLS 0
+#elif !defined(SRRG2_RUN_ARRIVE_POLLS)
+#define SRRG2_RUN_ARRIVE_POLLS 4096
+#endif
+#ifndef SRRG2_RUN_RECORD_POLLS
+#define SRRG2_RUN_RECORD_POLLS (1 << 16)
+#endif
+
+__device__ __forceinline__ bool run_wait_arrivals(const unsigned* sync, unsigned target) {
+  const int lane = threadIdx.x & 63;
+#pragma unroll 1
+  for (int spins = 0; spins < SRRG2_RUN_ARRIVE_POLLS; ++spins) {
+    unsigned n = 0;
+    if (lane < RUN_SYNC_SHARDS) n = __hip_atomic_load(sync + lane * RUN_SYNC_STRIDE, __ATOMIC_RELAXED, __HIP_MEMORY_SCOPE_AGENT);
+    n += __shfl_xor(n, 1);
+    n += __shfl_xor(n, 2);
+    n += __shfl_xor(n, 4);
+    if ((unsigned) __builtin_amdgcn_readfirstlane((int) n) >= target) return true;
+    __builtin_amdgcn_s_sleep(1);
+  }
+  return false;
+}
+__device__ __forceinline__ void run_bail(const RunArgs& R, int seq, int passes) {
+  if ((threadIdx.x & 63) == 0) {
+    __hip_atomic_store(R.sync + RUN_SYNC_BAIL, (unsigned) passes, __ATOMIC_RELAXED, __HIP_MEMORY_SCOPE_AGENT);
+    __threadfence_system();
+    *R.word_host = (int) (((unsigned) seq << 8) | (unsigned) passes);
+  }
+}
+template <int DIM>
+__device__ __forceinline__ bool run_view(const SliceDev& S, const RunArgs& R, int seq, int prob, int epoch, PassView& v) {
+  __shared__ unsigned run_rec_lds[PUB_SLICE_GRANULES + 1];
+  const int lane = threadIdx.x & 63;
+  if (threadIdx.x < 64) {
+    const unsigned long long* rec = S.fc.pub + ((size_t) prob * SRRG2_MAX_SLICES + S.slice_idx) * PUB_SLICE_GRANULES + lane;
+    const unsigned* ep = S.fc.pub_epoch + ((size_t) prob * PUB_EPOCH_REPLICAS + (blockIdx.y & (PUB_EPOCH_REPLICAS - 1))) * PUB_EPOCH_STRIDE;
+    unsigned long long g = 0ull;
+    bool ok = false;
+#pragma unroll 1
+    for (int spins = 0;; ++spins) {
+      if ((int) __hip_atomic_load(ep, __ATOMIC_RELAXED, __HIP_MEMORY_SCOPE_AGENT) >= epoch) {
+        g  = pub_load(rec);
+        ok = __all((unsigned) (g >> 32) == (unsigned) epoch);
+        if (ok) break;
+      }
+      if (__hip_atomic_load(R.sync + RUN_SYNC_BAIL, __ATOMIC_RELAXED, __HIP_MEMORY_SCOPE_AGENT) != 0u) break;
+      if (spins >= SRRG2_RUN_RECORD_POLLS) {
+        if (lane == 0) {
+          __hip_atomic_store(R.sync + RUN_SYNC_LOST, 1u, __ATOMIC_RELAXED, __HIP_MEMORY_SCOPE_AGENT);
+          __threadfence_system();
+          *R.word_host = (int) (((unsigned) seq << 8) | (unsigned) RUN_WORD_LOST);
+        }
+        break;
+      }
+      __builtin_amdgcn_s_sleep(4);
+    }
+    run_rec_lds[lane] = (unsigned) g;
+    if (lane == 0) run_rec_lds[PUB_SLICE_GRANULES] = ok ? 1u : 0u;
+  }
+  __syncthreads();
+  if (!run_rec_lds[PUB_SLICE_GRANULES]) return false;
+  pass_view_of_record(run_rec_lds, v);
+  return true;
 }
 
 template <int DIM>
@@ -2863,11 +2951,88 @@
 
 }
 
-template <int DIM, bool PLANE, int PPT, bool GATHER, int FUSED>
-__device__ __forceinline__ void icp_step_fast_body(const SliceDev& S, const ProblemDev* __restrict__ probs,
-                                                   ProblemState* __restrict__ states) {
+namespace srrg2amd {
+template <int D, int MAXS, bool PRIORS, bool RUN = false>
+__device__ __forceinline__ void final_wave_body(const CtlParams& C, const SliceDev* __restrict__ Sv, int ns,
+                                                ProblemState* __restrict__ states, srrg2_iteration_stats* __restrict__ stats,
+                                                ProblemOut* __restrict__ outs_host, srrg2_iteration_stats* __restrict__ stats_host,
+                                                int with_post, const RunIter* rit = nullptr);
+}
+struct RunCtlArgs {
+  FusedCtl fc;
+  float Sinv[12];
+  int slice_idx;
+  int variable_kind;
+};
+template <class T>
+__device__ __forceinline__ T wave_uniform_of(const T& x) {
+  static_assert(sizeof(T) % 4 == 0, "whole words");
+  int w[sizeof(T) / 4];
+  __builtin_memcpy(w, &x, sizeof(T));
+#pragma unroll
+  for (size_t i = 0; i < sizeof(T) / 4; ++i) w[i] = __builtin_amdgcn_readfirstlane(w[i]);
+  T r;
+  __builtin_memcpy(&r, w, sizeof(T));
+  return r;
+}
+__device__ __forceinline__ void run_slice_of(const RunCtlArgs& a, SliceDev& Sl) {
+  Sl.fc            = a.fc;
+  Sl.slice_idx     = a.slice_idx;
+  Sl.variable_kind = a.variable_kind;
+#pragma unroll
+  for (int i = 0; i < 12; ++i) Sl.Sinv[i] = a.Sinv[i];
+}
+template <int DIM>
+__device__ __attribute__((noinline)) void run_control_step(RunCtlArgs a_in, ProblemState* states_in, int prob_in, RunIter rit_in) {
+  const RunCtlArgs a = wave_uniform_of(a_in);
+  const RunIter rit  = wave_uniform_of(rit_in);
+  ProblemState* states = wave_uniform_of(states_in);
+  const int prob       = __builtin_amdgcn_readfirstlane(prob_in);
+  SliceDev Sl;
+  run_slice_of(a, Sl);
+  fused_control_if_due<DIM, false, true>(Sl, states, prob, &rit);
+}
+struct RunFinalArgs {
+  ProblemState* states;
+  srrg2_iteration_stats* stats;
+  ProblemOut* outs_host;
+  srrg2_iteration_stats* stats_host;
+  int with_post;
+  int pad_;
+};
+template <int D>
+__device__ __attribute__((noinline)) void run_final_step(RunCtlArgs a_in, RunFinalArgs f_in, RunIter rit_in) {
+  const RunCtlArgs a   = wave_uniform_of(a_in);
+  const RunFinalArgs f = wave_uniform_of(f_in);
+  const RunIter rit    = wave_uniform_of(rit_in);
+  SliceDev Sl;
+  run_slice_of(a, Sl);
+  srrg2amd::final_wave_body<D, 1, false, true>(*a.fc.ctl, &Sl, 1, f.states, f.stats, f.outs_host, f.stats_host, f.with_post, &rit);
+}
+struct RunCtx {
+  const RunArgs& R;
+  srrg2_iteration_stats* stats;
+  ProblemOut* outs_host;
+  srrg2_iteration_stats* stats_host;
+  int with_post;
+};
+template <int DIM, bool PLANE, int PPT, bool GATHER, int FUSED, bool RUN = false>
+__device__ __forceinline__ void icp_step_fast_body(const SliceDev& S_in, const ProblemDev* __restrict__ probs,
+                                                   ProblemState* __restrict__ states, const RunCtx* rx = nullptr) {
+  static_assert(!RUN || (PPT == 1 && !GATHER && FUSED == 1), "the run kernel: one point per thread, fused control steps");
   constexpr int D    = DIM == 3 ? 6 : 3;
   constexpr int ROWS = PLANE ? 1 : DIM;
+  const SliceDev& S = S_in;
+  RunIter rit{S.fc.epoch, S.partials, S.fc.prev_partials, S.fc.zero_partials};
+  auto run_ctl_args = [&]() {
+    RunCtlArgs a;
+    a.fc            = S.fc;
+    a.slice_idx     = S.slice_idx;
+    a.variable_kind = S.variable_kind;
+#pragma unroll
+    for (int i = 0; i < 12; ++i) a.Sinv[i] = S.Sinv[i];
+    return a;
+  };
   const int prob     = (FUSED ? blockIdx.x : blockIdx.y) + S.prob0;
   const int tile     = FUSED ? (int) blockIdx.y : (int) blockIdx.x;
   const ProblemState* st = &states[prob];
@@ -2877,7 +3042,11 @@
     if (pv.stop) return;
   } else {
     PASS_TS(S.fc.epoch, 0);
-    fused_control_if_due<DIM, FUSED == 2>(S, states, prob);
+    if constexpr (RUN) {
+      if (blockIdx.y == 0 && threadIdx.x < 64) run_control_step<DIM>(run_ctl_args(), states, prob, rit);
+    } else {
+      fused_control_if_due<DIM, FUSED == 2>(S, states, prob);
+    }
   }
   const ProblemDev pd = probs[prob];
   if (tile * (256 * PPT) >= pd.nm && (!FUSED || tile != 0)) return;
@@ -2958,8 +3127,41 @@
       if (PLANE || ngate) pn[k] = g.nrm[ppos];
     }
   }
+#pragma unroll 1
+  for (int ri = 0;; ++ri) {
   if constexpr (FUSED) {
-    pass_view_fused<DIM, FUSED == 2>(S, states, prob, pv);
+    bool designated = false;
+    if constexpr (RUN) designated = tile == 0 && threadIdx.x < 64;
+    if (RUN && ri > 0) {
+      if constexpr (RUN) {
+        if (designated) {
+          const int ntiles = max((pd.nm + 255) / 256, 1);
+          if (run_wait_arrivals(rx->R.sync, (unsigned) (ntiles * ri)))
+            run_control_step<DIM>(run_ctl_args(), states, prob, rit);
+          else
+            run_bail(rx->R, rx->R.seq, ri);
+        }
+        if (!run_view<DIM>(S, rx->R, rx->R.seq, prob, rit.epoch, pv)) return;
+      }
+    } else {
+      pass_view_fused<DIM, FUSED == 2>(S, states, prob, pv);
+    }
+    if constexpr (RUN) {
+      if (pv.stop) {
+        if (designated) {
+          if (lane < RUN_SYNC_SHARDS)
+            __hip_atomic_store(rx->R.sync + lane * RUN_SYNC_STRIDE, 0u, __ATOMIC_RELAXED, __HIP_MEMORY_SCOPE_AGENT);
+          const int round_l        = rx->R.round0 + rx->R.n_iters - 1;
+          long long* const base    = rx->R.partials;
+          const size_t set_stride  = (size_t) PARTIAL_SLOTS * ACC_N;
+          rit.epoch                = S.fc.epoch + rx->R.n_iters;
+          rit.prev_partials        = base + (size_t) (round_l % 3) * set_stride;
+          rit.zero_partials        = base + (size_t) ((round_l + 2) % 3) * set_stride;
+          run_final_step<D>(run_ctl_args(), RunFinalArgs{states, rx->stats, rx->outs_host, rx->stats_host, rx->with_post, 0}, rit);
+        }
+        return;
+      }
+    }
     if (pv.stop || tile * (256 * PPT) >= pd.nm) return;
     load_T(pv.T, T);
     load_T(pv.Tprev, Tprev);
@@ -3104,6 +3306,8 @@
       linearize(std::false_type{}, acc, have && ca, p[k], pf[k], pn[k], pnm[k], qx, qy, qz, best);
     }
     if (have) S.prev_m[gi_[k]] = excl;
+    if constexpr (RUN)
+      if (have) pm[k] = excl;
   }
   if constexpr (defer) {
     {
@@ -3129,13 +3333,41 @@
         }
         if (open) {
           S.prev_m[gi_[0]] = sexcl[0];
+          if constexpr (RUN) pm[0] = sexcl[0];
           d_best  = sbest[0];
           d_valid = true;
         }
       }
       linearize(std::true_type{}, acc, d_valid, p[0], pf[0], pn[0], pnm[0], d_qx, d_qy, d_qz, d_best);
-      block_reduce_store_biased<4>(acc, S.partials, prob, tile, PPT);
+      block_reduce_store_biased<4>(acc, RUN ? rit.partials : S.partials, prob, tile, PPT);
       if constexpr (FUSED) PASS_TS(S.fc.epoch, 3);
+      if constexpr (RUN) {
+        asm volatile("s_waitcnt vmcnt(0)" ::: "memory");
+        __syncthreads();
+        if (threadIdx.x == 0)
+          __hip_atomic_fetch_add(rx->R.sync + (tile & (RUN_SYNC_SHARDS - 1)) * RUN_SYNC_STRIDE, 1u, __ATOMIC_RELAXED,
+                                 __HIP_MEMORY_SCOPE_AGENT);
+        const bool designated   = tile == 0 && threadIdx.x < 64;
+        const int round_n       = rx->R.round0 + ri + 1;
+        long long* const base   = rx->R.partials;
+        const size_t set_stride = (size_t) PARTIAL_SLOTS * ACC_N;
+        rit.epoch               = S.fc.epoch + ri + 1;
+        rit.partials            = base + (size_t) (round_n % 3) * set_stride;
+        rit.prev_partials       = base + (size_t) ((round_n + 2) % 3) * set_stride;
+        rit.zero_partials       = base + (size_t) ((round_n + 1) % 3) * set_stride;
+        if (ri + 1 < rx->R.n_iters) continue;
+        if (designated) {
+          const int ntiles = max((pd.nm + 255) / 256, 1);
+          if (run_wait_arrivals(rx->R.sync, (unsigned) (ntiles * (ri + 1)))) {
+            if (lane < RUN_SYNC_SHARDS)
+              __hip_atomic_store(rx->R.sync + lane * RUN_SYNC_STRIDE, 0u, __ATOMIC_RELAXED, __HIP_MEMORY_SCOPE_AGENT);
+            run_final_step<D>(run_ctl_args(), RunFinalArgs{states, rx->stats, rx->outs_host, rx->stats_host, rx->with_post, 0}, rit);
+          } else {
+            run_bail(rx->R, rx->R.seq, ri + 1);
+          }
+        }
+        return;
+      }
       return;
     }
   }
@@ -3216,6 +3448,8 @@
   if constexpr (FUSED) PASS_TS_ANY(S.fc.epoch, 4);
   block_reduce_store_biased<4, 2>(acc, S.partials, prob, tile, PPT);
   if constexpr (FUSED) PASS_TS(S.fc.epoch, 3);
+  return;
+  }
 }
 
 template <int DIM, bool PLANE, int PPT, bool GATHER, int FUSED>
@@ -4705,7 +4939,8 @@
 }
 
 __device__ void icp_finalize_block(const CtlParams& C, ProblemState* st, const srrg2_iteration_stats* stats,
-                                   ProblemOut* outs_host, srrg2_iteration_stats* stats_host, int prob, bool with_post) {
+                                   ProblemOut* outs_host, srrg2_iteration_stats* stats_host, int prob, bool with_post,
+                                   int nthreads = 0) {
   if (with_post) {
     if (threadIdx.x == 0) icp_post_one(C, st, stats, prob);
     __syncthreads();
@@ -4714,7 +4949,7 @@
     const int n       = min(st->nstats, C.max_stats) * (int) (sizeof(srrg2_iteration_stats) / sizeof(int));
     const int* src    = reinterpret_cast<const int*>(stats + (size_t) prob * C.max_stats);
     int* dst          = reinterpret_cast<int*>(stats_host + (size_t) prob * C.max_stats);
-    for (int k = threadIdx.x; k < n; k += blockDim.x) dst[k] = src[k];
+    for (int k = threadIdx.x; k < n; k += nthreads > 0 ? nthreads : (int) blockDim.x) dst[k] = src[k];
   }
   __threadfence_system();
   __syncthreads();
@@ -4768,13 +5003,14 @@
 }
 
 namespace srrg2amd {
-template <int D, int MAXS, bool PRIORS>
+template <int D, int MAXS, bool PRIORS, bool RUN>
 __device__ __forceinline__ void final_wave_body(const CtlParams& C, const SliceDev* __restrict__ Sv, int ns,
                                                 ProblemState* __restrict__ states, srrg2_iteration_stats* __restrict__ stats,
                                                 ProblemOut* __restrict__ outs_host, srrg2_iteration_stats* __restrict__ stats_host,
-                                                int with_post) {
+                                                int with_post, const RunIter* rit) {
   const FusedCtl& F = Sv[0].fc;
   const int prob = blockIdx.x + C.prob0;
+  const unsigned f_epoch = (unsigned) (RUN ? rit->epoch : F.epoch);
   const int lane = threadIdx.x & 63;
   ProblemState* st = &states[prob];
   unsigned long long g[MAXS];
@@ -4784,14 +5020,14 @@
     g[z] = 0ull;
     if (z < ns) {
       g[z]  = pub_load(F.pub + ((size_t) prob * SRRG2_MAX_SLICES + Sv[z].slice_idx) * PUB_SLICE_GRANULES + lane);
-      stale = stale || (unsigned) (g[z] >> 32) != (unsigned) F.epoch;
+      stale = stale || (unsigned) (g[z] >> 32) != f_epoch;
     }
   }
   int ncorr_l = 0;
   if (lane < SRRG2_MAX_SLICES) ncorr_l = st->ncorr[lane];
   FinalRegs fin;
   fin.applied = false;
-  if (__any(stale)) wave_control<D, MAXS, true, PRIORS, true>(Sv, ns, states, prob, g, nullptr, &fin);
+  if (__any(stale)) wave_control<D, MAXS, true, PRIORS, true, RUN>(Sv, ns, states, prob, g, nullptr, &fin, rit);
 #pragma unroll
   for (int z = 0; z < MAXS; ++z) {
     if (z >= ns) break;
@@ -4806,7 +5042,7 @@
   }
   if (!fin.applied || !fin.stats_written) {
     __threadfence();
-    icp_finalize_block(C, st, stats, outs_host, stats_host, prob, with_post != 0);
+    icp_finalize_block(C, st, stats, outs_host, stats_host, prob, with_post != 0, RUN ? 64 : 0);
     return;
   }
   int status    = SRRG2_SUCCESS;
@@ -4874,6 +5110,14 @@
                                                              ProblemOut* __restrict__ outs_host,
                                                              srrg2_iteration_stats* __restrict__ stats_host, int with_post) {
   final_wave_body<6, 4, PRIORS>(*P.s[0].fc.ctl, P.s, ns, states, stats, outs_host, stats_host, with_post);
+}
+template <int DIM, bool PLANE>
+__global__ __launch_bounds__(256, 4) void k_icp_run_fast(SliceDev S, RunArgs R, const ProblemDev* __restrict__ probs,
+                                                         ProblemState* __restrict__ states, srrg2_iteration_stats* __restrict__ stats,
+                                                         ProblemOut* __restrict__ outs_host,
+                                                         srrg2_iteration_stats* __restrict__ stats_host, int with_post) {
+  const RunCtx rx{R, stats, outs_host, stats_host, with_post};
+  icp_step_fast_body<DIM, PLANE, 1, false, 1, true>(S, probs, states, &rx);
 }
 }
 
@@ -5281,6 +5525,27 @@
   });
 }
 
+int icp_run_fast_blocks_per_cu(int dim, bool plane) {
+  int n = 0;
+  with_dim_plane(dim, plane, [&](auto D, auto P) {
+    if (hipOccupancyMaxActiveBlocksPerMultiprocessor(&n, k_icp_run_fast<D(), P()>, 256, 0) != hipSuccess) {
+      (void) hipGetLastError();
+      n = 0;
+    }
+  });
+  return n;
+}
+void launch_icp_run_fast(int dim, bool plane, const SliceDev& S, const RunArgs& R, const ProblemDev* probs,
+                         ProblemState* states, srrg2_iteration_stats* stats, ProblemOut* outs_host,
+                         srrg2_iteration_stats* stats_host, bool with_post, int max_nm, hipStream_t s) {
+  if (max_nm <= 0) return;
+  const dim3 grid(1, (max_nm + 255) / 256);
+  with_dim_plane(dim, plane, [&](auto D, auto P) {
+    hipLaunchKernelGGL((k_icp_run_fast<D(), P()>), grid, dim3(256), 0, s, S, R, probs, states, stats, outs_host, stats_host,
+                       with_post ? 1 : 0);
+  });
+}
+
 void launch_icp_final_wave(const CtlParams& C, const SliceDev& S, ProblemState* states, srrg2_iteration_stats* stats,
                            ProblemOut* outs_host, srrg2_iteration_stats* stats_host, bool with_post, hipStream_t s) {
   const dim3 grid(ctl_problems(C));
```
